# Blosc/c-blosc

Measured on AMD Instinct MI355X. Metric: compress+decompress GB/s (uncompressed) at 1/2/4/8 GPUs vs HBM roofline; ratio, higher is better.
Workload: dtype u8; 1 GPU; config #2: byte-shuffle + lz4 clevel=5 typesize=8, 128 x 64 MiB bench19 chunks per GPU (8 GiB), step = compress pass + decompress pass, device-resident; chunks_per_gpu=128, chunks_total=128, chunk_bytes=67108864

## Files before the change

c-blosc_amd/csrc/blosc_api.hip:

```cpp
#include <errno.h>
#include <pthread.h>
#include <stdio.h>
#include <stdlib.h>
#include <string.h>

#include <memory>
#include <new>

#include "../../include/blosc.h"
#include "../../include/blosc_gpu.h"
#include "../../include/blosc_gpu_packed.h"
#include "../../include/blosc_gpu_params.h"
#include "../../include/blosc_gpu_select.h"
#include "../../include/blosc_gpu_getitem.h"
#include "../../include/blosc_gpu_take.h"
#include "../../include/blosc_gpu_put.h"
#include "../../include/blosc_gpu_checksum.h"
#include "blosc_format.h"
#include "engine.h"

using namespace bamd;

static pthread_mutex_t g_mutex = PTHREAD_MUTEX_INITIALIZER;
static int g_compressor = BLOSC_BLOSCLZ;
// ... 289 lines not shown

int blosc_decompress(const void* src, void* dest, size_t destsize) {
  if (!g_initlib) blosc_init();
  const char* ev;
  if ((ev = getenv("BLOSC_NTHREADS")) != NULL) {
    long v = strtol(ev, NULL, 10);
    if (v != EINVAL && v > 0) { int r = blosc_set_nthreads((int)v); if (r < 0) return r; }
  }
  const bool nolock = getenv("BLOSC_NOLOCK") != NULL;
  if (!nolock) pthread_mutex_lock(&g_mutex);
  int r = decompress_one(src, dest, destsize);
  if (!nolock) pthread_mutex_unlock(&g_mutex);
  return r;
}

int blosc_getitem(const void* src, int start, int nitems, void* dest) {
  return engine_getitem(src, start, nitems, dest, engine_is_device_pointer(src), engine_is_device_pointer(dest), (hipStream_t)0);
}

int blosc_gpu_set_device(int device) { return engine_set_device(device); }

static int compress_batch(int clevel, int doshuffle, size_t typesize, const char* compressor, size_t blocksize,
                          int nchunks, const void* const* src, const size_t* nbytes, void* const* dest,
                          const size_t* destsize, int* cbytes_out, void* stream, bool device_ptrs) {
  if (nchunks <= 0) return 0;
  CompressParams p;
  if (!call_params(clevel, doshuffle, typesize, compressor, blocksize, &p)) return answer_not_built(nchunks, cbytes_out, nullptr);
  return compress_call(&p, false, nchunks, jobs_from_arrays(nchunks, src, dest, nbytes, destsize), cbytes_out, device_ptrs, stream, nullptr);
}
int blosc_gpu_compress_batch(int clevel, int doshuffle, size_t typesize, const char* compressor, size_t blocksize,
                             int nchunks, const void* const* src, const size_t* nbytes, void* const* dest,
                             const size_t* destsize, int* cbytes_out, void* stream) {
  return compress_batch(clevel, doshuffle, typesize, compressor, blocksize, nchunks, src, nbytes, dest, destsize, cbytes_out, stream, true);
}
int blosc_gpu_compress_batch_host(int clevel, int doshuffle, size_t typesize, const char* compressor, size_t blocksize,
                                  int nchunks, const void* const* src, const size_t* nbytes, void* const* dest,
                                  const size_t* destsize, int* cbytes_out) {
  return compress_batch(clevel, doshuffle, typesize, compressor, blocksize, nchunks, src, nbytes, dest, destsize, cbytes_out, nullptr, false);
}

static int decompress_batch(int nchunks, const void* const* src, const size_t* srcsize, void* const* dest,
                            const size_t* destsize, int* nbytes_out, void* stream, bool device_ptrs) {
  if (nchunks <= 0) return 0;
  return decompress_call(nchunks, jobs_from_arrays(nchunks, src, dest, srcsize, destsize), nbytes_out, device_ptrs, stream, nullptr);
}
int blosc_gpu_decompress_batch(int nchunks, const void* const* src, const size_t* srcsize, void* const* dest,
                               const size_t* destsize, int* nbytes_out, void* stream) {
  return decompress_batch(nchunks, src, srcsize, dest, destsize, nbytes_out, stream, true);
}
int blosc_gpu_decompress_batch_host(int nchunks, const void* const* src, const size_t* srcsize, void* const* dest,
                                    const size_t* destsize, int* nbytes_out) {
  return decompress_batch(nchunks, src, srcsize, dest, destsize, nbytes_out, nullptr, false);
}

size_t blosc_gpu_packed_bound(int nchunks, const size_t* nbytes, size_t align) {
  if (nchunks <= 0 || !nbytes || !packed_align(&align)) return 0;
  size_t total = 0;
  for (int i = 0; i < nchunks; i++) total += (nbytes[i] + BLOSC_MAX_OVERHEAD + align - 1) / align * align;
  return total;
}

int blosc_gpu_compress_packed(int clevel, int doshuffle, size_t typesize, const char* compressor, size_t blocksize,
                              int nchunks, const void* const* src, const size_t* nbytes, void* dest, size_t destsize, size_t align,
                              size_t* offsets_out, int* cbytes_out, void* stream) {
  const int c = packed_compress_opening(nchunks, src, nbytes, dest, destsize, &align, offsets_out, cbytes_out);
  if (c != kGo) return c;
  CompressParams p;
  if (!call_params(clevel, doshuffle, typesize, compressor, blocksize, &p)) return answer_not_built(nchunks, cbytes_out, offsets_out);
  const PackedBuffer pk{dest, destsize, align, offsets_out};
  return compress_call(&p, false, nchunks, jobs_from_arrays(nchunks, src, nullptr, nbytes, nullptr), cbytes_out, true, stream, &pk);
}

int blosc_gpu_compress_batch_params(int nchunks, const blosc_gpu_cparams* params, const void* const* src, const size_t* nbytes,
                                    void* const* dest, const size_t* destsize, int* cbytes_out, void* stream) {
  if (nchunks <= 0) return 0;
  if (!params || !src || !nbytes || !dest || !destsize || !cbytes_out) return -1;
  return compress_call(chunk_params(nchunks, params).get(), true, nchunks, jobs_from_arrays(nchunks, src, dest, nbytes, destsize), cbytes_out, true, stream,
                       nullptr);
}
int blosc_gpu_compress_packed_params(int nchunks, const blosc_gpu_cparams* params, const void* const* src, const size_t* nbytes,
                                     void* dest, size_t destsize, size_t align, size_t* offsets_out, int* cbytes_out, void* stream) {
  const int c = packed_compress_opening(nchunks, src, nbytes, dest, destsize, &align, offsets_out, cbytes_out);
  if (c != kGo) return c;
  if (!params) return -1;
  const PackedBuffer pk{dest, destsize, align, offsets_out};
  return compress_call(chunk_params(nchunks, params).get(), true, nchunks, jobs_from_arrays(nchunks, src, nullptr, nbytes, nullptr), cbytes_out, true, stream,
                       &pk);
}

static bool select_tables(int nchunks, const int* cand_first, const blosc_gpu_cparams* cands, const int* choice_out) {
  if (!cand_first || !cands || !choice_out || cand_first[0] != 0) return false;
  for (int i = 0; i < nchunks; i++) if (cand_first[i + 1] < cand_first[i]) return false;
  return true;
}
int blosc_gpu_compress_batch_select(int nchunks, const int* cand_first, const blosc_gpu_cparams* cands, const void* const* src, const size_t* nbytes,
                                    void* const* dest, const size_t* destsize, int* cbytes_out, int* choice_out, int* cand_cbytes_out, void* stream) {
  if (nchunks <= 0) return 0;
  if (!src || !nbytes || !dest || !destsize || !cbytes_out || !select_tables(nchunks, cand_first, cands, choice_out)) return -1;
  const CandidateSelect sel{cand_first, choice_out, cand_cbytes_out};
  return compress_call(chunk_params(cand_first[nchunks], cands).get(), true, nchunks, jobs_from_arrays(nchunks, src, dest, nbytes, destsize), cbytes_out, true,
                       stream, nullptr, &sel);
}
int blosc_gpu_compress_packed_select(int nchunks, const int* cand_first, const blosc_gpu_cparams* cands, const void* const* src, const size_t* nbytes,
                                     void* dest, size_t destsize, size_t align, size_t* offsets_out, int* cbytes_out, int* choice_out,
                                     int* cand_cbytes_out, void* stream) {
  const int c = packed_compress_opening(nchunks, src, nbytes, dest, destsize, &align, offsets_out, cbytes_out);
  if (c != kGo) return c;
  if (!select_tables(nchunks, cand_first, cands, choice_out)) return -1;
  const PackedBuffer pk{dest, destsize, align, offsets_out};
  const CandidateSelect sel{cand_first, choice_out, cand_cbytes_out};
  return compress_call(chunk_params(cand_first[nchunks], cands).get(), true, nchunks, jobs_from_arrays(nchunks, src, nullptr, nbytes, nullptr), cbytes_out, true,
                       stream, &pk, &sel);
}

int blosc_gpu_decompress_packed(int nchunks, const void* container, size_t containersize, const size_t* offsets,
                                void* dest, size_t destsize, size_t* dest_offsets_out, int* nbytes_out, void* stream) {
  const int c = packed_opening(nchunks, dest_offsets_out);
  if (c != kGo) return c;
  if (!container || !offsets || !nbytes_out) return -1;
  const PackedBuffer pk{dest, dest ? destsize : 0, 0, dest_offsets_out};
  return decompress_call(nchunks, jobs_from_spans(nchunks, container, containersize, offsets, nullptr, BLOSC_MIN_HEADER_LENGTH), nbytes_out, true, stream, &pk);
}

int blosc_gpu_cbuffer_sizes_batch(int nchunks, const void* const* src, size_t* nbytes, size_t* cbytes, size_t* blocksize, void* stream) {
  if (nchunks < 0 || (nchunks > 0 && !src)) return -1;
  if (nchunks == 0) return 0;
  Table<Header> h = table<Header>(nchunks);
  if (!h) return -1;
  const int r = engine_chunk_headers(nchunks, src, h.get(), (hipStream_t)stream);
  for (int i = 0; r == 0 && i < nchunks; i++) {
    const bool known = h[i].version == BLOSC_VERSION_FORMAT;
    if (nbytes) nbytes[i] = known ? (size_t)h[i].nbytes : 0;
    if (cbytes) cbytes[i] = known ? (size_t)h[i].cbytes : 0;
    if (blocksize) blocksize[i] = known ? (size_t)h[i].blocksize : 0;
  }
  return r;
}

int blosc_gpu_device_count(void) { return engine_device_count(); }
int blosc_gpu_partition(size_t nchunks, int world, int rank, size_t* lo, size_t* hi) {
  if (world <= 0 || rank < 0 || rank >= world || !lo || !hi) return -1;
  const size_t w = (size_t)world, r = (size_t)rank;
  size_t l = (r * nchunks + w - 1) / w, h = ((r + 1) * nchunks + w - 1) / w;
  if (h > nchunks) h = nchunks;
  *lo = l; *hi = h;
  return 0;
}
struct MultiArg {
  int dev, rc; bool compress; size_t lo, hi;
  int clevel, doshuffle; size_t typesize; const char* compressor; size_t blocksize;
  const void* const* src; const size_t* insize; void* const* dest; const size_t* destsize; int* out;
};
static void* multi_worker(void* p) {
  MultiArg& a = *(MultiArg*)p;
  a.rc = 0;
  if (a.hi == a.lo) return nullptr;
  if (engine_thread_device(a.dev) != 0) { a.rc = -1; return nullptr; }
  const int n = (int)(a.hi - a.lo);
  const bool devp = engine_is_device_pointer(a.src[a.lo]);
  if (a.compress) a.rc = compress_batch(a.clevel, a.doshuffle, a.typesize, a.compressor, a.blocksize, n, a.src + a.lo, a.insize + a.lo, a.dest + a.lo,
                                        a.destsize + a.lo, a.out + a.lo, nullptr, devp);
  else a.rc = decompress_batch(n, a.src + a.lo, a.insize ? a.insize + a.lo : nullptr, a.dest + a.lo, a.destsize + a.lo, a.out + a.lo, nullptr, devp);
  (void)engine_thread_device(-1);
  return nullptr;
}
static int run_multi(MultiArg proto, int ndev, const int* devices, int nchunks) {
  if (nchunks <= 0) return 0;
  const int have = engine_device_count();
  if (ndev <= 0 || ndev > 64) return -1;
  MultiArg args[64];
  pthread_t th[64];
  for (int r = 0; r < ndev; r++) {
    args[r] = proto;
    args[r].dev = devices ? devices[r] : r;
    if (args[r].dev < 0 || args[r].dev >= have) { fprintf(stderr, "blosc_amd: multi-GPU call names device %d, this node shows %d\n", args[r].dev, have); return -1; }
    (void)blosc_gpu_partition((size_t)nchunks, ndev, r, &args[r].lo, &args[r].hi);
  }
  int started = 0, rc = 0;
  for (; started < ndev; started++) if (pthread_create(&th[started], nullptr, multi_worker, &args[started]) != 0) { rc = -1; break; }
  for (int r = 0; r < started; r++) { pthread_join(th[r], nullptr); if (args[r].rc < 0) rc = args[r].rc; }
  return rc;
}
int blosc_gpu_compress_batch_multi(int ndev, const int* devices, int clevel, int doshuffle, size_t typesize, const char* compressor, size_t blocksize,
                                   int nchunks, const void* const* src, const size_t* nbytes, void* const* dest, const size_t* destsize, int* cbytes_out) {
  MultiArg a{}; a.compress = true; a.clevel = clevel; a.doshuffle = doshuffle; a.typesize = typesize; a.compressor = compressor; a.blocksize = blocksize;
  a.src = src; a.insize = nbytes; a.dest = dest; a.destsize = destsize; a.out = cbytes_out;
  return run_multi(a, ndev, devices, nchunks);
}
int blosc_gpu_decompress_batch_multi(int ndev, const int* devices, int nchunks, const void* const* src, const size_t* srcsize, void* const* dest,
                                     const size_t* destsize, int* nbytes_out) {
  MultiArg a{}; a.compress = false; a.src = src; a.insize = srcsize; a.dest = dest; a.destsize = destsize; a.out = nbytes_out;
  return run_multi(a, ndev, devices, nchunks);
}

int blosc_gpu_getitem(const void* src, int start, int nitems, void* dest, void* stream) {
  return engine_getitem(src, start, nitems, dest, true, true, (hipStream_t)stream);
}

int blosc_gpu_getitem_batch(int nchunks, const void* const* src, int nranges, const int* chunk, const int* start, const int* nitems,
                            void* const* dest, int* result_out, void* stream) {
  if (nchunks < 0 || nranges < 0) return -1;
  if (nranges == 0) return 0;
  if ((nchunks > 0 && !src) || !chunk || !start || !nitems || !dest || !result_out) return -1;
  return getitem_call(nchunks, jobs_from_arrays(nchunks, src, nullptr, nullptr, nullptr), nranges, chunk, start, nitems, dest, result_out, stream, nullptr);
}
int blosc_gpu_getitem_packed(int nchunks, const void* container, size_t containersize, const size_t* offsets,
                             int nranges, const int* chunk, const int* start, const int* nitems,
                             void* dest, size_t destsize, size_t* dest_offsets_out, int* result_out, void* stream) {
  if (nchunks < 0) return -1;
  const int c = packed_opening(nranges, dest_offsets_out);
  if (c != kGo) return c;
  if ((nchunks > 0 && (!container || !offsets)) || !chunk || !start || !nitems || !result_out) return -1;
  const PackedBuffer pk{dest, dest ? destsize : 0, 0, dest_offsets_out};
  return getitem_call(nchunks, jobs_from_spans(nchunks, container, containersize, offsets, nullptr, BLOSC_MIN_HEADER_LENGTH), nranges, chunk, start, nitems,
                      nullptr, result_out, stream, &pk);
}

static int take_opening(int nchunks, size_t row_bytes, size_t nidx, const void* index, const void* dest) {
  if (nchunks < 0 || row_bytes < 1 || row_bytes > 65536) return -1;
  if (nidx && (!index || !dest)) return -1;
  return kGo;
}
static int take_call(int nchunks, const Table<Job>& jobs, size_t row_bytes, size_t nidx, const int64_t* index, void* dest, int* status,
                     int* chunk_rows_out, size_t* failed_out, void* stream) {
  if (!jobs) return -1;
  if (nchunks == 0 && nidx == 0) return 0;
  return engine_take(nchunks, jobs.get(), row_bytes, nidx, index, dest, status, chunk_rows_out, failed_out, (hipStream_t)stream);
}
int blosc_gpu_take_batch(int nchunks, const void* const* src, size_t row_bytes, size_t nidx, const int64_t* index, void* dest, int* status,
                         int* chunk_rows_out, size_t* failed_out, void* stream) {
  const int c = take_opening(nchunks, row_bytes, nidx, index, dest);
  if (c != kGo) return c;
  if (nchunks > 0 && !src) return -1;
  return take_call(nchunks, jobs_from_arrays(nchunks, src, nullptr, nullptr, nullptr), row_bytes, nidx, index, dest, status, chunk_rows_out, failed_out, stream);
}
int blosc_gpu_take_packed(int nchunks, const void* container, size_t containersize, const size_t* offsets, size_t row_bytes, size_t nidx,
                          const int64_t* index, void* dest, int* status, int* chunk_rows_out, size_t* failed_out, void* stream) {
  const int c = take_opening(nchunks, row_bytes, nidx, index, dest);
  if (c != kGo) return c;
  if (nchunks > 0 && (!container || !offsets)) return -1;
  return take_call(nchunks, jobs_from_spans(nchunks, container, containersize, offsets, nullptr, BLOSC_MIN_HEADER_LENGTH), row_bytes, nidx, index, dest, status,
                   chunk_rows_out, failed_out, stream);
}

static int put_opening(int nchunks, size_t row_bytes, size_t nidx, const void* index, const void* rows, const blosc_gpu_cparams* params, void* dest,
                       size_t destsize, size_t* align, size_t* offsets_out, int* cbytes_out) {
  const int c = take_opening(nchunks, row_bytes, nidx, index, rows);
  if (c != kGo) return c;
  if (nidx > (size_t)UINT32_MAX - 1 || !packed_align(align) || !offsets_out || (!dest && destsize)) return -1;
  if (nchunks > 0 && (!params || !cbytes_out)) return -1;
  return kGo;
}
static int put_call(int nchunks, const Table<Job>& jobs, size_t row_bytes, size_t nidx, const int64_t* index, const void* rows, const blosc_gpu_cparams* params,
                    void* dest, size_t destsize, size_t align, size_t* offsets_out, int* cbytes_out, int* rewritten_out, int* status, int* chunk_rows_out,
                    size_t* failed_out, void* stream) {
  if (!jobs) return -1;
  if (nchunks == 0 && nidx == 0) { offsets_out[0] = 0; if (failed_out) *failed_out = 0; return 0; }
  Table<CompressParams> p = chunk_params(nchunks, params);
  if (!p) return -1;
  const PackedBuffer pk{dest, destsize, align, offsets_out};
  return engine_put(nchunks, jobs.get(), row_bytes, nidx, index, rows, p.get(), &pk, cbytes_out, rewritten_out, status, chunk_rows_out, failed_out, (hipStream_t)stream);
}
int blosc_gpu_put_batch(int nchunks, const void* const* src, size_t row_bytes, size_t nidx, const int64_t* index, const void* rows,
                        const blosc_gpu_cparams* params, void* dest, size_t destsize, size_t align, size_t* offsets_out, int* cbytes_out,
                        int* rewritten_out, int* status, int* chunk_rows_out, size_t* failed_out, void* stream) {
  const int c = put_opening(nchunks, row_bytes, nidx, index, rows, params, dest, destsize, &align, offsets_out, cbytes_out);
  if (c != kGo) return c;
  if (nchunks > 0 && !src) return -1;
  return put_call(nchunks, jobs_from_arrays(nchunks, src, nullptr, nullptr, nullptr), row_bytes, nidx, index, rows, params, dest, destsize, align, offsets_out,
                  cbytes_out, rewritten_out, status, chunk_rows_out, failed_out, stream);
}
int blosc_gpu_put_packed(int nchunks, const void* container, size_t containersize, const size_t* offsets, size_t row_bytes, size_t nidx,
                         const int64_t* index, const void* rows, const blosc_gpu_cparams* params, void* dest, size_t destsize, size_t align,
                         size_t* offsets_out, int* cbytes_out, int* rewritten_out, int* status, int* chunk_rows_out, size_t* failed_out, void* stream) {
  const int c = put_opening(nchunks, row_bytes, nidx, index, rows, params, dest, destsize, &align, offsets_out, cbytes_out);
  if (c != kGo) return c;
  if (nchunks > 0 && (!container || !offsets)) return -1;
  const uintptr_t s0 = (uintptr_t)container, s1 = s0 + containersize, d0 = (uintptr_t)dest, d1 = d0 + destsize;
  if (nchunks > 0 && destsize && containersize && s0 < d1 && d0 < s1) return -1;
  return put_call(nchunks, jobs_from_spans(nchunks, container, containersize, offsets, nullptr, BLOSC_MIN_HEADER_LENGTH), row_bytes, nidx, index, rows, params,
                  dest, destsize, align, offsets_out, cbytes_out, rewritten_out, status, chunk_rows_out, failed_out, stream);
}

int blosc_gpu_checksum_batch(int kind, int nruns, const void* const* src, const size_t* nbytes, unsigned int* digest_out, void* stream) {
  const int c = checksum_opening(kind, nruns);
  if (c != kGo) return c;
  if (!src || !nbytes || !digest_out) return -1;
  return checksum_call(kind, nruns, jobs_from_arrays(nruns, src, nullptr, nbytes, nullptr), digest_out, stream);
}
int blosc_gpu_checksum_packed(int kind, int nruns, const void* container, size_t containersize, const size_t* offsets,
                              const size_t* length, unsigned int* digest_out, void* stream) {
  const int c = checksum_opening(kind, nruns);
  if (c != kGo) return c;
  if (!offsets || !digest_out) return -1;
  if (!container && offsets[nruns] > offsets[0]) return -1;
  return checksum_call(kind, nruns, jobs_from_spans(nruns, container, containersize, offsets, length, 0), digest_out, stream);
}

__attribute__((visibility("default"))) int blosc_internal_persistent_grids(int cap, const char** names, int* launched, int* occupancy) {
  return bamd::engine_persistent_grids(cap, names, launched, occupancy);
}
__attribute__((visibility("default"))) int blosc_internal_enc_lz_occupancy(int dynamic_lds) { return bamd::engine_enc_lz_occupancy(dynamic_lds); }
__attribute__((visibility("default"))) void blosc_internal_last_compress_tasks(unsigned out[3]) { bamd::engine_last_compress_tasks(out); }

__attribute__((visibility("default"))) void blosc_internal_shuffle(const size_t typesize, const size_t blocksize,
                                                                   const uint8_t* src, const uint8_t* dest) {
  if (engine_filter(0, typesize, blocksize, src, (void*)dest) != 0) fprintf(stderr, "blosc_amd: shuffle failed (no GPU?)\n");
}
__attribute__((visibility("default"))) void blosc_internal_unshuffle(const size_t typesize, const size_t blocksize,
                                                                     const uint8_t* src, const uint8_t* dest) {
  if (engine_filter(1, typesize, blocksize, src, (void*)dest) != 0) fprintf(stderr, "blosc_amd: unshuffle failed (no GPU?)\n");
}
__attribute__((visibility("default"))) void blosc_internal_shuffle_generic(const size_t typesize, const size_t blocksize,
                                                                           const uint8_t* const src, uint8_t* const dest) {
  blosc_internal_shuffle(typesize, blocksize, src, dest);
}
__attribute__((visibility("default"))) void blosc_internal_unshuffle_generic(const size_t typesize, const size_t blocksize,
                                                                             const uint8_t* const src, uint8_t* const dest) {
  blosc_internal_unshuffle(typesize, blocksize, src, dest);
}
#define BAMD_SHUFFLE_ALIAS(isa)                                                                                                                  \
  __attribute__((visibility("default"))) void blosc_internal_shuffle_##isa(const size_t typesize, const size_t blocksize, const uint8_t* const src, \
                                                                           uint8_t* const dest) { blosc_internal_shuffle(typesize, blocksize, src, dest); } \
  __attribute__((visibility("default"))) void blosc_internal_unshuffle_##isa(const size_t typesize, const size_t blocksize, const uint8_t* const src, \
                                                                             uint8_t* const dest) { blosc_internal_unshuffle(typesize, blocksize, src, dest); }
BAMD_SHUFFLE_ALIAS(sse2)
BAMD_SHUFFLE_ALIAS(avx2)
#undef BAMD_SHUFFLE_ALIAS
__attribute__((visibility("default"))) int blosc_internal_bitshuffle(const size_t typesize, const size_t blocksize,
                                                                     const uint8_t* src, const uint8_t* dest,
                                                                     const uint8_t* tmp) {
  (void)tmp;
  if (engine_filter(2, typesize, blocksize, src, (void*)dest) != 0) return -1;
  const size_t n = blocksize / typesize;
  return (int)((n % 8) ? n : n * typesize);
}
__attribute__((visibility("default"))) int blosc_internal_bitunshuffle(const size_t typesize, const size_t blocksize,
                                                                       const uint8_t* src, const uint8_t* dest,
                                                                       const uint8_t* tmp) {
  (void)tmp;
  if (engine_filter(3, typesize, blocksize, src, (void*)dest) != 0) return -1;
  const size_t n = blocksize / typesize;
  return (int)((n % 8) ? n : n * typesize);
}

__attribute__((visibility("default"))) int blosc_amd_policy_blocksize(int clevel, int typesize, int nbytes, int forced,
                                                                      int codec, int splitmode) {
  return compute_blocksize(clevel, typesize, nbytes, forced, codec, splitmode);
}
__attribute__((visibility("default"))) int blosc_amd_policy_split(int codec, int typesize, int blocksize, int splitmode) {
  return split_block(codec, typesize, blocksize, splitmode);
}
__attribute__((visibility("default"))) void blosc_amd_getitem_pass_bytes(size_t bytes) { engine_getitem_pass_bytes(bytes); }

__attribute__((visibility("default"))) void blosc_amd_checksum_tile_bytes(size_t bytes) { engine_checksum_tile_bytes(bytes); }

void blosc_gpu_profile(int enable) { engine_prof_enable(enable); }
void blosc_gpu_profile_reset(void) { engine_prof_reset(); }
int blosc_gpu_profile_get(const char* kernel, double* total_ms, int* launches) { return engine_prof_get(kernel, total_ms, launches); }

}
```

c-blosc_amd/csrc/enc_lz.h:

```cpp
constexpr int ENC_WAVES = 1;
#ifndef BAMD_ENC_HASH_BITS
#define BAMD_ENC_HASH_BITS 11
#endif
constexpr int ENC_HASH_BITS = BAMD_ENC_HASH_BITS;
constexpr int ENC_TAB = 1 << ENC_HASH_BITS;
typedef uint32_t enc_entry_t;
#ifndef BAMD_ENC_SPLIT_TAB
#define BAMD_ENC_SPLIT_TAB 1
#endif
constexpr int ENC_TAB_BYTES = BAMD_ENC_SPLIT_TAB ? ENC_TAB * 3 : ENC_TAB * 4;
#ifndef BAMD_ENC_MINWAVES
#define BAMD_ENC_MINWAVES (BAMD_ENC_SPLIT_TAB ? 6 : 5)
#endif
#ifndef BAMD_ENC_SEQ_SKIPCAP
#define BAMD_ENC_SEQ_SKIPCAP 32u
#endif
#ifndef BAMD_ENC_LZ_MINWAVES
#define BAMD_ENC_LZ_MINWAVES 6
#endif
constexpr int LDS_BYTES_PER_CU = 160 * 1024;
constexpr int LDS_GRANULE_BYTES = 1280;
constexpr int lds_occupied(int bytes) { return (bytes + LDS_GRANULE_BYTES - 1) / LDS_GRANULE_BYTES * LDS_GRANULE_BYTES; }
constexpr int lds_workgroups_per_cu(int bytes) { return bytes > 0 ? LDS_BYTES_PER_CU / lds_occupied(bytes) : 32; }
constexpr int ENC_LDS_WAVES = lds_workgroups_per_cu(ENC_TAB_BYTES);
constexpr int ENC_WAVES_PER_CU = ENC_LDS_WAVES < 4 * BAMD_ENC_MINWAVES ? ENC_LDS_WAVES : 4 * BAMD_ENC_MINWAVES;
constexpr int ENC_LZ_SCR_BYTES = 256;
constexpr int ENC_LZ_LDS_WAVES = lds_workgroups_per_cu(ENC_TAB_BYTES + ENC_LZ_SCR_BYTES);
constexpr int ENC_LZ_WAVES_PER_CU = ENC_LZ_LDS_WAVES < 4 * BAMD_ENC_LZ_MINWAVES ? ENC_LZ_LDS_WAVES : 4 * BAMD_ENC_LZ_MINWAVES;
static_assert(lds_occupied(ENC_TAB_BYTES + ENC_LZ_SCR_BYTES) * ENC_LZ_WAVES_PER_CU <= LDS_BYTES_PER_CU, "the LZ4 kernel's workgroups of one CU fit its LDS");

struct EncTable {
  __attribute__((address_space(3))) uint32_t* w;
  __attribute__((address_space(3))) uint16_t* pos;
  __attribute__((address_space(3))) uint8_t* tag;
  __device__ __forceinline__ void init(void* base) {
    w = (__attribute__((address_space(3))) uint32_t*)base;
    pos = (__attribute__((address_space(3))) uint16_t*)base;
    tag = (__attribute__((address_space(3))) uint8_t*)base + 2 * ENC_TAB;
  }
  __device__ __forceinline__ void clear(int lane) {
    for (int k = lane; k < ENC_TAB_BYTES / 4; k += 64) w[k] = 0u;
  }
  __device__ __forceinline__ void put(uint32_t h, uint32_t entry) {
    if (BAMD_ENC_SPLIT_TAB) { pos[h] = (uint16_t)entry; tag[h] = (uint8_t)(entry >> 24); }
    else w[h] = entry;
  }
  __device__ __forceinline__ uint32_t get(uint32_t h) const {
    if (BAMD_ENC_SPLIT_TAB) return (uint32_t)pos[h] | ((uint32_t)tag[h] << 24);
    return w[h];
  }
  __device__ __forceinline__ static bool tag_equal(uint32_t a, uint32_t b) {
    return BAMD_ENC_SPLIT_TAB ? ((a ^ b) >> 24) == 0u : ((a ^ b) >> 16) == 0u;
  }
};

__device__ __forceinline__ uint32_t enc_mix(uint32_t seq) { return seq * 2654435761u; }
__device__ __forceinline__ uint32_t enc_slot(uint32_t mix) { return mix >> (32 - ENC_HASH_BITS); }
__device__ __forceinline__ uint32_t enc_entry(uint32_t mix, uint32_t p) { return ((mix << ENC_HASH_BITS) & 0xffff0000u) | (p & 0xffffu); }

__device__ __forceinline__ uint64_t ld8u(const gu8* p) { return g_ld8(p); }

__device__ __forceinline__ uint32_t common16(const uint4& x, const uint4& y) {
  const uint64_t lo = ((uint64_t)(x.y ^ y.y) << 32) | (x.x ^ y.x);
  const uint64_t hi = ((uint64_t)(x.w ^ y.w) << 32) | (x.z ^ y.z);
  if (lo) return (uint32_t)__builtin_ctzll(lo) >> 3;
  return hi ? 8u + ((uint32_t)__builtin_ctzll(hi) >> 3) : 16u;
}

__device__ __forceinline__ uint32_t wave_common_fwd_rest(const gu8* src, uint32_t n, uint32_t a, uint32_t b,
                                                         uint32_t maxlen, uint32_t done, int lane) {
  if (done == 256u && done < maxlen && a + done + 1024u <= n) {
    const uint4 x0 = g_ld16(src + a + done + 16 * lane), y0 = g_ld16(src + b + done + 16 * lane);
    const uint32_t q1 = done + 16u * (uint32_t)lane;
    uint32_t e1 = common16(x0, y0);
    const uint32_t r1 = q1 < maxlen ? maxlen - q1 : 0u;
    if (e1 > r1) e1 = r1;
    const uint64_t s1 = __ballot(e1 < 16u);
    if (s1) { const int f = __builtin_ctzll(s1); return done + 16u * (uint32_t)f + (uint32_t)__builtin_amdgcn_readlane((int)e1, f); }
    done += 1024u;
  }
  while (done < maxlen && a + done + 2048u <= n) {
    const gu8* pa = src + a + done + 16 * lane;
    const gu8* pb = src + b + done + 16 * lane;
    const uint4 x0 = g_ld16(pa), x1 = g_ld16(pa + 1024);
    const uint4 y0 = g_ld16(pb), y1 = g_ld16(pb + 1024);
    const uint32_t q = done + 16u * (uint32_t)lane;
    uint32_t e0 = common16(x0, y0), e1 = common16(x1, y1);
    const uint32_t r0 = q < maxlen ? maxlen - q : 0u;
    const uint32_t r1 = q + 1024u < maxlen ? maxlen - q - 1024u : 0u;
    if (e0 > r0) e0 = r0;
    if (e1 > r1) e1 = r1;
    const uint64_t s0 = __ballot(e0 < 16u);
    if (s0) { const int f = __builtin_ctzll(s0); return done + 16u * (uint32_t)f + (uint32_t)__builtin_amdgcn_readlane((int)e0, f); }
    const uint64_t s1 = __ballot(e1 < 16u);
    if (s1) { const int f = __builtin_ctzll(s1); return done + 1024u + 16u * (uint32_t)f + (uint32_t)__builtin_amdgcn_readlane((int)e1, f); }
    done += 2048u;
  }
  while (done < maxlen) {
    const uint32_t q = done + 8u * (uint32_t)lane;
    uint32_t vb = 0;
    if (q < maxlen) vb = (maxlen - q < 8u) ? maxlen - q : 8u;
    uint32_t eq = 0;
    if (vb) {
      if (a + q + 8u <= n) {
        uint64_t x = ld8u(src + a + q) ^ ld8u(src + b + q);
        eq = x ? (uint32_t)(__builtin_ctzll(x) >> 3) : 8u;
        if (eq > vb) eq = vb;
      } else {
        while (eq < vb && src[a + q + eq] == src[b + q + eq]) eq++;
      }
    }
    const uint64_t stop = __ballot(eq < 8u);
    if (stop) {
      const int f = __builtin_ctzll(stop);
      return done + 8u * (uint32_t)f + (uint32_t)__builtin_amdgcn_readlane((int)eq, f);
    }
    done += 512u;
  }
  return maxlen;
}
__device__ __forceinline__ uint32_t wave_common_first256(uint32_t x, uint32_t maxlen, int lane) {
  const uint32_t q = 4u * (uint32_t)lane;
  uint32_t e0 = x ? (uint32_t)(__builtin_ctz(x) >> 3) : 4u;
  const uint32_t r0 = q < maxlen ? maxlen - q : 0u;
  if (e0 > r0) e0 = r0;
  const uint64_t s0 = __ballot(e0 < 4u);
  if (s0) { const int f = __builtin_ctzll(s0); return 4u * (uint32_t)f + (uint32_t)__builtin_amdgcn_readlane((int)e0, f); }
  return 0xffffffffu;
}
__device__ __forceinline__ uint32_t wave_common_fwd(const gu8* src, uint32_t n, uint32_t a, uint32_t b,
                                                    uint32_t maxlen, int lane) {
  uint32_t done = 0;
  if (maxlen && a + 256u <= n) {
    const uint32_t r = wave_common_first256(g_ld4(src + a + 4 * lane) ^ g_ld4(src + b + 4 * lane), maxlen, lane);
    if (r != 0xffffffffu) return r;
    done = 256u;
  }
  return wave_common_fwd_rest(src, n, a, b, maxlen, done, lane);
}

#ifdef BAMD_ENC_NOSTORE
#define ENC_ST1(ptr, val) do { (void)(ptr); (void)(val); } while (0)
#else
#define ENC_ST1(ptr, val) do { *(ptr) = (val); } while (0)
#endif
__device__ __forceinline__ uint32_t emit_ext255(gu8* p, uint32_t v, int lane) {
  const uint32_t n255 = v / 255u, rem = v - n255 * 255u;
  for (uint32_t k = (uint32_t)lane; k < n255; k += 64u) ENC_ST1(p + k, (uint8_t)255u);
  if (lane == 0) ENC_ST1(p + n255, (uint8_t)rem);
  return n255 + 1u;
}

enum { EF_LZ4 = 0, EF_BLOSCLZ = 1, EF_ZSTD = 2, EF_ZLIB = 3, EF_ZLIB2 = 4 };
#ifndef BAMD_ZSTD_MINLEN
#define BAMD_ZSTD_MINLEN 4
#endif

struct ZsSink {
  gu8* lit;
  uint32_t nlit, litcap;
  BAMD_GAS uint64_t* seq;
  uint32_t nseq, seqcap;
};
__device__ __forceinline__ uint32_t zs_emit_seq(ZsSink& z, const gu8* lit, uint32_t ll, uint32_t off, uint32_t mlen, int lit_lane0, uint32_t ownbyte, int lane);

struct DflSink {
  gu8* out; uint32_t cap;
  uint32_t pos;
  uint32_t acc, nb;
  volatile BAMD_LAS uint32_t* zb;
};
__device__ __forceinline__ uint32_t wave_incl_scan_u32(uint32_t v, int lane) {
#pragma unroll
  for (int d = 1; d < 64; d <<= 1) { const uint32_t t = (uint32_t)__shfl_up((int)v, d, 64); if (lane >= d) v += t; }
  return v;
}
__device__ __forceinline__ bool dfl_put_symbols(DflSink& z, uint32_t bits, uint32_t nbits, int lane) {
  const uint32_t incl = wave_incl_scan_u32(nbits, lane);
  const uint32_t total = (uint32_t)__builtin_amdgcn_readlane((int)incl, 63);
  z.zb[lane] = lane == 0 ? z.acc : 0u;
  if (lane == 0) z.zb[64] = 0u;
  BAMD_LDS_SYNC();
  if (nbits) {
    const uint32_t start = z.nb + incl - nbits, w = start >> 5, sh = start & 31u;
    __hip_atomic_fetch_or((BAMD_LAS uint32_t*)z.zb + w, bits << sh, __ATOMIC_RELAXED, __HIP_MEMORY_SCOPE_WAVEFRONT);
    if (sh + nbits > 32u) __hip_atomic_fetch_or((BAMD_LAS uint32_t*)z.zb + w + 1u, bits >> (32u - sh), __ATOMIC_RELAXED, __HIP_MEMORY_SCOPE_WAVEFRONT);
  }
  const uint32_t fill = z.nb + total, ndw = fill >> 5;
  if (z.pos + 4u * ndw + 16u > z.cap) return false;
  BAMD_LDS_SYNC();
  const uint32_t mine = z.zb[lane], rest = z.zb[ndw];
  if ((uint32_t)lane < ndw) g_st4(z.out + z.pos + 4u * (uint32_t)lane, mine);
  z.acc = uni(rest); z.nb = fill & 31u; z.pos += 4u * ndw;
  return true;
}
__device__ __forceinline__ uint32_t dfl_emit_seq(DflSink& z, const gu8* lit, uint32_t ll, uint32_t dist, uint32_t mlen, int lit_lane0, uint32_t ownbyte, int lane) {
  const bool in_regs = lit_lane0 >= 0 && ll <= 64u && (uint32_t)lit_lane0 + ll <= 64u;
  const uint32_t np = mlen ? dfl::npieces(mlen) : 0u;
  uint32_t ldone = 0, pdone = 0;
  do {
    const uint32_t lcnt = ll - ldone < 64u ? ll - ldone : 64u;
    uint32_t pcnt = 0;
    if (ldone + lcnt == ll) { pcnt = np - pdone < 64u - lcnt ? np - pdone : 64u - lcnt; }
    const uint32_t vreg = in_regs ? (uint32_t)__builtin_amdgcn_ds_bpermute((int)(((uint32_t)lit_lane0 + (uint32_t)lane) & 63u) << 2, (int)ownbyte) & 0xffu : 0u;
    dfl::Sym s = {0u, 0u};
    if ((uint32_t)lane < lcnt) s = dfl::literal(in_regs ? vreg : (uint32_t)lit[ldone + (uint32_t)lane]);
    else if ((uint32_t)lane < lcnt + pcnt) s = dfl::match(dfl::piece_len(mlen, pdone + (uint32_t)lane - lcnt, np), dist);
    if (!dfl_put_symbols(z, s.bits, s.nbits, lane)) return 0xffffffffu;
    ldone += lcnt; pdone += pcnt;
  } while (ldone < ll || pdone < np);
  return 0u;
}

__device__ __forceinline__ void emit_literals(gu8* dst, const gu8* lit, uint32_t ll, int lit_lane0, uint32_t ownbyte, int lane) {
  if (lit_lane0 >= 0 && ll <= 64u && (uint32_t)lit_lane0 + ll <= 64u) {
    const uint32_t v = (uint32_t)__builtin_amdgcn_ds_bpermute((int)(((uint32_t)lit_lane0 + (uint32_t)lane) & 63u) << 2, (int)ownbyte);
    if ((uint32_t)lane < ll) ENC_ST1(dst + lane, (uint8_t)v);
  } else {
    wave_copy_disjoint(dst, lit, ll, lane);
  }
}

__device__ __forceinline__ uint32_t lz4_emit_seq(gu8* dst, uint32_t op, uint32_t cap, const gu8* lit,
                                                 uint32_t ll, uint32_t off, uint32_t mlen, int lit_lane0, uint32_t ownbyte, int lane) {
  if (op + 1u + ll + (2u + 1u + 5u) + ll / 255u > cap) return 0xffffffffu;
  const uint32_t mcode = mlen - 4u;
  if (ll < 15u && mcode < 15u + 255u && (ll == 0u || (lit_lane0 >= 0 && (uint32_t)lit_lane0 + ll <= 64u))) {
    if (op + 1u + ll + 2u + (1u + 5u) + (mcode + 240u) / 255u > cap) return 0xffffffffu;
    const uint32_t v = (uint32_t)__builtin_amdgcn_ds_bpermute((int)(((uint32_t)lit_lane0 + (uint32_t)lane - 1u) & 63u) << 2, (int)ownbyte);
    uint32_t b = v;
    b = lane == 0 ? ((ll << 4) | (mcode < 15u ? mcode : 15u)) : b;
    b = (uint32_t)lane == ll + 1u ? off : b;
    b = (uint32_t)lane == ll + 2u ? off >> 8 : b;
    b = (uint32_t)lane == ll + 3u ? mcode - 15u : b;
    const uint32_t total = ll + 3u + (mcode >= 15u ? 1u : 0u);
    if ((uint32_t)lane < total) ENC_ST1(dst + op + lane, (uint8_t)b);
    return op + total;
  }
  const uint32_t tok = ((ll < 15u ? ll : 15u) << 4) | (mcode < 15u ? mcode : 15u);
  if (lane == 0) ENC_ST1(dst + op, (uint8_t)tok);
  op += 1u;
  if (ll >= 15u) op += emit_ext255(dst + op, ll - 15u, lane);
  emit_literals(dst + op, lit, ll, lit_lane0, ownbyte, lane);
  op += ll;
  if (lane < 2) ENC_ST1(dst + op + lane, (uint8_t)(off >> (8 * lane)));
  op += 2u;
  if (op + (1u + 5u) + (mcode + 240u) / 255u > cap) return 0xffffffffu;
  if (mcode >= 15u) op += emit_ext255(dst + op, mcode - 15u, lane);
  return op;
}
__device__ __forceinline__ uint32_t lz4_emit_tail(gu8* dst, uint32_t op, uint32_t cap, const gu8* lit,
                                                  uint32_t run, int lane) {
  if (op + run + 1u + (run + 255u - 15u) / 255u > cap) return 0xffffffffu;
  if (lane == 0) dst[op] = (uint8_t)((run < 15u ? run : 15u) << 4);
  op += 1u;
  if (run >= 15u) op += emit_ext255(dst + op, run - 15u, lane);
  wave_copy_disjoint(dst + op, lit, run, lane);
  return op + run;
}

__device__ __forceinline__ uint32_t blz_emit_literals(gu8* dst, uint32_t op, uint32_t cap, const gu8* lit,
                                                      uint32_t ll, int lane) {
  if (ll == 0u) return op;
  const uint32_t nch = (ll + 31u) >> 5;
  if (op + ll + nch > cap) return 0xffffffffu;
  for (uint32_t c = (uint32_t)lane; c < nch; c += 64u) {
    const uint32_t cnt = (ll - 32u * c < 32u) ? ll - 32u * c : 32u;
    dst[op + 33u * c] = (uint8_t)(cnt - 1u);
  }
  for (uint32_t k = (uint32_t)lane; k < ll; k += 64u) dst[op + k + (k >> 5) + 1u] = lit[k];
  return op + ll + nch;
}
__device__ __forceinline__ uint32_t blz_emit_match(gu8* dst, uint32_t op, uint32_t cap, uint32_t dist,
                                                   uint32_t mlen, int lane) {
  const uint32_t L = mlen - 2u;
  uint32_t bd = dist - 1u;
  const bool far = bd >= 8191u;
  if (far) bd -= 8191u;
  const uint32_t hi = far ? 31u : (bd >> 8);
  const uint32_t next = (L >= 7u) ? (L - 7u) / 255u + 1u : 0u;
  const uint32_t total = 1u + next + (far ? 3u : 1u);
  if (op + total + 2u > cap) return 0xffffffffu;
  if (lane == 0) dst[op] = (uint8_t)(((L < 7u ? L : 7u) << 5) | hi);
  op += 1u;
  if (L >= 7u) op += emit_ext255(dst + op, L - 7u, lane);
  if (far) {
    if (lane == 0) { dst[op] = 255u; dst[op + 1] = (uint8_t)(bd >> 8); dst[op + 2] = (uint8_t)bd; }
    op += 3u;
  } else {
    if (lane == 0) dst[op] = (uint8_t)bd;
    op += 1u;
  }
  return op;
}

#ifndef BAMD_ENC_RANK_CAP
#define BAMD_ENC_RANK_CAP 20
#endif
constexpr uint32_t RANK_CAP = BAMD_ENC_RANK_CAP;

struct Bytes20 { uint64_t a, b; uint32_t c; };

__device__ __forceinline__ Bytes20 load20(const gu8* src, uint32_t pos, uint32_t n) {
  Bytes20 r;
  if (pos + 20u <= n) { r.a = g_ld8(src + pos); r.b = g_ld8(src + pos + 8u); r.c = RANK_CAP > 16u ? g_ld4(src + pos + 16u) : 0u; }
  else {
    r.a = 0; r.b = 0; r.c = 0;
    for (uint32_t k = 0; k < 20u && pos + k < n; k++) {
      const uint64_t v = src[pos + k];
      if (k < 8u) r.a |= v << (8u * k); else if (k < 16u) r.b |= v << (8u * (k - 8u)); else r.c |= (uint32_t)v << (8u * (k - 16u));
    }
  }
  return r;
}
__device__ __forceinline__ uint32_t common20(const Bytes20& x, const Bytes20& y) {
  uint64_t d = x.a ^ y.a;
  if (d) return (uint32_t)__builtin_ctzll(d) >> 3;
  d = x.b ^ y.b;
  if (d) return 8u + ((uint32_t)__builtin_ctzll(d) >> 3);
  const uint32_t e = x.c ^ y.c;
  return e ? 16u + ((uint32_t)__builtin_ctz(e) >> 3) : 20u;
}
__device__ __forceinline__ uint32_t runlen20(const Bytes20& x, uint32_t v) {
  const uint64_t rep = 0x0101010101010101ull * (uint64_t)v;
  Bytes20 y; y.a = rep; y.b = rep; y.c = (uint32_t)rep;
  return common20(x, y);
}
template <int N> __device__ __forceinline__ uint32_t dpp_row_shr0(uint32_t v) {
  return (uint32_t)__builtin_amdgcn_update_dpp(0, (int)v, 0x110 + N, 0xf, 0xf, true);
}
__device__ __forceinline__ uint32_t wave_max_u32(uint32_t v) {
  uint32_t t;
// ... 452 lines not shown
```

c-blosc_amd/csrc/enc_lz4p.h:

```cpp
#ifndef BAMD_ENC_PAR
#define BAMD_ENC_PAR 1
#endif
constexpr int ENC_SCR_BYTES = 256;
static_assert(ENC_SCR_BYTES == ENC_LZ_SCR_BYTES, "enc_lz.h sizes the persistent grid with this scratch in mind");
static_assert((ENC_TAB_BYTES + ENC_SCR_BYTES) % LDS_GRANULE_BYTES == 0 || !BAMD_ENC_SPLIT_TAB, "table + scratch fill whole LDS granules");
#ifndef BAMD_ENC_BACK2
#define BAMD_ENC_BACK2 1
#endif
#ifndef BAMD_ENC_SKIPCAP
#define BAMD_ENC_SKIPCAP 32u
#endif
#ifndef BAMD_ENC_NEIGHBOUR
#define BAMD_ENC_NEIGHBOUR 4u
#endif
#ifndef BAMD_ENC_KEEPJ
#define BAMD_ENC_KEEPJ 0
#endif
#ifndef BAMD_ENC_EXT2
#define BAMD_ENC_EXT2 1
#endif
#ifndef BAMD_ENC_LAUNDER
#define BAMD_ENC_LAUNDER 1
#endif
#ifndef BAMD_ENC_PREFULL
#define BAMD_ENC_PREFULL 1
#endif

template <int N> __device__ __forceinline__ uint32_t dpp_row_shl0(uint32_t v) {
  return (uint32_t)__builtin_amdgcn_update_dpp(0, (int)v, 0x100 + N, 0xf, 0xf, true);
}
__device__ __forceinline__ uint32_t umax32(uint32_t a, uint32_t b) { return a > b ? a : b; }
__device__ __forceinline__ uint32_t umin32(uint32_t a, uint32_t b) { return a < b ? a : b; }

__device__ __forceinline__ uint32_t wave_common_fwd_lite(const gu8* src, uint32_t n, uint32_t a, uint32_t b, uint32_t maxlen, int lane) {
  uint32_t done = 0;
  if (maxlen && a + 256u <= n) {
    const uint32_t x = g_ld4(src + a + 4 * lane) ^ g_ld4(src + b + 4 * lane);
    const uint32_t q = 4u * (uint32_t)lane;
    uint32_t e0 = x ? (uint32_t)(__builtin_ctz(x) >> 3) : 4u;
    const uint32_t r0 = q < maxlen ? maxlen - q : 0u;
    if (e0 > r0) e0 = r0;
    const uint64_t s0 = __ballot(e0 < 4u);
    if (s0) { const int f = __builtin_ctzll(s0); return 4u * (uint32_t)f + (uint32_t)__builtin_amdgcn_readlane((int)e0, f); }
    done = 256u;
  }
  while (done < maxlen && a + done + 1024u <= n) {
    const uint4 x0 = g_ld16(src + a + done + 16 * lane), y0 = g_ld16(src + b + done + 16 * lane);
    const uint32_t q1 = done + 16u * (uint32_t)lane;
    uint32_t e1 = common16(x0, y0);
    const uint32_t r1 = q1 < maxlen ? maxlen - q1 : 0u;
    if (e1 > r1) e1 = r1;
    const uint64_t s1 = __ballot(e1 < 16u);
    if (s1) { const int f = __builtin_ctzll(s1); return done + 16u * (uint32_t)f + (uint32_t)__builtin_amdgcn_readlane((int)e1, f); }
    done += 1024u;
  }
  while (done < maxlen) {
    const uint32_t q = done + 8u * (uint32_t)lane;
    uint32_t vb = 0;
    if (q < maxlen) vb = (maxlen - q < 8u) ? maxlen - q : 8u;
    uint32_t eq = 0;
    if (vb) {
      if (a + q + 8u <= n) {
        const uint64_t x = ld8u(src + a + q) ^ ld8u(src + b + q);
        eq = x ? (uint32_t)(__builtin_ctzll(x) >> 3) : 8u;
        if (eq > vb) eq = vb;
      } else {
        while (eq < vb && src[a + q + eq] == src[b + q + eq]) eq++;
      }
    }
    const uint64_t stop = __ballot(eq < 8u);
    if (stop) { const int f = __builtin_ctzll(stop); return done + 8u * (uint32_t)f + (uint32_t)__builtin_amdgcn_readlane((int)eq, f); }
    done += 512u;
  }
  return maxlen;
}

template <int SS>
__device__ uint32_t lz4_encode_wave_par(const gu8* __restrict__ src, uint32_t n, gu8* __restrict__ dst, uint32_t cap,
                                        int clevel, enc_entry_t* tab_generic, int lane_in EPROF_ARG) {
  static_assert(SS == 0 || SS == 1, "one or two positions per lane");
  const int lane = lane_in;
  constexpr uint32_t SPAN = 64u << SS;
  EncTable tab;
  tab.init((void*)tab_generic);
  volatile BAMD_LAS uint32_t* scr = (volatile BAMD_LAS uint32_t*)((BAMD_LAS uint8_t*)(void*)tab_generic + ENC_TAB_BYTES);
  if (n < 13u) return 0u;
  const uint32_t last_start = n - 12u;
  const uint32_t mlimit = n - 5u;
  const int accel = 10 - clevel;
  const uint32_t minlen = clevel >= 9 ? 4u : (clevel >= 6 ? 5u : 7u);
  tab.clear(lane);
  EncWindow win;
  win.init(src, n, lane);
  uint32_t ip = 0, anchor = 0, op = 0, nfail = 0;
  bool ins_pending = false;
  while (ip <= last_start) {
    int lane = lane_in;
#if !defined(BAMD_WAVE_EMU) && BAMD_ENC_LAUNDER
    asm volatile("; lane of this step" : "+v"(lane));
#endif
    const uint32_t lq = (uint32_t)lane << SS;
    const uint32_t p = ip + lq;
    const bool live = p <= last_start;
    const bool live1 = SS && p + 1u <= last_start;
    win.seek(ip, lane);
    const uint32_t lo = ip >= 4u ? ip - 4u : 0u;
    const uint32_t rb = lo & ~3u;
    const uint32_t D = (rb - win.wbase) >> 2;
    const int gsel = (int)((D + (uint32_t)lane) << 2);
    const uint32_t ra = (uint32_t)__builtin_amdgcn_ds_bpermute(gsel, (int)win.w0);
    const uint32_t rc = (uint32_t)__builtin_amdgcn_ds_bpermute(gsel, (int)win.w1);
    const uint32_t r = (D + (uint32_t)lane < 64u) ? ra : rc;
    const uint32_t bo0 = ip - rb;
    const uint32_t bo = bo0 + lq;
    const int ksel = (int)((bo >> 2) << 2);
    const uint32_t x0 = (uint32_t)__builtin_amdgcn_ds_bpermute(ksel, (int)r);
    const uint32_t x1 = (uint32_t)__builtin_amdgcn_ds_bpermute(ksel + 4, (int)r);
    const uint32_t x2 = (uint32_t)__builtin_amdgcn_ds_bpermute(ksel + 8, (int)r);
    const uint32_t x3 = (uint32_t)__builtin_amdgcn_ds_bpermute(ksel + 12, (int)r);
    const uint32_t x4 = (uint32_t)__builtin_amdgcn_ds_bpermute(ksel + 16, (int)r);
    const uint32_t x5 = (uint32_t)__builtin_amdgcn_ds_bpermute(ksel + 20, (int)r);
    const uint32_t sh = bo & 3u;
    const uint32_t o0 = __builtin_amdgcn_alignbyte(x1, x0, sh), o1 = __builtin_amdgcn_alignbyte(x2, x1, sh);
    const uint32_t o2 = __builtin_amdgcn_alignbyte(x3, x2, sh), o3 = __builtin_amdgcn_alignbyte(x4, x3, sh);
    const uint32_t o4 = __builtin_amdgcn_alignbyte(x5, x4, sh);
    const uint32_t ownpre = __builtin_amdgcn_alignbyte(x0, (uint32_t)__builtin_amdgcn_ds_bpermute(ksel - 4, (int)r), sh);
    Bytes20 own;
    own.a = ((uint64_t)o1 << 32) | o0; own.b = ((uint64_t)o3 << 32) | o2; own.c = RANK_CAP > 16u ? o4 : 0u;
    const uint64_t r01 = ((uint64_t)(uint32_t)__builtin_amdgcn_readlane((int)r, 1) << 32) | (uint32_t)__builtin_amdgcn_readlane((int)r, 0);
    const uint32_t before2 = bo0 >= 2u ? (uint32_t)(r01 >> (8u * (bo0 - 2u))) & 0xffffu : 0u;
    uint32_t prev;
    if (SS) prev = ownpre >> 24;
    else prev = (uint32_t)__builtin_amdgcn_update_dpp(0, (int)(o0 & 0xffu), 0x138, 0xf, 0xf, false);
    if (lane == 0) prev = ip ? (bo0 >= 2u ? before2 >> 8 : (uint32_t)(r01 >> (8u * (bo0 - 1u))) & 0xffu) : 0x100u;
    if (ins_pending) {
      const uint32_t m2 = enc_mix(before2 | (o0 << 16));
      if (lane == 0) tab.put(enc_slot(m2), enc_entry(m2, ip - 2u));
      ins_pending = false;
    }
    uint32_t cand = 0, limit = 0;
    bool tab_ok = false;
    const uint32_t mix = enc_mix(o0);
#define PAR_PUT() do { const uint32_t mix_ = enc_mix((uint32_t)own.a); tab.put(enc_slot(mix_), enc_entry(mix_, p)); } while (0)
#define PAR_PUT1() do { const uint32_t mix1_ = enc_mix((uint32_t)(own.a >> 8)); tab.put(enc_slot(mix1_), enc_entry(mix1_, p + 1u)); } while (0)
    if (live) {
      limit = mlimit - p; if (limit > RANK_CAP) limit = RANK_CAP;
      const uint32_t h = enc_slot(mix), mine = enc_entry(mix, p);
      const uint32_t e = tab.get(h);
      const uint32_t d = (p - e) & 0xffffu;
      if (d != 0u && d <= p && EncTable::tag_equal(e, mine)) { cand = p - d; tab_ok = true; }
    } else {
      prev = 0x100u;
    }
    PROF_LAP(8); PROF_ADD(0, 1);
    uint32_t len = 0, nb = 0;
    if (tab_ok) {
      const uint32_t cpre = cand >= 4u ? ld4u(src + cand - 4u) : 0u;
      const Bytes20 cb = load20(src, cand, n);
      if (cand >= 4u) { const uint32_t x = cpre ^ ownpre; nb = x ? (uint32_t)__builtin_clz(x) >> 3 : 4u; }
      len = common20(own, cb);
      if (len > limit) len = limit;
      if (len < 4u || len + (SS && nb ? 1u : 0u) < minlen) len = 0;
    }
    if (live && prev < 0x100u) {
      uint32_t rl = runlen20(own, prev);
      if (rl > limit) rl = limit;
      const uint32_t xr = (ownpre ^ (ownpre << 8)) | 0xffu;
      const uint32_t nbr = p >= 5u ? (uint32_t)__builtin_clz(xr) >> 3 : 0u;
      if (rl >= 4u && rl + (SS && nbr ? 1u : 0u) >= minlen && rl > len) { len = rl; cand = p - 1u; nb = nbr; }
    }
    win.settle(lane);
    PROF_LAP(9);
    const uint32_t step_end = ip + SPAN;
    const uint32_t cn = (p - cand) | (nb << 28);
    uint32_t S = len ? (((len + (SS && nb ? 1u : 0u) + SPAN - lq) << 11) | ((63u - (uint32_t)lane) << 5) | len) : 0u;
    S = umax32(S, dpp_row_shl0<1>(S)); S = umax32(S, dpp_row_shl0<2>(S)); S = umax32(S, dpp_row_shl0<4>(S)); S = umax32(S, dpp_row_shl0<8>(S));
    {
      const uint32_t t3 = (uint32_t)__builtin_amdgcn_readlane((int)S, 48);
      const uint32_t t2 = umax32((uint32_t)__builtin_amdgcn_readlane((int)S, 32), t3);
      const uint32_t t1 = umax32((uint32_t)__builtin_amdgcn_readlane((int)S, 16), t2);
      const uint32_t add = lane < 16 ? t1 : (lane < 32 ? t2 : (lane < 48 ? t3 : 0u));
      S = umax32(S, add);
    }
    uint32_t J0;
    {
      const uint32_t wS = 63u - ((S >> 5) & 63u), LS = S & 31u;
      const uint32_t nx = ((wS << SS) + LS + (SS ? 1u : 0u)) >> SS;
      J0 = (S == 0u || LS >= RANK_CAP || nx > 63u) ? 63u : nx;
    }
#if BAMD_ENC_KEEPJ
    const uint32_t J1 = (uint32_t)__builtin_amdgcn_ds_bpermute((int)(J0 << 2), (int)J0);
    const uint32_t J2 = (uint32_t)__builtin_amdgcn_ds_bpermute((int)(J1 << 2), (int)J1);
    const uint32_t J3 = (uint32_t)__builtin_amdgcn_ds_bpermute((int)(J2 << 2), (int)J2);
#endif
    uint32_t lane_lo = 0;
    bool any = false, tail_open = false;
    for (;;) {
#if !defined(BAMD_WAVE_EMU) && BAMD_ENC_LAUNDER
      asm volatile("; lane of this chain" : "+v"(lane));
#endif
#if !BAMD_ENC_KEEPJ
      const uint32_t J1 = (uint32_t)__builtin_amdgcn_ds_bpermute((int)(J0 << 2), (int)J0);
      const uint32_t J2 = (uint32_t)__builtin_amdgcn_ds_bpermute((int)(J1 << 2), (int)J1);
      const uint32_t J3 = (uint32_t)__builtin_amdgcn_ds_bpermute((int)(J2 << 2), (int)J2);
#endif
      uint32_t c = umin32((lane_lo + (SS ? 1u : 0u)) >> SS, 63u);
      { const uint32_t t = (uint32_t)__builtin_amdgcn_ds_bpermute((int)(c << 2), (int)J0); c = (lane & 1) ? t : c; }
      { const uint32_t t = (uint32_t)__builtin_amdgcn_ds_bpermute((int)(c << 2), (int)J1); c = (lane & 2) ? t : c; }
      { const uint32_t t = (uint32_t)__builtin_amdgcn_ds_bpermute((int)(c << 2), (int)J2); c = (lane & 4) ? t : c; }
      { const uint32_t t = (uint32_t)__builtin_amdgcn_ds_bpermute((int)(c << 2), (int)J3); c = (lane & 8) ? t : c; }
      const uint32_t Sr = (uint32_t)__builtin_amdgcn_ds_bpermute((int)(c << 2), (int)S);
      const bool valid = lane < 16 && c < 63u && Sr != 0u;
      const uint32_t nseq = (uint32_t)__builtin_popcountll(__ballot(valid));
      if (nseq == 0u) { tail_open = any; break; }
      any = true;
      const uint32_t last = nseq - 1u;
      const uint32_t w = 63u - ((Sr >> 5) & 63u), L = Sr & 31u;
      const uint32_t wq = w << SS;
      const uint32_t cnr = (uint32_t)__builtin_amdgcn_ds_bpermute((int)(w << 2), (int)cn);
      const uint32_t dist_r = cnr & 0xffffu, nb_r = cnr >> 28;
      const uint32_t cand_r = ip + wq - dist_r;
      uint32_t cq = c;
      if (SS) { const uint32_t e_prev = dpp_row_shr0<1>(wq + L); cq = lane == 0 ? lane_lo : e_prev; }
      const uint32_t room = wq - cq;
      const uint32_t w_last = (uint32_t)__builtin_amdgcn_readlane((int)wq, (int)last), L_last = (uint32_t)__builtin_amdgcn_readlane((int)L, (int)last);
      const uint32_t pm_last = ip + w_last;
      uint32_t mext = 0;
      if (L_last >= RANK_CAP && pm_last + RANK_CAP < mlimit) {
        const uint32_t c_last = (uint32_t)__builtin_amdgcn_readlane((int)cand_r, (int)last);
        mext = BAMD_ENC_EXT2 ? wave_common_fwd(src, n, pm_last + RANK_CAP, c_last + RANK_CAP, mlimit - (pm_last + RANK_CAP), lane)
                              : wave_common_fwd_lite(src, n, pm_last + RANK_CAP, c_last + RANK_CAP, mlimit - (pm_last + RANK_CAP), lane);
      }
      uint32_t back = valid ? umin32(nb_r, umin32(room, cand_r)) : 0u;
      if (BAMD_ENC_BACK2) {
        const bool more = valid && back == 4u && room > 4u && cand_r >= 12u;
        if (__ballot(more)) {
          const uint32_t pm = ip + wq;
          const uint64_t a = g_ld8(src + (more ? pm - 12u : 0u)), b = g_ld8(src + (more ? cand_r - 12u : 0u));
          const uint64_t x = a ^ b;
          const uint32_t eq = x ? (uint32_t)__builtin_clzll(x) >> 3 : 8u;
          if (more) back += umin32(eq, room - 4u);
        }
      }
      uint32_t pre = lane_lo == 0u ? ip - anchor : 0u;
      uint32_t pre_ext = 0;
      if (BAMD_ENC_PREFULL && pre) {
        const uint32_t b0 = (uint32_t)__builtin_amdgcn_readlane((int)back, 0), room0 = (uint32_t)__builtin_amdgcn_readlane((int)room, 0);
        const uint32_t cand0 = (uint32_t)__builtin_amdgcn_readlane((int)cand_r, 0);
        if (b0 == room0 && cand0 > b0) {
          uint32_t maxb = umin32(pre, cand0 - b0);
          if (maxb > 64u) maxb = 64u;
          const uint32_t pm0 = ip + (uint32_t)__builtin_amdgcn_readlane((int)wq, 0) - b0, cm0 = cand0 - b0;
          const bool bl = (uint32_t)lane < maxb;
          const uint32_t bx = src[bl ? pm0 - 1u - (uint32_t)lane : pm0], by = src[bl ? cm0 - 1u - (uint32_t)lane : cm0];
          const uint64_t bm = __ballot(!bl || bx != by);
          pre_ext = bm ? (uint32_t)__builtin_ctzll(bm) : 64u;
          pre -= pre_ext;
        }
      }
      PROF_LAP(10); PROF_ADD(2, L_last >= RANK_CAP); PROF_ADD(6, nseq);
      const uint32_t mlen = L + back + ((uint32_t)lane == last ? mext : 0u) + (lane == 0 ? pre_ext : 0u);
      const uint32_t mcode = mlen - 4u;
      const uint32_t inl = room - back;
      const uint32_t ll = inl + (lane == 0 ? pre : 0u);
      const bool r0pre = pre != 0u && lane == 0;
      const uint32_t hdr = r0pre ? 0u : (ll >= 15u ? 2u : 1u);
      const uint32_t nme = mcode >= 15u ? 1u : 0u;
      const uint32_t size = valid ? hdr + inl + 2u + nme : 0u;
      uint32_t incl = size;
      incl += dpp_row_shr0<1>(incl); incl += dpp_row_shr0<2>(incl); incl += dpp_row_shr0<4>(incl); incl += dpp_row_shr0<8>(incl);
      const uint32_t excl = incl - size;
      const uint32_t mcode_last = (uint32_t)__builtin_amdgcn_readlane((int)mcode, (int)last);
      const uint32_t extra_last = mcode_last >= 15u + 255u ? (mcode_last - 15u) / 255u : 0u;
      const uint32_t total = (uint32_t)__builtin_amdgcn_readlane((int)incl, (int)last) + extra_last;
      uint32_t ll0 = 0, prebytes = 0;
      if (pre) { ll0 = (uint32_t)__builtin_amdgcn_readlane((int)ll, 0); prebytes = 1u + (ll0 >= 15u ? 1u + (ll0 - 15u) / 255u : 0u) + pre; }
      if (op + prebytes + total + 8u > cap) return 0u;
      if (pre) {
        const uint32_t mc0 = (uint32_t)__builtin_amdgcn_readlane((int)mcode, 0);
        if (lane == 0) ENC_ST1(dst + op, (uint8_t)(((ll0 < 15u ? ll0 : 15u) << 4) | (mc0 < 15u ? mc0 : 15u)));
        op += 1u;
        if (ll0 >= 15u) op += emit_ext255(dst + op, ll0 - 15u, lane);
        wave_copy_disjoint(dst + op, src + anchor, pre, lane);
        op += pre;
        PROF_ADD(3, 1);
      }
      scr[lane] = 0u;
      BAMD_LDS_SYNC();
      if (valid) scr[cq >> SS] = 0x80000000u | (excl + hdr) | (inl << 10) | (w << 17) | (L << 23) | (SS ? (cq & 1u) << 28 : 0u);
      BAMD_LDS_SYNC();
      const uint32_t pw = scr[lane];
      const uint32_t myw = (SS && (pw & (1u << 28))) ? 0u : pw;
      const uint32_t myw1 = (SS && (pw & (1u << 28))) ? pw : 0u;
      const uint64_t fm = __ballot((myw >> 31) != 0u);
      uint32_t s;
      bool has;
      if (SS) {
        const uint64_t fm1 = __ballot((myw1 >> 31) != 0u);
        const uint64_t be = fm & ((2ull << lane) - 1ull), bo_ = fm1 & ((1ull << lane) - 1ull);
        const uint32_t se = 2u * (63u - (uint32_t)__builtin_clzll(be | 1ull)), so = 2u * (63u - (uint32_t)__builtin_clzll(bo_ | 1ull)) + 1u;
        s = (bo_ != 0ull && (be == 0ull || so > se)) ? so : se;
        has = (be | bo_) != 0ull;
      } else {
        const uint64_t below = fm & ((2ull << lane) - 1ull);
        s = 63u - (uint32_t)__builtin_clzll(below | 1ull);
        has = below != 0ull;
      }
      const uint32_t inf = scr[s >> SS];
      BAMD_LDS_SYNC();
      {
        const uint32_t tpos = op + excl;
        if (valid && hdr) ENC_ST1(dst + tpos, (uint8_t)(((ll < 15u ? ll : 15u) << 4) | (mcode < 15u ? mcode : 15u)));
        if (valid && hdr == 2u) ENC_ST1(dst + tpos + 1u, (uint8_t)(ll - 15u));
        const uint32_t opos = tpos + hdr + inl;
#ifndef BAMD_ENC_NOSTORE
        if (valid) g_st2(dst + opos, dist_r);
#endif
        if (valid && nme) ENC_ST1(dst + opos + 2u, (uint8_t)(mcode - 15u < 255u ? mcode - 15u : 255u));
        if (extra_last) {
          const uint32_t opos_last = (uint32_t)__builtin_amdgcn_readlane((int)opos, (int)last);
          emit_ext255(dst + opos_last + 2u, mcode_last - 15u, lane);
        }
      }
      {
        const uint32_t k = lq - s;
        const uint32_t i_out = inf & 1023u, i_inl = (inf >> 10) & 127u, i_w = ((inf >> 17) & 63u) << SS, i_L = (inf >> 23) & 31u;
        if (has && k < i_inl) ENC_ST1(dst + op + i_out + k, (uint8_t)own.a);
        const bool open_end = i_L < RANK_CAP;
        const uint32_t e = i_w + i_L;
        if (live && has && (lq <= i_w || (open_end && (lq + 2u == e || lq >= e)))) PAR_PUT();
      }
      if (SS) {
        const bool own1 = (myw1 >> 31) != 0u;
        const uint32_t inf1 = own1 ? myw1 : inf;
        const bool has1 = has || own1;
        const uint32_t q1 = lq + 1u, k1 = own1 ? 0u : q1 - s;
        const uint32_t j_out = inf1 & 1023u, j_inl = (inf1 >> 10) & 127u, j_w = ((inf1 >> 17) & 63u) << SS, j_L = (inf1 >> 23) & 31u;
        if (has1 && k1 < j_inl) ENC_ST1(dst + op + j_out + k1, (uint8_t)(own.a >> 8));
        const bool open1 = j_L < RANK_CAP;
        const uint32_t e1 = j_w + j_L;
        if (live1 && has1 && (q1 <= j_w || (open1 && (q1 + 2u == e1 || q1 >= e1)))) PAR_PUT1();
      }
      op += total;
      const uint32_t e_last = w_last + L_last + mext;
      anchor = ip + e_last;
      PROF_LAP(11);
      if (L_last < RANK_CAP || e_last >= SPAN) break;
      lane_lo = e_last;
      if (live && lq + 2u == lane_lo) PAR_PUT();
      if (live1 && lq + 3u == lane_lo) PAR_PUT1();
    }
    if (!any) {
      PROF_ADD(1, 1);
      if (live) PAR_PUT();
      if (live1) PAR_PUT1();
      nfail += 1u << SS;
      uint32_t adv = (nfail * (uint32_t)accel) / 16u;
      if (adv > BAMD_ENC_SKIPCAP - (1u << SS)) adv = BAMD_ENC_SKIPCAP - (1u << SS);
      if (BAMD_ENC_NEIGHBOUR && ((nfail >> SS) & (BAMD_ENC_NEIGHBOUR - 1u)) == 0u) adv = 0u;
      ip += SPAN + 64u * adv;
      continue;
    }
    nfail = 0;
    if (anchor >= step_end) {
      ip = anchor;
      ins_pending = true;
    } else {
      if (tail_open && live && lq >= lane_lo) PAR_PUT();
      if (tail_open && live1 && lq + 1u >= lane_lo) PAR_PUT1();
      ip = step_end;
    }
  }
#undef PAR_PUT
#undef PAR_PUT1
  op = lz4_emit_tail(dst, op, cap, src + anchor, n - anchor, lane);
  if (op == 0xffffffffu) return 0u;
  PROF_LAP(12);
  return op < n ? op : 0u;
}

#ifndef BAMD_ENC_STRIDE2_MAXCLEVEL
#define BAMD_ENC_STRIDE2_MAXCLEVEL 5
#endif
__device__ __forceinline__ uint32_t lz4_encode_wave_auto(const gu8* __restrict__ src, uint32_t n, gu8* __restrict__ dst, uint32_t cap,
                                                         int clevel, enc_entry_t* tab_generic, int lane EPROF_ARG) {
  if (clevel <= BAMD_ENC_STRIDE2_MAXCLEVEL) return lz4_encode_wave_par<1>(src, n, dst, cap, clevel, tab_generic, lane EPROF_PASS);
  return lz4_encode_wave_par<0>(src, n, dst, cap, clevel, tab_generic, lane EPROF_PASS);
}
```

c-blosc_amd/csrc/enc_shuffle.h:

```cpp
template <int T>
struct ElemRows { uint4 a, b; };

template <int T>
__device__ __forceinline__ ElemRows<T> shuffle_load(const gu8* src, uint32_t e, int lane) {
  ElemRows<T> x;
  const gu8* in = src + (size_t)(e + 4u * (uint32_t)lane) * T;
  x.a = g_ld16(in);
  if (T == 8) x.b = g_ld16(in + 16); else x.b = make_uint4(0, 0, 0, 0);
  return x;
}
template <int T>
__device__ __forceinline__ void shuffle_store(gu8* dst, uint32_t N, uint32_t e, int lane, const ElemRows<T>& x) {
  gu8* o = dst + e + 4u * (uint32_t)lane;
  uint32_t r0, r1, r2, r3;
  if (T == 8) {
    transpose4x4(x.a.x, x.a.z, x.b.x, x.b.z, r0, r1, r2, r3);
    g_st4(o, r0); g_st4(o + (size_t)N, r1); g_st4(o + 2 * (size_t)N, r2); g_st4(o + 3 * (size_t)N, r3);
    transpose4x4(x.a.y, x.a.w, x.b.y, x.b.w, r0, r1, r2, r3);
    g_st4(o + 4 * (size_t)N, r0); g_st4(o + 5 * (size_t)N, r1); g_st4(o + 6 * (size_t)N, r2); g_st4(o + 7 * (size_t)N, r3);
  } else {
    transpose4x4(x.a.x, x.a.y, x.a.z, x.a.w, r0, r1, r2, r3);
    g_st4(o, r0); g_st4(o + (size_t)N, r1); g_st4(o + 2 * (size_t)N, r2); g_st4(o + 3 * (size_t)N, r3);
  }
}
struct ElemRows2 { uint32_t lo, hi; };
struct ElemRows16 { uint4 v[4]; };
__device__ __forceinline__ ElemRows2 shuffle_load2(const gu8* src, uint32_t e, int lane) {
  const uint64_t w = g_ld8(src + (size_t)(e + 4u * (uint32_t)lane) * 2u);
  ElemRows2 x; x.lo = (uint32_t)w; x.hi = (uint32_t)(w >> 32);
  return x;
}
__device__ __forceinline__ void shuffle_rows2(const ElemRows2& x, uint32_t (&r)[16]) {
  r[0] = __builtin_amdgcn_perm(x.hi, x.lo, 0x06040200u);
  r[1] = __builtin_amdgcn_perm(x.hi, x.lo, 0x07050301u);
}
__device__ __forceinline__ ElemRows16 shuffle_load16(const gu8* src, uint32_t e, int lane) {
  const gu8* in = src + (size_t)(e + 16u * ((uint32_t)lane >> 2) + ((uint32_t)lane & 3u)) * 16u;
  ElemRows16 x;
#pragma unroll
  for (int k = 0; k < 4; k++) x.v[k] = g_ld16(in + 64 * k);
  return x;
}
__device__ __forceinline__ void shuffle_rows16(const ElemRows16& x, uint32_t (&r)[16], int lane) {
  transpose4x4(x.v[0].x, x.v[1].x, x.v[2].x, x.v[3].x, r[0], r[1], r[2], r[3]);
  transpose4x4(x.v[0].y, x.v[1].y, x.v[2].y, x.v[3].y, r[4], r[5], r[6], r[7]);
  transpose4x4(x.v[0].z, x.v[1].z, x.v[2].z, x.v[3].z, r[8], r[9], r[10], r[11]);
  transpose4x4(x.v[0].w, x.v[1].w, x.v[2].w, x.v[3].w, r[12], r[13], r[14], r[15]);
#pragma unroll
  for (int j = 0; j < 16; j++) r[j] = quad_byte_transpose(r[j], lane);
}
template <int T>
__device__ __forceinline__ void shuffle_store_rows(gu8* dst, uint32_t N, uint32_t e, int lane, const uint32_t (&r)[16]) {
  gu8* o = dst + e + 4u * (uint32_t)lane;
#pragma unroll
  for (int k = 0; k < T; k++) g_st4(o + (size_t)k * N, r[k]);
}
__device__ __forceinline__ uint32_t shuffle_block_rows2(const gu8* src, gu8* dst, uint32_t N, int lane) {
  uint32_t e = 0, r[16];
  for (; e + 1024u <= N; e += 1024u) {
    const ElemRows2 a = shuffle_load2(src, e, lane), b = shuffle_load2(src, e + 256u, lane);
    const ElemRows2 c = shuffle_load2(src, e + 512u, lane), d = shuffle_load2(src, e + 768u, lane);
    shuffle_rows2(a, r); shuffle_store_rows<2>(dst, N, e, lane, r);
    shuffle_rows2(b, r); shuffle_store_rows<2>(dst, N, e + 256u, lane, r);
    shuffle_rows2(c, r); shuffle_store_rows<2>(dst, N, e + 512u, lane, r);
    shuffle_rows2(d, r); shuffle_store_rows<2>(dst, N, e + 768u, lane, r);
  }
  for (; e + 256u <= N; e += 256u) { shuffle_rows2(shuffle_load2(src, e, lane), r); shuffle_store_rows<2>(dst, N, e, lane, r); }
  return e;
}
__device__ __forceinline__ uint32_t shuffle_block_rows16(const gu8* src, gu8* dst, uint32_t N, int lane) {
  uint32_t e = 0, r[16];
  for (; e + 512u <= N; e += 512u) {
    const ElemRows16 a = shuffle_load16(src, e, lane), b = shuffle_load16(src, e + 256u, lane);
    shuffle_rows16(a, r, lane); shuffle_store_rows<16>(dst, N, e, lane, r);
    shuffle_rows16(b, r, lane); shuffle_store_rows<16>(dst, N, e + 256u, lane, r);
  }
  for (; e + 256u <= N; e += 256u) { shuffle_rows16(shuffle_load16(src, e, lane), r, lane); shuffle_store_rows<16>(dst, N, e, lane, r); }
  return e;
}
template <int T>
__device__ void shuffle_block_wave_T(const gu8* src, gu8* dst, uint32_t bsize, int lane) {
  const uint32_t N = bsize / T;
  uint32_t e = 0;
  if constexpr (T == 2) e = shuffle_block_rows2(src, dst, N, lane);
  else if constexpr (T == 16) e = shuffle_block_rows16(src, dst, N, lane);
  else {
  for (; e + 1024u <= N; e += 1024u) {
    const ElemRows<T> a = shuffle_load<T>(src, e, lane), b = shuffle_load<T>(src, e + 256u, lane);
    const ElemRows<T> c = shuffle_load<T>(src, e + 512u, lane), d = shuffle_load<T>(src, e + 768u, lane);
    shuffle_store<T>(dst, N, e, lane, a); shuffle_store<T>(dst, N, e + 256u, lane, b);
    shuffle_store<T>(dst, N, e + 512u, lane, c); shuffle_store<T>(dst, N, e + 768u, lane, d);
  }
  for (; e + 256u <= N; e += 256u) shuffle_store<T>(dst, N, e, lane, shuffle_load<T>(src, e, lane));
  }
  for (uint32_t k = e * T + (uint32_t)lane; k < N * T; k += 64u) { const uint32_t el = k / T, j = k - el * T; dst[(size_t)j * N + el] = src[k]; }
  for (uint32_t k = N * T + (uint32_t)lane; k < bsize; k += 64u) dst[k] = src[k];
}

template <int T>
__device__ __forceinline__ void shuffle_rows(const ElemRows<T>& x, uint32_t (&r)[8]) {
  if (T == 8) {
    transpose4x4(x.a.x, x.a.z, x.b.x, x.b.z, r[0], r[1], r[2], r[3]);
    transpose4x4(x.a.y, x.a.w, x.b.y, x.b.w, r[4], r[5], r[6], r[7]);
  } else {
    transpose4x4(x.a.x, x.a.y, x.a.z, x.a.w, r[0], r[1], r[2], r[3]);
    r[4] = r[5] = r[6] = r[7] = 0;
  }
}
__device__ __forceinline__ uint32_t row_period(uint32_t w, int lane) {
  uint32_t p = 256u;
  for (uint32_t sh = 32u; sh >= 1u; sh >>= 1) {
    const uint32_t other = (uint32_t)__builtin_amdgcn_ds_bpermute((int)((((uint32_t)lane + sh) & 63u) << 2), (int)w);
    if (__ballot(other != w) != 0ull) return p;
    p = 4u * sh;
  }
  const uint32_t w0 = (uint32_t)__builtin_amdgcn_readfirstlane((int)w);
  if ((w0 >> 16) != (w0 & 0xffffu)) return 4u;
  return ((w0 >> 8) & 0xffu) == (w0 & 0xffu) ? 1u : 2u;
}
template <int T>
__device__ uint32_t shuffle_block_wave_detect(const gu8* src, gu8* dst, uint32_t bsize, int lane, uint32_t (&period)[8]) {
  const uint32_t N = bsize / T;
  uint32_t row0[8], r[8];
  uint32_t per = (1u << T) - 1u;
  shuffle_rows<T>(shuffle_load<T>(src, 0u, lane), row0);
  auto step = [&](const ElemRows<T>& x, uint32_t e) {
    if (per == 0u) { shuffle_store<T>(dst, N, e, lane, x); return; }
    shuffle_rows<T>(x, r);
    gu8* o = dst + e + 4u * (uint32_t)lane;
#pragma unroll
    for (int k = 0; k < T; k++) {
      if (per & (1u << k)) {
        if (__ballot(r[k] != row0[k]) == 0ull) continue;
        per &= ~(1u << k);
        for (uint32_t t = 0; t < e; t += 256u) g_st4(dst + (size_t)k * N + t + 4u * (uint32_t)lane, row0[k]);
      }
      g_st4(o + (size_t)k * N, r[k]);
    }
  };
  uint32_t e = 256u;
  for (; e + 1024u <= N; e += 1024u) {
    const ElemRows<T> a = shuffle_load<T>(src, e, lane), b = shuffle_load<T>(src, e + 256u, lane);
    const ElemRows<T> c = shuffle_load<T>(src, e + 512u, lane), d = shuffle_load<T>(src, e + 768u, lane);
    step(a, e); step(b, e + 256u); step(c, e + 512u); step(d, e + 768u);
  }
  for (; e + 256u <= N; e += 256u) step(shuffle_load<T>(src, e, lane), e);
#pragma unroll
  for (int k = 0; k < T; k++) {
    period[k] = 0u;
    if (per & (1u << k)) {
      g_st4(dst + (size_t)k * N + 4u * (uint32_t)lane, row0[k]);
      period[k] = row_period(row0[k], lane);
    }
  }
  return per;
}

template <int T>
__device__ uint32_t shuffle_block_wave_detect_x(const gu8* src, gu8* dst, uint32_t bsize, int lane, uint32_t (&period)[16]) {
  static_assert(T == 2 || T == 16, "typesize 4 / 8 use shuffle_block_wave_detect");
  const uint32_t N = bsize / T;
  uint32_t row0[16], r[16];
  uint32_t per = (1u << T) - 1u;
  if constexpr (T == 2) shuffle_rows2(shuffle_load2(src, 0u, lane), row0); else shuffle_rows16(shuffle_load16(src, 0u, lane), row0, lane);
  auto step = [&](uint32_t e) {
    if (per == 0u) { shuffle_store_rows<T>(dst, N, e, lane, r); return; }
    gu8* o = dst + e + 4u * (uint32_t)lane;
#pragma unroll
    for (int k = 0; k < T; k++) {
      if (per & (1u << k)) {
        if (__ballot(r[k] != row0[k]) == 0ull) continue;
        per &= ~(1u << k);
        for (uint32_t t = 0; t < e; t += 256u) g_st4(dst + (size_t)k * N + t + 4u * (uint32_t)lane, row0[k]);
      }
      g_st4(o + (size_t)k * N, r[k]);
    }
  };
  uint32_t e = 256u;
  if constexpr (T == 2) {
    for (; e + 1024u <= N; e += 1024u) {
      const ElemRows2 a = shuffle_load2(src, e, lane), b = shuffle_load2(src, e + 256u, lane);
      const ElemRows2 c = shuffle_load2(src, e + 512u, lane), d = shuffle_load2(src, e + 768u, lane);
      shuffle_rows2(a, r); step(e); shuffle_rows2(b, r); step(e + 256u); shuffle_rows2(c, r); step(e + 512u); shuffle_rows2(d, r); step(e + 768u);
    }
    for (; e + 256u <= N; e += 256u) { shuffle_rows2(shuffle_load2(src, e, lane), r); step(e); }
  } else {
    for (; e + 256u <= N; e += 256u) { shuffle_rows16(shuffle_load16(src, e, lane), r, lane); step(e); }
  }
#pragma unroll
  for (int k = 0; k < T; k++) {
    period[k] = 0u;
    if (per & (1u << k)) {
      g_st4(dst + (size_t)k * N + 4u * (uint32_t)lane, row0[k]);
      period[k] = row_period(row0[k], lane);
    }
  }
  return per;
}

template <int T>
__device__ __forceinline__ void shuffle_block_detect_T(const gu8* src, gu8* dst, uint32_t bsize, StreamDesc* planes, int lane) {
  uint32_t period[(T == 4 || T == 8) ? 8 : 16];
  uint32_t per;
  if constexpr (T == 4 || T == 8) per = shuffle_block_wave_detect<T>(src, dst, bsize, lane, period);
  else per = shuffle_block_wave_detect_x<T>(src, dst, bsize, lane, period);
#pragma unroll
  for (int k = 0; k < T; k++)
    if ((per & (1u << k)) && lane == 0) planes[k].result = -(int32_t)period[k];
}
__device__ __attribute__((noinline)) void shuffle_block_task_x(const gu8* src_, gu8* dst_, uint32_t bsize_, uint32_t T_, bool det_, StreamDesc* planes_, int lane) {
  const gu8* src = uni_ptr(src_); gu8* dst = uni_ptr(dst_);
  const uint32_t bsize = uni(bsize_), T = uni(T_); const bool det = uni((uint32_t)det_) != 0u;
  const uint64_t pv = (uint64_t)planes_;
  StreamDesc* planes = (StreamDesc*)(((uint64_t)uni((uint32_t)(pv >> 32)) << 32) | uni((uint32_t)pv));
  if (T == 16u) { if (det) shuffle_block_detect_T<16>(src, dst, bsize, planes, lane); else shuffle_block_wave_T<16>(src, dst, bsize, lane); }
  else { if (det) shuffle_block_detect_T<2>(src, dst, bsize, planes, lane); else shuffle_block_wave_T<2>(src, dst, bsize, lane); }
}
template <int T, int EPL>
__device__ __forceinline__ void bitshuffle_pass(const gu8* src, gu8* dst, uint32_t rowlen, uint32_t e0, uint32_t nchunks, int lane) {
  constexpr uint32_t CB = (uint32_t)EPL * T, NDW = CB / 4u;
  constexpr int G = EPL / 8;
  static_assert(EPL == 32 || EPL == 16, "a dword or two bytes of every bit row per lane");
  const uint32_t m0 = e0 >> 3, t = (uint32_t)lane;
  if (t >= nchunks) return;
  const gu8* in = src + (size_t)(e0 + (uint32_t)EPL * t) * T;
  uint32_t w[NDW];
#pragma unroll
  for (uint32_t k = 0; k < NDW / 4u; k++) { const uint4 v = g_ld16(in + 16u * k); w[4 * k] = v.x; w[4 * k + 1] = v.y; w[4 * k + 2] = v.z; w[4 * k + 3] = v.w; }
#pragma unroll
  for (int j = 0; j < T; j++) {
    uint64_t x[G];
#pragma unroll
    for (int g = 0; g < G; g++) {
      uint64_t v = 0;
#pragma unroll
      for (int k = 0; k < 8; k++) { const int idx = (8 * g + k) * T + j; v |= (uint64_t)((w[idx >> 2] >> (8 * (idx & 3))) & 0xffu) << (8 * k); }
      x[g] = bit_transpose8(v);
    }
#pragma unroll
    for (int b = 0; b < 8; b++) {
      uint32_t rw = 0;
#pragma unroll
      for (int g = 0; g < G; g++) rw |= (uint32_t)((x[g] >> (8 * b)) & 0xff) << (8 * g);
      gu8* rp = dst + (size_t)(8 * j + b) * rowlen + m0 + (uint32_t)G * t;
      if (G == 4) g_st4(rp, rw); else g_st2(rp, rw);
    }
  }
}
template <int T>
__device__ void bitshuffle_block_wave_T(const gu8* src, gu8* dst, uint32_t bsize, int lane) {
  constexpr int EPL = T == 8 ? 16 : 32;
  const uint32_t N = bsize / T;
  if (bsize < T || (N & 7u)) {
    for (uint32_t k = 16u * (uint32_t)lane; k < bsize; k += 1024u) {
      if (k + 16u <= bsize) g_st16(dst + k, g_ld16(src + k));
      else for (uint32_t t = k; t < bsize; t++) dst[t] = src[t];
    }
    return;
  }
  const uint32_t rowlen = N >> 3;
  uint32_t e0 = 0;
  for (; e0 + 64u * EPL <= N; e0 += 64u * EPL) bitshuffle_pass<T, EPL>(src, dst, rowlen, e0, 64u, lane);
  if (N - e0 >= (uint32_t)EPL) { const uint32_t nch = (N - e0) / (uint32_t)EPL; bitshuffle_pass<T, EPL>(src, dst, rowlen, e0, nch, lane); e0 += (uint32_t)EPL * nch; }
  if ((uint32_t)lane < ((N - e0) >> 3)) {
    const uint32_t m = (e0 >> 3) + (uint32_t)lane;
#pragma unroll
    for (int j = 0; j < T; j++) {
      uint64_t v = 0;
#pragma unroll
      for (int k = 0; k < 8; k++) v |= (uint64_t)src[(size_t)(8u * m + (uint32_t)k) * T + (uint32_t)j] << (8 * k);
      v = bit_transpose8(v);
#pragma unroll
      for (int b = 0; b < 8; b++) dst[(size_t)(8 * j + b) * rowlen + m] = (uint8_t)(v >> (8 * b));
    }
  }
  for (uint32_t k = N * T + (uint32_t)lane; k < bsize; k += 64u) dst[k] = src[k];
}
__device__ __attribute__((noinline)) void bitshuffle_block_task_x(const gu8* src_, gu8* dst_, uint32_t bsize_, uint32_t T_, int lane) {
  const gu8* src = uni_ptr(src_); gu8* dst = uni_ptr(dst_);
  const uint32_t bsize = uni(bsize_), T = uni(T_);
  if (T == 8u) bitshuffle_block_wave_T<8>(src, dst, bsize, lane);
  else if (T == 4u) bitshuffle_block_wave_T<4>(src, dst, bsize, lane);
  else if (T == 2u) bitshuffle_block_wave_T<2>(src, dst, bsize, lane);
  else bitshuffle_block_wave_T<1>(src, dst, bsize, lane);
}

__device__ __forceinline__ bool shuffle_generic_T(uint32_t T) { return T >= 3u && T <= 32u && T != 4u && T != 8u && T != 16u; }
__device__ __attribute__((noinline)) void shuffle_block_generic(volatile uint32_t* lds_, const gu8* src_, gu8* dst_, uint32_t bsize_, uint32_t T_, int lane) {
  const uint64_t lv = (uint64_t)lds_;
  lu8* S = (lu8*)(BAMD_LAS uint32_t*)(volatile uint32_t*)(((uint64_t)uni((uint32_t)(lv >> 32)) << 32) | uni((uint32_t)lv));
  const gu8* src = uni_ptr(src_); gu8* dst = uni_ptr(dst_);
  const uint32_t bsize = uni(bsize_), T = uni(T_), N = bsize / T;
  const uint32_t H = ((uint32_t)ENC_TAB_BYTES / 128u) / T;
  static_assert(128u * 32u <= (uint32_t)ENC_TAB_BYTES, "a half tile of the widest element must fit the smallest table a wave owns");
  uint32_t e = 0;
  while (e + 128u <= N) {
    const uint32_t h_here = (N - e) / 128u < H ? (N - e) / 128u : H, K = 128u * h_here;
    const gu8* in = src + (size_t)e * T;
    for (uint32_t q = (uint32_t)lane; q < K * T / 16u; q += 64u) l_st16(S + 16u * q, g_ld16(in + 16u * q));
    LDS_ORDER(); BAMD_LDS_SYNC();
    for (uint32_t el = 4u * (uint32_t)lane; el < K; el += 256u) {
      const lu8* mine = S + el * T;
      if ((T & 3u) == 0u) {
        const BAMD_LAS uint32_t* w = (const BAMD_LAS uint32_t*)mine;
        for (uint32_t j = 0; j < T; j += 4u) {
          uint32_t r0, r1, r2, r3;
          transpose4x4(w[j / 4u], w[(T + j) / 4u], w[(2u * T + j) / 4u], w[(3u * T + j) / 4u], r0, r1, r2, r3);
          gu8* o = dst + (size_t)j * N + e + el;
          g_st4(o, r0); g_st4(o + (size_t)N, r1); g_st4(o + 2 * (size_t)N, r2); g_st4(o + 3 * (size_t)N, r3);
        }
        continue;
      }
      for (uint32_t j = 0; j < T; j++) {
        const uint32_t v = (uint32_t)mine[j] | ((uint32_t)mine[T + j] << 8) | ((uint32_t)mine[2u * T + j] << 16) | ((uint32_t)mine[3u * T + j] << 24);
        g_st4(dst + (size_t)j * N + e + el, v);
      }
    }
    LDS_ORDER(); BAMD_LDS_SYNC();
    e += K;
  }
  for (uint32_t k = e * T + (uint32_t)lane; k < N * T; k += 64u) { const uint32_t el = k / T, j = k - el * T; dst[(size_t)j * N + el] = src[k]; }
  for (uint32_t k = N * T + (uint32_t)lane; k < bsize; k += 64u) dst[k] = src[k];
}

__device__ __attribute__((noinline)) void shuffle_block_task(const ChunkDesc* chunks, const BlockDesc* blocks, uint32_t gb,
                                                             uint32_t* blk_ready, StreamDesc* streams, int detect, int lane, volatile uint32_t* lds) {
  const BlockDesc* b = blocks + gb;
  const ChunkDesc* c = chunks + uni((uint32_t)b->chunk);
  const uint32_t blk = uni((uint32_t)b->blk), bsize = uni((uint32_t)b->bsize), bs = uni((uint32_t)c->blocksize);
  const gu8* src = uni_ptr(as_global(c->src)) + (size_t)blk * bs;
  gu8* dst = uni_ptr(as_global(c->filt)) + (size_t)blk * bs;
  const uint32_t T = uni((uint32_t)c->typesize), N = bsize / T;
  const bool det = detect && uni((uint32_t)b->nstreams) == T && N * T == bsize && (N & 255u) == 0u && N >= 1024u &&
                   (uni((uint32_t)c->fmt) == (uint32_t)FMT_LZ4 || uni((uint32_t)c->fmt) == (uint32_t)FMT_BLOSCLZ);
  StreamDesc* planes = streams + uni((uint32_t)b->first_stream);
  if (uni(c->mode) & CH_BITSHUFFLE) bitshuffle_block_task_x(src, dst, bsize, T, lane);
  else if (shuffle_generic_T(T)) shuffle_block_generic(lds, src, dst, bsize, T, lane);
  else if (T == 8u) { if (det) shuffle_block_detect_T<8>(src, dst, bsize, planes, lane); else shuffle_block_wave_T<8>(src, dst, bsize, lane); }
  else if (T == 4u) { if (det) shuffle_block_detect_T<4>(src, dst, bsize, planes, lane); else shuffle_block_wave_T<4>(src, dst, bsize, lane); }
  else shuffle_block_task_x(src, dst, bsize, T, det, planes, lane);
  __builtin_amdgcn_s_waitcnt(0);
  if (lane == 0) __hip_atomic_store(&blk_ready[gb], 1u, __ATOMIC_RELAXED, __HIP_MEMORY_SCOPE_AGENT);
}

__device__ __forceinline__ uint32_t emit_periodic_stream(const gu8* in, uint32_t n, gu8* out, uint32_t cap, uint32_t p, bool lz4, int lane) {
  uint32_t op;
  if (lz4) {
    op = lz4_emit_seq(out, 0u, cap, in, p, p, n - 5u - p, -1, 0u, lane);
    if (op == 0xffffffffu) return 0u;
    op = lz4_emit_tail(out, op, cap, in + 251u, 5u, lane);
    return op == 0xffffffffu ? 0u : op;
  }
  op = blz_emit_literals(out, 0u, cap, in, p, lane);
  if (op == 0xffffffffu) return 0u;
  op = blz_emit_match(out, op, cap, p, n - 2u - p, lane);
  if (op == 0xffffffffu) return 0u;
  op = blz_emit_literals(out, op, cap, in + 254u, 2u, lane);
  if (op == 0xffffffffu) return 0u;
  if (lane == 0) out[0] |= 0x20u;
  return op;
}
```

c-blosc_amd/csrc/engine.h:

```cpp
#pragma once
#include <hip/hip_runtime.h>
#include <stddef.h>
#include <stdint.h>

namespace bamd {

struct CompressParams {
  int clevel;
  int doshuffle;
  size_t typesize;
  int codec;
  int32_t forced_blocksize;
  int splitmode;
};

struct Job {
  const void* src;
  void* dst;
  size_t srcsize;
  size_t dstsize;
};

struct PackedBuffer {
  void* base;
  size_t size;
  size_t align;
  size_t* offsets;
};

struct CandidateSelect {
  const int* cand_first;
  int* choice;
  int* cand_results;
};
int engine_compress_batch(const CompressParams* params, bool per_chunk, int n, const Job* jobs, int* results, bool device_ptrs,
                          hipStream_t stream, const PackedBuffer* packed = nullptr, const CandidateSelect* select = nullptr);
int engine_decompress_batch(int n, const Job* jobs, int* results, bool device_ptrs, hipStream_t stream,
                            const PackedBuffer* packed = nullptr);
struct Header;
int engine_chunk_headers(int n, const void* const* src, Header* out, hipStream_t stream);
int engine_getitem(const void* src, int start, int nitems, void* dest, bool src_on_device, bool dst_on_device,
                   hipStream_t stream);
struct ItemRange { int chunk, start, nitems; void* dst; };
int engine_getitem_batch(int nchunks, const Job* chunks, int nranges, const ItemRange* ranges, int* results, hipStream_t stream,
                         const PackedBuffer* packed = nullptr);
void engine_getitem_pass_bytes(size_t bytes);
int engine_take(int nchunks, const Job* chunks, size_t row_bytes, size_t nidx, const int64_t* index, void* dest, int* status,
                int* chunk_rows_out, size_t* failed_out, hipStream_t stream);
int engine_put(int nchunks, const Job* chunks, size_t row_bytes, size_t nidx, const int64_t* index, const void* rows, const CompressParams* params,
               const PackedBuffer* out, int* cbytes_out, int* rewritten_out, int* status, int* chunk_rows_out, size_t* failed_out, hipStream_t stream);

int engine_checksum_batch(int kind, int n, const Job* runs, uint32_t* digests, hipStream_t stream);
void engine_checksum_tile_bytes(size_t bytes);

int engine_filter(int kind, size_t typesize, size_t blocksize, const void* src, void* dst);

int engine_persistent_grids(int cap, const char** names, int* launched, int* occupancy);
int engine_enc_lz_occupancy(int dynamic_lds);
void engine_last_compress_tasks(uint32_t out[3]);

int engine_set_device(int dev);
int engine_thread_device(int dev);
int engine_device_count();
void engine_release();
bool engine_is_device_pointer(const void* p);

void engine_prof_enable(int on);
void engine_prof_reset();
int engine_prof_get(const char* kernel, double* total_ms, int* launches);

}
```

c-blosc_amd/csrc/engine.hip:

```cpp
#include "engine.h"

#include <pthread.h>
#include <stdio.h>
#include <stdlib.h>
#include <string.h>

#include <map>
#include <atomic>
#include <mutex>
#include <string>
#include <vector>
#include <algorithm>

#include <chrono>
#include "blosc_format.h"
#include "dev_types.h"
#include "queue_order.h"

#include "k_filters.hip"
#include "k_decode.hip"
#include "k_encode.hip"
#include "k_zstd.hip"
#include "k_zstd2.hip"
#include "k_zlib.hip"
// ... 269 lines not shown
  }
}

static void atfork_prepare() { g_pick_mu.lock(); for (int i = 0; i < kMaxCtx; i++) g_ctx[i].mu.lock(); }
static void atfork_parent() { for (int i = kMaxCtx - 1; i >= 0; i--) g_ctx[i].mu.unlock(); g_pick_mu.unlock(); }
static void atfork_child() { for (int i = kMaxCtx - 1; i >= 0; i--) g_ctx[i].mu.unlock(); g_pick_mu.unlock(); g_forked = true; }

static int ensure_device(EngineState& st) {
  if (g_forked) {
    fprintf(stderr, "blosc_amd: this process was forked after the library had initialised its HIP device; a device context does not survive fork() - call exec() or use the library only in the parent\n");
    return -1;
  }
  static std::once_flag atfork_once;
  std::call_once(atfork_once, [] { (void)pthread_atfork(atfork_prepare, atfork_parent, atfork_child); });
  const int want_dev = wanted_device();
  if (st.device_ok && want_dev == st.device) { HIP_TRY(hipSetDevice(st.device)); return 0; }
  if (st.device_ok) {
    (void)hipSetDevice(st.device);
    st.dev.release(); st.io.release(); st.enc_tabs.drop(); st.dec_tabs.drop();
    if (st.own) { (void)hipStreamDestroy(st.own); st.own = nullptr; }
    for (auto& p : st.prof_pending) { (void)hipEventDestroy(p.a); (void)hipEventDestroy(p.b); }
    st.prof_pending.clear();
    for (hipEvent_t e : st.ev_pool) (void)hipEventDestroy(e);
    st.ev_pool.clear();
    st.device_ok = false;
  }
  st.device = want_dev;
  int cnt = 0;
  hipError_t e = hipGetDeviceCount(&cnt);
  if (e != hipSuccess || cnt <= 0) {
    if (!g_warned.exchange(true))
      fprintf(stderr, "blosc_amd: no usable HIP device (%s); this library has no CPU path\n",
              e == hipSuccess ? "device count 0" : hipGetErrorString(e));
    return -1;
  }
  if (st.device >= 0) HIP_TRY(hipSetDevice(st.device));
  else { HIP_TRY(hipGetDevice(&st.device)); int none = -1; (void)g_device.compare_exchange_strong(none, st.device); }
  probe_topology(st);
  hipDeviceProp_t pr;
  const bool have_props = hipGetDeviceProperties(&pr, st.device) == hipSuccess;
  st.cus = (have_props && pr.multiProcessorCount > 0) ? pr.multiProcessorCount : 256;
  if (!st.single_queue && !(have_props && (strncmp(pr.gcnArchName, "gfx950", 6) == 0 || strncmp(pr.gcnArchName, "gfx942", 6) == 0))) {
    st.single_queue = true;
    if (debug_enabled()) fprintf(stderr, "blosc_amd: %s is not on the allow-list of the relaxed in-kernel hand-off; using one task queue and unfused filters\n", have_props ? pr.gcnArchName : "(unknown device)");
  }
  query_persistent_grids(st.grid_wpc, st.grid_occupancy);
  st.enc_cost_valid = st.dec_cost_valid = false;
  st.device_ok = true;
  st.device_hint.store(st.device, std::memory_order_relaxed);
  return 0;
}

static hipEvent_t prof_event(EngineState& st) {
  if (!st.ev_pool.empty()) { hipEvent_t e = st.ev_pool.back(); st.ev_pool.pop_back(); return e; }
  hipEvent_t e; (void)hipEventCreate(&e); return e;
}
struct HostTime { double t[2][6] = {}; long calls[2] = {}; };
static HostTime g_ht;
static double now_ms() { return std::chrono::duration<double, std::milli>(std::chrono::steady_clock::now().time_since_epoch()).count(); }
static std::mutex g_ht_mu;
struct HostPhases {
  const int dir; double last = 0.0;
  explicit HostPhases(int dir_) : dir(dir_) { if (hosttime_on()) { last = now_ms(); std::lock_guard<std::mutex> l(g_ht_mu); g_ht.calls[dir]++; } }
  void mark(int i) {
    if (!hosttime_on()) return;
    const double t = now_ms();
    std::lock_guard<std::mutex> l(g_ht_mu);
    g_ht.t[dir][i] += t - last; last = t;
  }
};
struct ProfScope {
  EngineState& st; hipStream_t s; const char* name; hipEvent_t a{}, b{}; bool on;
  ProfScope(EngineState& st_, hipStream_t s_, const char* n) : st(st_), s(s_), name(n), on(g_prof.load(std::memory_order_relaxed)) {
    if (on) { a = prof_event(st); b = prof_event(st); (void)hipEventRecord(a, s); }
  }
  ~ProfScope() { if (on) { (void)hipEventRecord(b, s); st.prof_pending.push_back({name, a, b}); } }
};
static void prof_collect(EngineState& st) {
  for (auto& p : st.prof_pending) {
    float ms = 0;
    if (hipEventElapsedTime(&ms, p.a, p.b) == hipSuccess) { auto& e = st.prof_acc[p.name]; e.ms += ms; e.launches++; }
    st.ev_pool.push_back(p.a); st.ev_pool.push_back(p.b);
  }
  st.prof_pending.clear();
}

__global__ void k_gather_headers(const uint8_t* const* __restrict__ srcs, uint8_t* __restrict__ out, int n) {
  int i = blockIdx.x * blockDim.x + threadIdx.x;
  if (i >= n * 16) return;
  out[i] = srcs[i >> 4][i & 15];
}

static unsigned persistent_grid(const EngineState& st, size_t nitems, int waves_per_cu) {
  const int cus = st.cus > 0 ? st.cus : 256;
  size_t g = (size_t)cus * (size_t)waves_per_cu;
  if (nitems < g) g = nitems;
  return (unsigned)(g < 8 ? 8 : g);
}

static dim3 grid1(size_t n, int per) { return dim3((unsigned)((n + per - 1) / per)); }

static bool fused_typesize(int T) { return T >= 2 && T <= 32; }
static bool fused_fast_typesize(int T) { return T == 8 || T == 4 || T == 2 || T == 16; }
static bool bitunshuffle_fused_host(int T) { return T == 1 || T == 2 || T == 4 || T == 8; }

static void order_signature(const std::vector<BlockDesc>& blocks, const uint32_t* cost, bool valid, std::vector<int>& sig) {
  bool seen[257] = {false};
  for (const BlockDesc& b : blocks) seen[b.nstreams < 0 ? 0 : (b.nstreams > 256 ? 256 : b.nstreams)] = true;
  sig.clear();
  std::vector<int> order; int nheavy = 0;
  for (int T = 2; T <= 256; T++) {
    if (!seen[T]) continue;
    plane_order(cost, valid && sched_enabled(), T, order, &nheavy);
    std::sort(order.begin(), order.begin() + (nheavy < T ? nheavy : T));
    sig.push_back(T); sig.push_back(nheavy); sig.insert(sig.end(), order.begin(), order.begin() + (nheavy < T ? nheavy : 0));
  }
}

static int call_stream(EngineState& st, bool host_buffers, hipStream_t* stream) {
  if (!host_buffers || *stream != (hipStream_t)0 || ctx_count() == 1) return 0;
  if (!st.own) HIP_TRY(hipStreamCreateWithFlags(&st.own, hipStreamNonBlocking));
  *stream = st.own;
  return 0;
}

static int filter_tile_count(int32_t elems, int per_tile) { const int t = (elems + per_tile - 1) / per_tile; return t < 1 ? 1 : t; }

constexpr size_t kTicketGap = 32;
constexpr size_t kEncTicketWords = 16;
constexpr size_t kDecTicketWords = 8;
static size_t ticket_offset(size_t nchunks) { return sizeof(int32_t) * nchunks + kTicketGap; }

struct HostStaging {
  const bool host;
  size_t in_bytes = 0, out_bytes = 0, in_at = 0, out_at = 0;
  uint8_t *in_base = nullptr, *out_base = nullptr;
  void add(size_t in, size_t out) { if (host) { in_bytes = align_up(in_bytes, 256) + in; out_bytes = align_up(out_bytes, 256) + out; } }
  int reserve(DeviceArena& io) {
    if (!host) return 0;
    const size_t out_off = align_up(in_bytes + 256, 256);
    if (io.ensure(out_off + out_bytes + 512)) return -1;
    in_base = io.base; out_base = io.base + out_off; return 0;
  }
  int stage(ChunkDesc& c, const void* src, size_t in, size_t out, hipStream_t stream) {
    if (!host) return 0;
    in_at = align_up(in_at, 256); out_at = align_up(out_at, 256);
    HIP_TRY(hipMemcpyAsync(in_base + in_at, src, in, hipMemcpyHostToDevice, stream));
    c.src = in_base + in_at; c.dst = out_base + out_at;
    in_at += in; out_at += out; return 0;
  }
  int collect(int n, const Job* jobs, const std::vector<ChunkDesc>& chunks, const std::vector<uint8_t>& live, const int* results, hipStream_t stream) {
    if (!host) return 0;
    for (int i = 0; i < n; i++)
      if (live[(size_t)i] && results[i] > 0) HIP_TRY(hipMemcpyAsync(jobs[i].dst, chunks[(size_t)i].dst, (size_t)results[i], hipMemcpyDeviceToHost, stream));
    HIP_TRY(hipStreamSynchronize(stream));
    return 0;
  }
};

#ifdef BAMD_PROFILE_DECODE
struct StreamProfile {
  uint32_t* d = nullptr; std::string path; size_t bytes; hipStream_t stream;
  StreamProfile(const char* switch_name, size_t nrec, hipStream_t s, const char* suffix = "") : path(getenv(switch_name) ? getenv(switch_name) : ""), bytes(nrec * 64), stream(s) {
    if (!path.empty()) path += suffix;
    if (!path.empty() && bytes && hipMalloc((void**)&d, bytes) == hipSuccess) (void)hipMemsetAsync(d, 0, bytes, stream);
  }
  ~StreamProfile() {
    if (!d) return;
    std::vector<uint32_t> h(bytes / 4);
    (void)hipStreamSynchronize(stream); (void)hipMemcpy(h.data(), d, bytes, hipMemcpyDeviceToHost); (void)hipFree(d);
    FILE* f = fopen(path.c_str(), "wb");
    if (f) { fwrite(h.data(), 4, h.size(), f); fclose(f); }
  }
};
#define BAMD_STREAM_PROFILE(var, switch_name, nstr) StreamProfile var(switch_name, nstr, stream)
#define BAMD_WAVE_PROFILE(var, switch_name, nwaves) StreamProfile var(switch_name, nwaves, stream, ".waves")
#define BAMD_PROF_ARG(var) , var.d
#else
#define BAMD_STREAM_PROFILE(var, switch_name, nstr)
#define BAMD_WAVE_PROFILE(var, switch_name, nwaves)
#define BAMD_PROF_ARG(var)
#endif

struct EncVariant { int mode = kEncModes; int waves_per_cu = 0; };
static const char* enc_profile_name(int mode) {
  return kEncMode[mode].family == FAM_ZSTD ? "k_zstd_encode" : (kEncMode[mode].family == FAM_ZLIB ? "k_zlib_encode" : (kEncMode[mode].search ? "k_lz4hc_encode" : "k_encode_streams"));
}
constexpr int enc_mode_wanted(int family, bool search, bool tables, bool huffman, bool dynamic) {
  const bool zstd = family == FAM_ZSTD;
  const EncMode want = {nullptr, family, search, zstd && (tables || search), zstd && huffman && (tables || search), family == FAM_ZLIB && dynamic};
  int m = 0;
  while (m < kEncModes && !(kEncMode[m].family == want.family && kEncMode[m].search == want.search && kEncMode[m].tables == want.tables &&
                            kEncMode[m].huffman == want.huffman && kEncMode[m].dynamic == want.dynamic)) m++;
  return m;
}
constexpr int enc_modes_composed() {
  unsigned seen = 0;
  for (int s = 0; s < (FAM_ZLIB + 1) * 16; s++) {
    const int m = enc_mode_wanted(s >> 4, s & 1, s & 2, s & 4, s & 8);
    if (m == kEncModes) return -1;
    seen |= 1u << m;
  }
  return __builtin_popcount(seen);
}
static_assert(enc_modes_composed() == kEncModes, "every setting of the encoder switches has its row, and every row a setting");
static EncVariant encoder_variant(const EngineState& st, int codec, int clevel) {
  EncVariant v;
  const int family = codec == kZstd ? FAM_ZSTD : (codec == kZlib ? FAM_ZLIB : FAM_LZ);
  const bool search = family == FAM_ZSTD ? zstd_search_enabled(clevel) : (family == FAM_ZLIB ? zlib_search_enabled() : codec == kLZ4HC && lz4hc_search_enabled());
  v.mode = enc_mode_wanted(family, search, zstd_tables_enabled(), zstd_huffman_enabled(), zlib_dynamic_enabled());
  v.waves_per_cu = st.grid_wpc[v.mode];
  return v;
}

struct EncodeBatch {
  std::vector<ChunkDesc> chunks; std::vector<uint8_t> live;
  std::vector<uint8_t> variant;
  EncVariant variants[kEncModes]; bool present[kEncModes] = {false}; int ngroups = 0;
  EngineState::TableKey key;
  size_t nstr = 0, filt_bytes = 0, stage_bytes = 0;
  int tiles_shuf = 0, tiles_bit = 0; bool any_shuf = false, any_bit = false;
  explicit EncodeBatch(int n) : chunks((size_t)n), live((size_t)n, 0), variant((size_t)n, (uint8_t)kEncModes) {}
};

static bool add_encode_chunk(const CompressParams& p, const Job& job, int i, int n, bool may_fuse, EncodeBatch& B, int* result) {
  ChunkDesc& c = B.chunks[(size_t)i];
  std::vector<BlockDesc>& blocks = B.key.blocks;
  memset(&c, 0, sizeof c);
  c.mode = CH_SKIP;
  size_t nbytes = job.srcsize, destsize = job.dstsize, typesize = p.typesize;
  const int codec = p.codec;
  *result = 0;
  if (nbytes > (size_t)kMaxBufferSize || destsize < (size_t)kMaxOverhead) return false;
  if (destsize - kMaxOverhead > nbytes) destsize = nbytes + kMaxOverhead;
  if (p.clevel < 0 || p.clevel > 9 || (p.doshuffle != 0 && p.doshuffle != 1 && p.doshuffle != 2) || typesize == 0) { *result = -10; return false; }
  if (typesize > (size_t)kMaxTypeSize) typesize = 1;
  if (codec != kBloscLZ && codec != kLZ4 && codec != kLZ4HC && codec != kZlib && codec != kZstd) { *result = -5; return false; }
  const int32_t T = (int32_t)typesize, nb = (int32_t)nbytes;
  const int32_t bs = compute_blocksize(p.clevel, T, nb, p.forced_blocksize, codec, p.splitmode);
  const int32_t leftover = nb % bs, nblocks = nb / bs + (leftover > 0 ? 1 : 0);
  const bool memcpyed = (p.clevel == 0) || (nb < kMinBufferSize);
  const int split = split_block(codec, T, bs, p.splitmode);
  int flags = ((!split) << 4) | (codec_to_format(codec) << 5);
  if (memcpyed) flags |= kFlagMemcpyed;
  if (p.doshuffle == 1) flags |= kFlagShuffle;
  if (p.doshuffle == 2) flags |= kFlagBitShuffle;
  if (memcpyed && (size_t)nb + kMaxOverhead > destsize) return false;

  c.src = (const uint8_t*)job.src; c.dst = (uint8_t*)job.dst;
  c.nbytes = nb; c.cbytes = (int32_t)destsize; c.blocksize = bs; c.typesize = T;
  c.nblocks = nblocks; c.leftover = leftover; c.nsplits = split ? T : 1;
  c.fmt = codec_to_format(codec); c.clevel = (codec == kLZ4HC) ? 9 : p.clevel; c.hdr_flags = flags;
  c.mode = 0;
  c.first_block = (int32_t)blocks.size(); c.first_stream = (int32_t)B.nstr;
  if (memcpyed) c.mode |= CH_MEMCPYED;
  else if (p.doshuffle == 1 && T > 1) { c.mode |= CH_SHUFFLE; if (fused_typesize(T) && fuse_enabled() && may_fuse) c.mode |= CH_FUSED_SHUF; }
  else if (p.doshuffle == 2) { c.mode |= CH_BITSHUFFLE; if (bitunshuffle_fused_host(T) && fuse_enabled() && may_fuse) c.mode |= CH_FUSED_SHUF; }
  const bool filtered = (c.mode & (CH_SHUFFLE | CH_BITSHUFFLE)) != 0;
  if (filtered && !(c.mode & CH_FUSED_SHUF)) {
    if (c.mode & CH_SHUFFLE) { B.any_shuf = true; B.tiles_shuf = std::max(B.tiles_shuf, filter_tile_count(bs / T, shuffle_tile_elems(T))); }
    else { B.any_bit = true; B.tiles_bit = std::max(B.tiles_bit, filter_tile_count(bs / T, bitshuffle_tile_elems(T))); }
  }
  if (blocks.capacity() < blocks.size() + (size_t)nblocks) blocks.reserve(std::max(blocks.size() + (size_t)nblocks, (size_t)(n - i) * (size_t)nblocks + blocks.size()));
  for (int32_t j = 0; j < nblocks; j++) {
    BlockDesc b;
    b.chunk = i; b.blk = j; b.first_stream = (int32_t)B.nstr;
    const bool last = (j == nblocks - 1) && leftover > 0;
    b.nstreams = memcpyed ? 0 : ((split && !last) ? T : 1);
    b.bsize = last ? leftover : bs; b.flags = 0;
    B.nstr += (size_t)b.nstreams;
    blocks.push_back(b);
  }
  if (!memcpyed) {
    if (filtered) B.filt_bytes = align_up(B.filt_bytes, 256) + (size_t)nb;
    B.stage_bytes = align_up(B.stage_bytes, 256) + (size_t)nb;
  }
  return true;
}

int engine_persistent_grids(int cap, const char** names, int* launched, int* occupancy) {
  CtxGuard ctx; EngineState& st = *ctx.st;
  int wpc[kGridKernels], occ[kGridKernels];
  if (st.device_ok && wanted_device() == st.device) { memcpy(wpc, st.grid_wpc, sizeof wpc); memcpy(occ, st.grid_occupancy, sizeof occ); }
  else {
    const int dev = wanted_device();
    if (dev < 0 || hipSetDevice(dev) != hipSuccess) return -1;
    query_persistent_grids(wpc, occ);
  }
  for (int i = 0; i < kGridKernels && i < cap; i++) { names[i] = grid_kernels()[i].name; launched[i] = wpc[i]; occupancy[i] = occ[i]; }
  return kGridKernels;
}
int engine_enc_lz_occupancy(int dynamic_lds) {
#ifdef BAMD_WAVE_EMU
  return -1;
#else
  const int dev = wanted_device();
  int occ = -1;
  if (dev < 0 || hipSetDevice(dev) != hipSuccess) return -1;
  if (hipOccupancyMaxActiveBlocksPerMultiprocessor(&occ, grid_kernels()[ENC_LZ].fn, 64 * ENC_WAVES, (size_t)dynamic_lds) != hipSuccess) { (void)hipGetLastError(); return -1; }
  return occ;
#endif
}
static std::atomic<uint32_t> g_last_enc_tasks[3];
void engine_last_compress_tasks(uint32_t out[3]) { for (int i = 0; i < 3; i++) out[i] = g_last_enc_tasks[i].load(); }

struct SelectRun { int nchunks; const int* first; int* choice; int* answers; };

static int compress_entries_in(EngineState& st, const CompressParams* params, bool per_chunk, int n, const Job* jobs, int* results, bool device_ptrs,
                               hipStream_t stream, const PackedBuffer* packed, const SelectRun* sel) {
  if (n <= 0) return 0;
  if ((packed || sel) && !device_ptrs) return -1;
  if (ensure_device(st) || call_stream(st, !device_ptrs, &stream)) return -1;
  HostPhases ht(0);
  EncodeBatch B(n);
  HostStaging io{!device_ptrs};
  std::vector<ChunkDesc>& chunks = B.chunks;
  int8_t variant_of[6][10]; memset(variant_of, -1, sizeof variant_of);
  for (int i = 0; i < n; i++) {
    const CompressParams& p = params[per_chunk ? i : 0];
    B.live[(size_t)i] = add_encode_chunk(p, jobs[i], i, n, !st.single_queue, B, &results[i]);
    if (!B.live[(size_t)i]) continue;
    io.add((size_t)chunks[(size_t)i].nbytes, (size_t)chunks[(size_t)i].cbytes);
    if (chunks[(size_t)i].mode & CH_MEMCPYED) continue;
    int8_t& m = variant_of[p.codec][p.clevel];
    if (m < 0) { const EncVariant v = encoder_variant(st, p.codec, p.clevel); m = (int8_t)v.mode; B.variants[v.mode] = v; }
    B.variant[(size_t)i] = (uint8_t)m;
    if (!B.present[m]) { B.present[m] = true; B.ngroups++; }
  }
  const size_t nblk = B.key.blocks.size(), nstr = B.nstr;
  const bool feedback = B.ngroups <= 1;
  const bool cost_valid = feedback && st.enc_cost_valid;
  const size_t ngrp = (size_t)(B.ngroups > 0 ? B.ngroups : 1);
  ht.mark(0);
  EngineState::TableCache& tc = st.enc_tabs;
  B.key.nq = st.single_queue ? 1 : 8;
  B.key.modes.resize((size_t)n);
  for (int i = 0; i < n; i++) B.key.modes[(size_t)i] = (chunks[(size_t)i].mode & CH_FUSED_SHUF) | (B.variant[(size_t)i] < kEncModes ? (uint32_t)(B.variant[(size_t)i] + 1) << 8 : 0u);
  order_signature(B.key.blocks, st.enc_cost, cost_valid, B.key.order);
  Carver pc;
  if (tc.begin("compress", B.key, 0, 0, pc, [&](EngineState::TableCache& t) {
        t.groups.clear();
        std::vector<int32_t> q;
        for (int m = 0; m < kEncModes; m++) {
          if (!B.present[m]) continue;
          size_t sh_at = 0;
          build_encode_queues(B.key.blocks, chunks, st.enc_cost, cost_valid, q, B.key.nq, &sh_at, B.ngroups > 1 ? B.variant.data() : nullptr, m);
          t.groups.push_back({m, t.queues.size(), t.queues.size() + sh_at, q[8]});
          t.queues.insert(t.queues.end(), q.begin(), q.end());
        }
      })) return -1;
  Carver cv;
  const size_t o_chunks = cv.take(sizeof(ChunkDesc) * (size_t)n);
  const size_t o_streams = cv.take(sizeof(StreamDesc) * (nstr ? nstr : 1));
  const size_t o_blkoff = cv.take(sizeof(int32_t) * (nblk ? nblk : 1));
  const size_t sel_bytes = sel ? sizeof(int32_t) * ((size_t)sel->nchunks + (size_t)n) : 0;
  const size_t o_sel = cv.take(sel_bytes + ticket_offset((size_t)n) + sizeof(uint32_t) * kEncTicketWords * ngrp);
  const size_t o_results = o_sel + sel_bytes;
  const size_t o_ready = cv.take(sizeof(uint32_t) * (nblk ? nblk : 1));
  const size_t o_cost = cv.take(sizeof(uint32_t) * kCostWords * ngrp);
  const size_t clear_bytes = cv.off - o_results;
  const size_t o_filt = cv.take(B.filt_bytes + 256);
  const size_t o_stage = cv.take(B.stage_bytes + 256);
  const size_t p_chunks = pc.take(sizeof(ChunkDesc) * (size_t)n);
  const size_t p_results = pc.take(sel_bytes + sizeof(int32_t) * (size_t)n);
  const size_t p_first = sel ? pc.take(sizeof(int32_t) * ((size_t)sel->nchunks + 1 + (size_t)n)) : 0;
  const size_t p_cost = pc.take(sizeof(uint32_t) * kCostWords * ngrp);
  const size_t p_offsets = packed ? pc.take(sizeof(uint64_t) * ((size_t)n + 1)) : 0;
  struct GroupRun { const EngineState::EncGroup* g; EncVariant v; size_t o_ctabs, o_seqbufs, o_ticket, o_cost, p_cost; };
  std::vector<GroupRun> runs;
  for (size_t k = 0; k < tc.groups.size(); k++) {
    GroupRun r{&tc.groups[k], B.variants[tc.groups[k].mode], 0, 0, o_results + ticket_offset((size_t)n) + sizeof(uint32_t) * kEncTicketWords * k,
               o_cost + sizeof(uint32_t) * kCostWords * k, p_cost + sizeof(uint32_t) * kCostWords * k};
    const size_t zwaves = (size_t)(st.cus > 0 ? st.cus : 256) * (size_t)r.v.waves_per_cu;
    if (kEncMode[r.v.mode].family == FAM_ZSTD) r.o_ctabs = cv.take(sizeof(zenc::CTabs) + 64);
    if (enc_seq_words(r.v.mode)) r.o_seqbufs = cv.take(zwaves * enc_seq_words(r.v.mode) * sizeof(uint64_t) + 64);
    runs.push_back(r);
  }
  const size_t o_offsets = (packed || sel) ? cv.take(sizeof(uint64_t) * ((size_t)n + 1)) : 0;
  const size_t o_first = sel ? cv.take(sizeof(int32_t) * ((size_t)sel->nchunks + 1)) : 0;
  if (st.dev.ensure(cv.off)) return -1;
  uint8_t* D = st.dev.base;
  for (const GroupRun& r : runs) {
    if (!r.o_ctabs) continue;
    static const zenc::CTabs host_tabs = [] { zenc::CTabs t; zenc::build_predefined(t); return t; }();
    HIP_TRY(hipMemcpyAsync(D + r.o_ctabs, &host_tabs, sizeof host_tabs, hipMemcpyHostToDevice, stream));
  }
  if (io.reserve(st.io)) return -1;
  {
    size_t fo = 0, so = 0;
    for (int i = 0; i < n; i++) {
      if (!B.live[(size_t)i]) continue;
      ChunkDesc& c = chunks[(size_t)i];
      if (io.stage(c, jobs[i].src, (size_t)c.nbytes, (size_t)c.cbytes, stream)) return -1;
      if (c.mode & CH_MEMCPYED) continue;
      const bool filtered = (c.mode & (CH_SHUFFLE | CH_BITSHUFFLE)) != 0;
      if (filtered) { fo = align_up(fo, 256); c.filt = D + o_filt + fo; fo += (size_t)c.nbytes; }
      so = align_up(so, 256); c.stage = D + o_stage + so; so += (size_t)c.nbytes;
    }
  }
  ht.mark(1);
  if (st.pin.ensure(pc.off)) return -1;
  uint8_t* P = st.pin.base;
  memcpy(P + p_chunks, chunks.data(), sizeof(ChunkDesc) * (size_t)n);
  if (tc.upload(B.key, P, stream)) return -1;
  HIP_TRY(hipMemsetAsync(D + o_results, 0, clear_bytes, stream));
  HIP_TRY(hipMemcpyAsync(D + o_chunks, P + p_chunks, sizeof(ChunkDesc) * (size_t)n, hipMemcpyHostToDevice, stream));
  if (sel) {
    const size_t first_bytes = sizeof(int32_t) * ((size_t)sel->nchunks + 1);
    memcpy(P + p_first, sel->first, first_bytes);
    memcpy(P + p_first + first_bytes, results, sizeof(int32_t) * (size_t)n);
    HIP_TRY(hipMemcpyAsync(D + o_first, P + p_first, first_bytes, hipMemcpyHostToDevice, stream));
    HIP_TRY(hipMemcpyAsync(D + o_results, P + p_first + first_bytes, sizeof(int32_t) * (size_t)n, hipMemcpyHostToDevice, stream));
  }

  ChunkDesc* d_chunks = (ChunkDesc*)(D + o_chunks); BlockDesc* d_blocks = tc.d_blocks(); StreamDesc* d_streams = (StreamDesc*)(D + o_streams);
  int32_t* d_blkoff = (int32_t*)(D + o_blkoff); int32_t* d_results = (int32_t*)(D + o_results);
  ht.mark(2);
  if (nstr) hipLaunchKernelGGL(k_encode_plan, grid1(nblk, 256), dim3(256), 0, stream, d_chunks, d_blocks, d_streams, (int)nblk);
  if (B.any_shuf && nblk) {
    ProfScope ps(st, stream, "k_shuffle");
    hipLaunchKernelGGL(k_shuffle, dim3((unsigned)nblk, (unsigned)B.tiles_shuf), dim3(FT_THREADS), 0, stream, d_chunks, d_blocks);
  }
  if (B.any_bit && nblk) {
    ProfScope ps(st, stream, "k_bitshuffle");
    hipLaunchKernelGGL(k_bitfilter_fast<0>, dim3((unsigned)nblk, (unsigned)B.tiles_bit), dim3(FT_THREADS), 0, stream, d_chunks, d_blocks);
    hipLaunchKernelGGL(k_bitshuffle, dim3((unsigned)nblk, (unsigned)B.tiles_bit), dim3(FT_THREADS), 0, stream, d_chunks, d_blocks, 1);
  }
  for (const GroupRun& r : runs) {
    const EngineState::EncGroup& g = *r.g;
    if (!nstr || g.ntasks <= 0) continue;
    ProfScope ps(st, stream, enc_profile_name(r.v.mode));
    const int32_t* d_qoff = tc.d_qoff() + g.q_at; const int32_t* d_qlist = d_qoff + 9; const int32_t* d_shoff = tc.d_qoff() + g.sh_at;
    uint32_t* d_ticket = (uint32_t*)(D + r.o_ticket);
    uint32_t* d_cost = (uint32_t*)(D + r.o_cost);
    uint32_t* d_ready = (uint32_t*)(D + o_ready);
    uint64_t* d_seqbufs = r.o_seqbufs ? (uint64_t*)(D + r.o_seqbufs) : nullptr;
    const zenc::CTabs* d_ctabs = r.o_ctabs ? (const zenc::CTabs*)(D + r.o_ctabs) : nullptr;
    const int detect = (kEncMode[r.v.mode].family == FAM_LZ && periodic_enabled()) ? 1 : 0;
    const dim3 grid(persistent_grid(st, (size_t)g.ntasks, r.v.waves_per_cu)), block(64 * ENC_WAVES);
    BAMD_STREAM_PROFILE(prof, "BLOSC_AMD_ENC_PROFILE", nstr);
    BAMD_WAVE_PROFILE(wprof, "BLOSC_AMD_ENC_PROFILE", grid.x);
    hipLaunchKernelGGL(enc_kernel(r.v.mode), grid, block, 0, stream, d_streams, d_ticket, d_qlist, d_qoff, d_shoff, d_chunks, d_blocks, d_ready, d_cost, st.single_queue ? 1 : 0, d_seqbufs, d_ctabs, detect BAMD_PROF_ARG(prof) BAMD_PROF_ARG(wprof));
  }
  if (!packed && !sel) {
    ProfScope ps(st, stream, "k_chunk_scan");
    hipLaunchKernelGGL(k_chunk_scan, dim3((unsigned)n), dim3(SCAN_THREADS), 0, stream, d_chunks, d_blocks, d_streams, d_blkoff, d_results);
  } else {
    uint64_t* d_offsets = (uint64_t*)(D + o_offsets);
    {
      ProfScope ps(st, stream, "k_chunk_scan");
      hipLaunchKernelGGL(k_chunk_scan_packed, dim3((unsigned)n), dim3(SCAN_THREADS), 0, stream, d_chunks, d_blocks, d_streams, d_blkoff, d_results);
    }
    if (sel) {
      ProfScope ps(st, stream, "k_candidate_select");
      hipLaunchKernelGGL(k_candidate_select, dim3((unsigned)sel->nchunks), dim3(SELECT_THREADS), 0, stream, d_chunks, d_results, (const int32_t*)(D + o_first),
                         (int32_t*)(D + o_sel) + sel->nchunks, (int32_t*)(D + o_sel));
    }
    if (packed) {
      ProfScope ps(st, stream, "k_packed_layout");
      hipLaunchKernelGGL(k_packed_layout, dim3(1), dim3(SCAN_THREADS), 0, stream, d_chunks, d_results, n, (uint8_t*)packed->base, (uint64_t)packed->size,
                         (uint64_t)packed->align, d_offsets);
      hipLaunchKernelGGL(k_packed_headers, dim3((unsigned)n), dim3(SCAN_THREADS), 0, stream, d_chunks, d_blkoff, d_results, d_offsets, (uint64_t)packed->size);
    } else {
      HIP_TRY(hipMemsetAsync(d_offsets, 0, sizeof(uint64_t) * ((size_t)n + 1), stream));
      hipLaunchKernelGGL(k_packed_headers, dim3((unsigned)n), dim3(SCAN_THREADS), 0, stream, d_chunks, d_blkoff, d_results, d_offsets, (uint64_t)0);
    }
  }
  if (nblk) {
    ProfScope ps(st, stream, "k_chunk_compact");
    hipLaunchKernelGGL(k_chunk_compact, dim3((unsigned)nblk), dim3(COMPACT_THREADS), 0, stream, d_chunks, d_blocks, d_streams, d_blkoff);
  }
  HIP_TRY(hipGetLastError());
  HIP_TRY(hipMemcpyAsync(P + p_results, D + o_sel, sel_bytes + sizeof(int32_t) * (size_t)n, hipMemcpyDeviceToHost, stream));
  HIP_TRY(hipMemcpyAsync(P + p_cost, D + o_cost, sizeof(uint32_t) * kCostWords * ngrp, hipMemcpyDeviceToHost, stream));
  if (packed) HIP_TRY(hipMemcpyAsync(P + p_offsets, D + o_offsets, sizeof(uint64_t) * ((size_t)n + 1), hipMemcpyDeviceToHost, stream));
  ht.mark(3);
  HIP_TRY(hipStreamSynchronize(stream));
  ht.mark(4);
  prof_collect(st);
  uint32_t taken = 0, nshuf = 0;
  for (const GroupRun& r : runs) {
    if (!nstr) break;
    const uint32_t* cost = (const uint32_t*)(P + r.p_cost);
    if (check_done(cost, (size_t)r.g->ntasks, 0, "compress")) return -1;
    taken += cost[256];
    nshuf += (uint32_t)tc.queues[r.g->sh_at + 8];
  }
  if (packed) for (int i = 0; i <= n; i++) packed->offsets[i] = (size_t)((const uint64_t*)(P + p_offsets))[i];
  if (nstr) { g_last_enc_tasks[0] = taken; g_last_enc_tasks[1] = (uint32_t)nstr; g_last_enc_tasks[2] = nshuf; }
  tc.commit(B.key);
  if (feedback && nstr >= 4096) { memcpy(st.enc_cost, P + p_cost, sizeof st.enc_cost); st.enc_cost_valid = true; }
  const int32_t* r = (const int32_t*)(P + p_results + sel_bytes);
  for (int i = 0; i < n; i++) if (B.live[(size_t)i]) results[i] = r[i];
  if (sel) {
    memcpy(sel->choice, P + p_results, sizeof(int32_t) * (size_t)sel->nchunks);
    memcpy(sel->answers, P + p_results + sizeof(int32_t) * (size_t)sel->nchunks, sizeof(int32_t) * (size_t)n);
  }
  return io.collect(n, jobs, chunks, B.live, results, stream);
}

static int compress_entries(const CompressParams* params, bool per_chunk, int n, const Job* jobs, int* results, bool device_ptrs,
                            hipStream_t stream, const PackedBuffer* packed, const SelectRun* sel) {
  if (n <= 0) return 0;
  if ((packed || sel) && !device_ptrs) return -1;
  CtxGuard ctx;
  return compress_entries_in(*ctx.st, params, per_chunk, n, jobs, results, device_ptrs, stream, packed, sel);
}

int engine_compress_batch(const CompressParams* params, bool per_chunk, int n, const Job* jobs, int* results, bool device_ptrs,
                          hipStream_t stream, const PackedBuffer* packed, const CandidateSelect* select) {
  if (!select) return compress_entries(params, per_chunk, n, jobs, results, device_ptrs, stream, packed, nullptr);
  if (n <= 0) return 0;
  if (!device_ptrs || !per_chunk) return -1;
  const int* first = select->cand_first;
  const int E = first[n];
  std::vector<Job> entries((size_t)E);
  for (int i = 0; i < n; i++) for (int e = first[i]; e < first[i + 1]; e++) entries[(size_t)e] = jobs[i];
  std::vector<int> sizes((size_t)E, 0), answers((size_t)E, 0), choice((size_t)n, -1);
  std::vector<size_t> offsets((size_t)E + 1, 0);
  PackedBuffer pk{};
  if (packed) { pk = *packed; pk.offsets = offsets.data(); }
  const SelectRun run{n, first, choice.data(), answers.data()};
  if (compress_entries(params, true, E, entries.data(), sizes.data(), true, stream, packed ? &pk : nullptr, &run)) return -1;
  for (int i = 0; i < n; i++) {
    const int f = first[i], c = choice[(size_t)i];
    results[i] = f == first[i + 1] ? -10 : (c >= 0 ? sizes[(size_t)(f + c)] : answers[(size_t)f]);
    select->choice[i] = c;
    if (packed) packed->offsets[i] = offsets[(size_t)f];
  }
  if (packed) packed->offsets[n] = offsets[(size_t)E];
  if (select->cand_results && E > 0) memcpy(select->cand_results, answers.data(), sizeof(int) * (size_t)E);
  return 0;
}

static int classify_for_decompress(const Header& h, size_t srcsize, size_t destsize, int* res, int* fmt) {
  if (h.nbytes == 0) { *res = 0; return 0; }
  if (h.blocksize <= 0 || (size_t)h.blocksize > destsize || h.blocksize > kMaxBlockSize || h.typesize <= 0) { *res = -1; return 0; }
  if (h.version != kVersionFormat) { *res = -1; return 0; }
  if (h.flags & kFlagReserved) { *res = -1; return 0; }
  const bool neg = h.nbytes < 0;
  if (!neg && (size_t)h.nbytes > destsize) { *res = -1; return 0; }
  if (srcsize && (h.cbytes < 0 || (size_t)h.cbytes > srcsize)) { *res = -1; return 0; }
  if (h.flags & kFlagMemcpyed) {
    if ((int32_t)((uint32_t)h.nbytes + (uint32_t)kMaxOverhead) != h.cbytes) { *res = -1; return 0; }
    *fmt = 0;
    if (neg) { *res = 0; return 0; }
    return 1;
  }
  const int f = (h.flags & 0xe0) >> 5;
  if (f != FMT_BLOSCLZ && f != FMT_LZ4 && f != FMT_ZLIB && f != FMT_ZSTD) { *res = -5; return 0; }
  if (h.versionlz != 1) { *res = -9; return 0; }
  *fmt = f;
  int32_t nblocks = h.nbytes / h.blocksize + ((h.nbytes % h.blocksize) > 0 ? 1 : 0);
  if (nblocks > (h.cbytes - 16) / 4) { *res = -1; return 0; }
  if (neg) { *res = 0; return 0; }
  return 1;
}

static int fetch_headers(EngineState& st, int n, const Job* jobs, bool device_ptrs, hipStream_t stream,
                         std::vector<Header>& hdrs) {
  hdrs.resize((size_t)n);
  if (!device_ptrs) {
    for (int i = 0; i < n; i++) hdrs[(size_t)i] = parse_header((const uint8_t*)jobs[i].src);
    return 0;
  }
  if (st.dev.ensure(16)) return -1;
  Carver cv;
  const size_t o_ptrs = cv.take(sizeof(void*) * (size_t)n);
  const size_t o_hdr = cv.take(16 * (size_t)n);
  if (st.pin.ensure(cv.off)) return -1;
  const void** pp = (const void**)(st.pin.base + o_ptrs);
  bool any_short = false;
  for (int i = 0; i < n; i++) { const bool sh = jobs[i].srcsize && jobs[i].srcsize < (size_t)kMaxOverhead; any_short |= sh; pp[i] = sh ? (const void*)st.dev.base : jobs[i].src; }
  if (any_short) HIP_TRY(hipMemsetAsync(st.dev.base, 0, 16, stream));
  hipLaunchKernelGGL(k_gather_headers, grid1((size_t)n * 16, 256), dim3(256), 0, stream,
                     (const uint8_t* const*)(st.pin.base + o_ptrs), st.pin.base + o_hdr, n);
  HIP_TRY(hipGetLastError());
  HIP_TRY(hipStreamSynchronize(stream));
  for (int i = 0; i < n; i++) hdrs[(size_t)i] = parse_header(st.pin.base + o_hdr + 16 * (size_t)i);
  for (int i = 0; i < n; i++) if (jobs[i].srcsize && jobs[i].srcsize < (size_t)kMaxOverhead) { hdrs[(size_t)i] = Header{}; hdrs[(size_t)i].nbytes = -1; hdrs[(size_t)i].version = -1; }
  return 0;
}

static void add_decode_chunk(const Header& h, int fmt, int chunk_index, int32_t j0, int32_t j1,
                             ChunkDesc& c, std::vector<BlockDesc>& blocks, size_t& nstreams) {
  memset(&c, 0, sizeof c);
  const int32_t T = h.typesize, bs = h.blocksize;
  c.nbytes = h.nbytes; c.cbytes = h.cbytes; c.blocksize = bs; c.typesize = T;
  c.nblocks = h.nbytes / bs + ((h.nbytes % bs) ? 1 : 0);
  c.leftover = h.nbytes % bs;
  c.fmt = fmt;
  const bool dont_split = (h.flags & kFlagDontSplit) != 0;
  const bool split = !dont_split && T <= kMaxSplits && bs / T >= kMinBufferSize;
  c.nsplits = split ? T : 1;
  c.mode = 0;
  if (h.flags & kFlagMemcpyed) c.mode |= CH_MEMCPYED;
  else if ((h.flags & kFlagShuffle) && T > 1) c.mode |= CH_SHUFFLE;
  else if (h.flags & kFlagBitShuffle) c.mode |= CH_BITSHUFFLE;
  c.first_block = (int32_t)blocks.size();
  c.first_stream = (int32_t)nstreams;
  if (c.mode & CH_MEMCPYED) return;
  for (int32_t j = j0; j < j1; j++) {
    BlockDesc b;
    b.chunk = chunk_index; b.blk = j; b.first_stream = (int32_t)nstreams;
    const bool last = (j == c.nblocks - 1) && c.leftover > 0;
    b.nstreams = (split && !last) ? T : 1;
    b.bsize = last ? c.leftover : bs; b.flags = fmt == FMT_ZSTD ? BLK_Z : (fmt == FMT_ZLIB ? (BLK_Z | BLK_ZLIB) : 0);
    nstreams += (size_t)b.nstreams;
    blocks.push_back(b);
  }
}

struct DecodeLaunch {
  ChunkDesc* d_chunks; BlockDesc* d_blocks; StreamDesc* d_streams; int32_t* d_status; uint32_t* d_ticket; uint32_t* d_blkdone;
  size_t clear_bytes;
  uint32_t* d_spans; uint8_t* d_pat;
  uint32_t* d_cost;
  uint32_t* d_zticket; bool any_zstd;
  bool any_zlib;
  const int32_t* d_zqlist; const int32_t* d_zqoff; size_t nstr_zlib;
  ZMeta* d_zmeta; ptrdiff_t zseq_delta;
  ZgLds* d_zgscr;
  ZcTab* d_zctab;
  const int32_t* d_qlist; const int32_t* d_qoff;
  size_t nblk, nstr; int nchunks;
  bool any_shuf, any_bit, any_copy; int tiles_shuf, tiles_bit;
  size_t nstr_queued;
};

struct DecodeShape {
  int nchunks; size_t nblk, nstr;
  size_t filt_bytes;
  size_t zlit_bytes;
  bool any_zstd, two_phase;
  size_t out_bytes = 0;
  size_t extra_bytes = 0;
};
struct DecodeAreas { uint8_t *filt, *zlit, *out, *extra; };
static int decode_workspace(EngineState& st, const DecodeShape& s, DecodeLaunch& L, DecodeAreas& A) {
  const size_t n = (size_t)s.nchunks, nblk1 = s.nblk ? s.nblk : 1, nstr1 = s.nstr ? s.nstr : 1;
  const int zstd2 = (s.any_zstd && s.two_phase) ? zstd2_mode() : 0;
  const bool use_zctab = zstd2 == 2 && BAMD_ZSTD_SEQ_KERNEL && !BAMD_ZSTD_LDS_FSE;
  Carver cv;
  const size_t o_chunks = cv.take(sizeof(ChunkDesc) * n);
  const size_t o_streams = cv.take(sizeof(StreamDesc) * nstr1);
  const size_t o_blkdone = ticket_offset(n) + sizeof(uint32_t) * kDecTicketWords;
  const size_t o_status = cv.take(o_blkdone + sizeof(uint32_t) * nblk1);
  const size_t o_cost = cv.take(sizeof(uint32_t) * kCostWords);
  L.clear_bytes = cv.off - o_status;
  const size_t o_spans = cv.take(8 * nstr1);
  const size_t o_pat = cv.take(span_enabled() ? (size_t)2048 * nstr1 : 256);
  const size_t o_filt = cv.take(s.filt_bytes + 256);
  const size_t o_zlit = cv.take(s.zlit_bytes + 256);
  const size_t o_zseq = cv.take(s.zlit_bytes + 512);
  const size_t o_zmeta = cv.take(s.any_zstd && s.two_phase ? sizeof(ZMeta) * nstr1 : 64);
  const size_t o_zticket = cv.take(64);
  const size_t o_zgscr = cv.take(zstd2 == 2 ? sizeof(ZgLds) * nstr1 : 64);
  const size_t o_zctab = cv.take(use_zctab ? sizeof(ZcTab) * nstr1 : 64);
  const size_t o_out = cv.take(s.out_bytes ? s.out_bytes + 256 : 0);
  const size_t o_extra = cv.take(s.extra_bytes);
  if (st.dev.ensure(cv.off)) return -1;
  uint8_t* D = st.dev.base;
  A = DecodeAreas{D + o_filt, D + o_zlit, D + o_out, D + o_extra};
  L.d_chunks = (ChunkDesc*)(D + o_chunks); L.d_streams = (StreamDesc*)(D + o_streams);
  L.d_status = (int32_t*)(D + o_status);
  L.d_ticket = (uint32_t*)(D + o_status + ticket_offset(n));
  L.d_blkdone = (uint32_t*)(D + o_status + o_blkdone);
  L.d_cost = (uint32_t*)(D + o_cost);
  L.d_spans = span_enabled() ? (uint32_t*)(D + o_spans) : nullptr; L.d_pat = D + o_pat;
  L.d_zticket = (uint32_t*)(D + o_zticket);
  L.d_zmeta = (s.any_zstd && s.two_phase) ? (ZMeta*)(D + o_zmeta) : nullptr; L.zseq_delta = (ptrdiff_t)o_zseq - (ptrdiff_t)o_zlit + 8;
  L.d_zgscr = zstd2 == 2 ? (ZgLds*)(D + o_zgscr) : nullptr;
  L.d_zctab = use_zctab ? (ZcTab*)(D + o_zctab) : nullptr;
  L.nblk = s.nblk; L.nstr = s.nstr; L.nchunks = s.nchunks;
  return 0;
}
static int clear_decode_counters(const DecodeLaunch& L, hipStream_t stream) {
  HIP_TRY(hipMemsetAsync(L.d_status, 0, L.clear_bytes, stream));
  if (L.any_zstd || L.any_zlib) HIP_TRY(hipMemsetAsync(L.d_zticket, 0, 64, stream));
  return 0;
}

static int read_back_decode(const DecodeLaunch& L, void* status, void* cost, hipStream_t stream) {
  HIP_TRY(hipMemcpyAsync(status, L.d_status, sizeof(int32_t) * (size_t)L.nchunks, hipMemcpyDeviceToHost, stream));
  HIP_TRY(hipMemcpyAsync(cost, L.d_cost, sizeof(uint32_t) * kCostWords, hipMemcpyDeviceToHost, stream));
  return 0;
}
static int decode_feedback(EngineState& st, const DecodeLaunch& L, const void* cost, const char* what) {
  if (check_done((const uint32_t*)cost, L.nstr_queued, L.any_zstd ? L.nstr : 0, what, L.nstr_zlib)) return -1;
  if (L.nstr >= 4096) { memcpy(st.dec_cost, cost, sizeof st.dec_cost); st.dec_cost_valid = true; }
  return 0;
}

static int launch_decode(EngineState& st, const DecodeLaunch& L, hipStream_t stream) {
  if (L.nblk) {
    {
      ProfScope ps(st, stream, "k_decode_plan");
      hipLaunchKernelGGL(k_decode_plan, grid1(L.nblk, 256), dim3(256), 0, stream, L.d_chunks, L.d_blocks, L.d_streams, L.d_status, (int)L.nblk);
    }
    if (L.nstr_queued) {
      ProfScope ps(st, stream, "k_decode_streams");
      const dim3 dgrid(persistent_grid(st, L.nstr_queued ? L.nstr_queued : 1, st.grid_wpc[GRID_DECODE]));
      BAMD_STREAM_PROFILE(prof, "BLOSC_AMD_DEC_PROFILE", L.nstr);
      hipLaunchKernelGGL(k_decode_streams, dgrid, dim3(64 * DEC_WAVES), 0, stream, L.d_streams, L.d_status, L.d_ticket, L.d_qlist, L.d_qoff, L.d_chunks, L.d_blocks, L.d_blkdone, L.d_spans, L.d_pat, L.d_cost, st.single_queue ? 1 : 0 BAMD_PROF_ARG(prof));
    }
    const int zstd2 = zstd2_mode();
    const uint32_t* d_taken = nullptr;
    if (L.any_zstd && L.d_zmeta && zstd2) {
      {
        ProfScope ps(st, stream, "k_zstd_entropy");
        if (zstd2 == 2 && L.d_zgscr) hipLaunchKernelGGL(k_zstd_entropy_t<true>, grid1(L.nstr, ZG_FRAMES), dim3(64), 0, stream, L.d_streams, (int)L.nstr, L.d_chunks, L.d_blocks, L.d_zmeta, L.zseq_delta, L.d_zgscr, L.d_zctab);
        else hipLaunchKernelGGL(k_zstd_entropy_t<false>, grid1(L.nstr, ZG_FRAMES), dim3(64), 0, stream, L.d_streams, (int)L.nstr, L.d_chunks, L.d_blocks, L.d_zmeta, L.zseq_delta, (ZgLds*)nullptr, (ZcTab*)nullptr);
      }
      if (zstd2 == 2 && L.d_zgscr && BAMD_ZSTD_SEQ_KERNEL && !BAMD_ZSTD_LDS_FSE) {
        ProfScope ps(st, stream, "k_zstd_seq");
        hipLaunchKernelGGL(k_zstd_seq, grid1(L.nstr, ZSEQ_FRAMES), dim3(64), 0, stream, L.d_streams, (int)L.nstr, L.d_chunks, L.d_blocks, L.d_zmeta, L.zseq_delta, L.d_zgscr, L.d_zctab);
      }
      {
        ProfScope ps(st, stream, "k_zstd_exec");
        hipLaunchKernelGGL(k_zstd_exec, dim3(persistent_grid(st, L.nstr, st.grid_wpc[GRID_ZSTD_EXEC])), dim3(64), 0, stream, L.d_streams, (int)L.nstr, L.d_status, L.d_zticket + 1,
                           L.d_chunks, L.d_blocks, L.d_zmeta, L.zseq_delta);
      }
      d_taken = (const uint32_t*)L.d_zmeta;
    }
    if (L.any_zstd) {
      ProfScope ps(st, stream, "k_zstd_streams");
      BAMD_STREAM_PROFILE(zprof, "BLOSC_AMD_ZSTD_PROFILE", L.nstr);
      hipLaunchKernelGGL(k_zstd_streams, dim3(persistent_grid(st, L.nstr, st.grid_wpc[GRID_ZSTD_STREAMS])), dim3(64), 0, stream, L.d_streams, (int)L.nstr, L.d_status,
                         L.d_zticket, L.d_chunks, L.d_blocks, L.d_cost + 257, d_taken BAMD_PROF_ARG(zprof));
    }
    if (L.any_zlib) {
      ProfScope ps(st, stream, "k_zlib_streams");
      hipLaunchKernelGGL(k_zlib_streams, dim3(persistent_grid(st, L.nstr_zlib ? L.nstr_zlib : 1, st.grid_wpc[GRID_ZLIB_STREAMS])), dim3(64), 0, stream, L.d_streams, L.d_status,
                         L.d_zticket + 8, L.d_zqlist, L.d_zqoff, L.d_cost + 259, L.d_chunks, L.d_blocks, L.d_blkdone, st.single_queue ? 1 : 0);
    }
    if (L.any_shuf) {
      ProfScope ps(st, stream, "k_unshuffle");
      hipLaunchKernelGGL(k_unshuffle, dim3((unsigned)L.nblk, (unsigned)L.tiles_shuf), dim3(FT_THREADS), 0, stream, L.d_chunks, L.d_blocks);
    }
    if (L.any_bit) {
      ProfScope ps(st, stream, "k_bitunshuffle");
// ... 924 lines not shown
```

c-blosc_amd/csrc/k_encode.hip:

```cpp
#include <hip/hip_runtime.h>
#include <stdint.h>
#include "dev_types.h"
#include "wave_prims.h"
#include "zstd_enc.h"
#include "deflate_enc.h"

namespace bamd {

#ifdef BAMD_PROFILE_DECODE
#define EPROF_ARG , DecProf& prof_
#define EPROF_PASS , prof_
#else
#define EPROF_ARG
#define EPROF_PASS
#endif

#include "enc_lz.h"
#include "enc_lz4p.h"
#include "enc_zstd.h"
#include "enc_zlib.h"
#include "enc_shuffle.h"

enum { FAM_LZ, FAM_ZSTD, FAM_ZLIB };
struct EncMode { const char* name; int family; bool search, tables, huffman, dynamic; };
#define BAMD_ENC_MODES(ROW) \
  ROW(ENC_LZ,          FAM_LZ,   false, false, false, false) \
  ROW(ENC_ZSTD,        FAM_ZSTD, false, false, false, false) \
  ROW(ENC_ZLIB,        FAM_ZLIB, false, false, false, false) \
  ROW(ENC_HC,          FAM_LZ,   true,  false, false, false) \
  ROW(ENC_ZSTD_T,      FAM_ZSTD, false, true,  false, false) \
  ROW(ENC_ZSTD_HC,     FAM_ZSTD, true,  true,  false, false) \
  ROW(ENC_ZLIB_HC,     FAM_ZLIB, true,  false, false, false) \
  ROW(ENC_ZSTD_TH,     FAM_ZSTD, false, true,  true,  false) \
  ROW(ENC_ZSTD_HCH,    FAM_ZSTD, true,  true,  true,  false) \
  ROW(ENC_ZLIB_DYN,    FAM_ZLIB, false, false, false, true)  \
  ROW(ENC_ZLIB_DYN_HC, FAM_ZLIB, true,  false, false, true)
#define BAMD_ENC_ENUMERATOR(NAME, ...) NAME,
#define BAMD_ENC_ROW(NAME, ...) {"k_encode_streams_t<" #NAME ">", __VA_ARGS__},
enum { BAMD_ENC_MODES(BAMD_ENC_ENUMERATOR) kEncModes };
constexpr EncMode kEncMode[kEncModes] = {BAMD_ENC_MODES(BAMD_ENC_ROW)};
#undef BAMD_ENC_ENUMERATOR
#undef BAMD_ENC_ROW
constexpr uint32_t enc_seq_words(int mode) { return kEncMode[mode].family == FAM_ZSTD ? ZS_SEQCAP : (kEncMode[mode].dynamic ? ZD_SCRATCH_U64 : 0u); }
#ifndef BAMD_ENC_HELP
#define BAMD_ENC_HELP 256
#endif
template <int MODE>
__device__ __attribute__((noinline)) void encode_one_stream(StreamDesc* sd_, enc_entry_t* tab_, const ChunkDesc* chunks_, uint32_t* blk_ready_, int lane,
                                                            const BlockDesc* blocks_, uint32_t sid_, uint32_t* plane_cost_, uint64_t* seqbuf_
#ifdef BAMD_PROFILE_DECODE
                                                            , uint32_t* profslot_
#endif
                                                            ) {
  StreamDesc* sd; enc_entry_t* tab; const ChunkDesc* chunks; uint32_t* blk_ready; const BlockDesc* blocks; uint32_t sid; uint32_t* plane_cost; uint64_t* seqbuf;
#ifdef BAMD_PROFILE_DECODE
  uint32_t* profslot;
#endif
  PROF_DECL
#ifdef BAMD_PROFILE_DECODE
  prof_.c[4] = 0; prof_.c[5] = 0;
#endif
  sd = uni_gp(sd_); tab = uni_gp(tab_); chunks = uni_gp(chunks_); blk_ready = uni_gp(blk_ready_); blocks = uni_gp(blocks_);
  plane_cost = uni_gp(plane_cost_); seqbuf = uni_gp(seqbuf_); sid = uni(sid_);
#ifdef BAMD_PROFILE_DECODE
  profslot = uni_gp(profslot_);
#endif
  const uint32_t n = uni((uint32_t)sd->in_size), cap = uni((uint32_t)sd->out_size);
  const uint32_t aux = uni((uint32_t)sd->aux);
  const int clevel = (int)(aux & 15u);
  if (uni(chunks[uni((uint32_t)sd->chunk)].mode) & CH_FUSED_SHUF) {
    const uint32_t gb = aux >> 4;
    while (__hip_atomic_load(&blk_ready[gb], __ATOMIC_RELAXED, __HIP_MEMORY_SCOPE_AGENT) == 0u) __builtin_amdgcn_s_sleep(16);
    __builtin_amdgcn_fence(__ATOMIC_ACQUIRE, "agent");
  }
  PROF_LAP(13);
  const uint64_t cost_t0 = __builtin_amdgcn_s_memtime();
  uint32_t r;
  const int32_t hint = (int32_t)uni((uint32_t)sd->result);
  constexpr EncMode M = kEncMode[MODE];
  if (M.family == FAM_ZSTD) r = seqbuf ? zstd_encode_wave<M.tables, M.search, M.huffman>(uni_ptr(as_global(sd->in)), n, uni_ptr(as_global(sd->out)), cap, clevel, tab, (BAMD_GAS uint64_t*)seqbuf, lane EPROF_PASS) : 0u;
  else if (M.dynamic) r = seqbuf ? zlib_dyn_encode_wave<M.search>(uni_ptr(as_global(sd->in)), n, uni_ptr(as_global(sd->out)), cap, clevel, tab, (BAMD_GAS uint64_t*)seqbuf, lane EPROF_PASS) : 0u;
  else if (M.family == FAM_ZLIB) r = zlib_encode_wave<M.search>(uni_ptr(as_global(sd->in)), n, uni_ptr(as_global(sd->out)), cap, clevel, tab, lane EPROF_PASS);
  else if (hint < 0) r = emit_periodic_stream(uni_ptr(as_global(sd->in)), n, uni_ptr(as_global(sd->out)), cap, (uint32_t)-hint, uni((uint32_t)sd->fmt) == (uint32_t)FMT_LZ4, lane);
  else if (M.search) r = lz4hc_encode_wave(uni_ptr(as_global(sd->in)), n, uni_ptr(as_global(sd->out)), cap, tab, lane);
  else if (sd->fmt == FMT_LZ4) r = BAMD_ENC_PAR ? lz4_encode_wave_auto(uni_ptr(as_global(sd->in)), n, uni_ptr(as_global(sd->out)), cap, clevel, tab, lane EPROF_PASS)
                                                : lz_encode_wave<EF_LZ4>(uni_ptr(as_global(sd->in)), n, uni_ptr(as_global(sd->out)), cap, clevel, tab, lane EPROF_PASS);
  else r = lz_encode_wave<EF_BLOSCLZ>(uni_ptr(as_global(sd->in)), n, uni_ptr(as_global(sd->out)), cap, clevel, tab, lane EPROF_PASS);
  if (lane == 0) sd->result = (int32_t)r;
  if (plane_cost && lane == 0) {
    const uint32_t j = sid - (uint32_t)blocks[aux >> 4].first_stream;
    atomicAdd(plane_cost + (j & 255u), (uint32_t)((__builtin_amdgcn_s_memtime() - cost_t0) >> 10));
  }
#ifdef BAMD_PROFILE_DECODE
  prof_.c[15] = (uint32_t)__builtin_amdgcn_s_memrealtime();
  if (lane == 0 && profslot) for (int i_ = 0; i_ < 16; i_++) profslot[i_] = prof_.c[i_];
#endif
}

constexpr int enc_tab_bytes(int mode) { return kEncMode[mode].search ? HC_TAB_BYTES : ENC_TAB_BYTES; }
constexpr int enc_writer_lds_bytes(int mode) { return kEncMode[mode].family == FAM_ZSTD ? ZS_LDS_BYTES : (kEncMode[mode].family == FAM_ZLIB ? DFL_LDS_BYTES : (mode == ENC_LZ ? ENC_SCR_BYTES : 0)); }
constexpr int enc_lds_bytes(int mode) { return enc_tab_bytes(mode) + enc_writer_lds_bytes(mode); }
constexpr int enc_min_waves(int mode) { return kEncMode[mode].search ? 2 : (kEncMode[mode].tables ? 5 : (mode == ENC_LZ ? BAMD_ENC_LZ_MINWAVES : BAMD_ENC_MINWAVES)); }
constexpr int enc_grid_bound(int mode) { return lds_workgroups_per_cu(enc_lds_bytes(mode)) < 32 ? lds_workgroups_per_cu(enc_lds_bytes(mode)) : 32; }
template <int MODE>
__global__ __launch_bounds__(64 * ENC_WAVES, enc_min_waves(MODE)) void k_encode_streams_t(
    StreamDesc* __restrict__ streams, uint32_t* __restrict__ tickets , const int32_t* __restrict__ qlist,
    const int32_t* __restrict__ qoff , const int32_t* __restrict__ shoff , const ChunkDesc* __restrict__ chunks, const BlockDesc* __restrict__ blocks,
    uint32_t* __restrict__ blk_ready, uint32_t* __restrict__ plane_cost, int single_queue,
    uint64_t* __restrict__ seqbufs, const zenc::CTabs* __restrict__ ctabs, int detect_periodic
#ifdef BAMD_PROFILE_DECODE
    , uint32_t* __restrict__ profbuf, uint32_t* __restrict__ profwave
#endif
    ) {
#ifdef BAMD_PROFILE_DECODE
  const uint64_t wt_entry = __builtin_amdgcn_s_memtime(), wr_entry = __builtin_amdgcn_s_memrealtime();
  uint64_t wt_stream = 0, wt_shuffle = 0, wt_wait = 0, wt_wait_first = 0;
  uint32_t wn_stream = 0, wn_shuffle = 0;
#define WPROF_BEGIN(t) const uint64_t t = __builtin_amdgcn_s_memtime()
#define WPROF_END(acc, t) acc += __builtin_amdgcn_s_memtime() - t
#else
#define WPROF_BEGIN(t)
#define WPROF_END(acc, t)
#endif
  constexpr bool ZSTD = kEncMode[MODE].family == FAM_ZSTD;
  constexpr uint32_t SEQWORDS = enc_seq_words(MODE);
  constexpr int TABBYTES = enc_tab_bytes(MODE);
  __shared__ __attribute__((aligned(16))) enc_entry_t tabs[ENC_WAVES][lds_occupied(enc_lds_bytes(MODE)) / 4];
  static_assert(ENC_WAVES == 1, "one stream per wave, one wave per workgroup");
  const int lane = threadIdx.x & 63;
  if (ZSTD) {
    const uint32_t* g = (const uint32_t*)ctabs;
    for (uint32_t k = (uint32_t)lane; k < sizeof(zenc::CTabs) / 4u; k += 64u) tabs[0][TABBYTES / 4 + k] = g[k];
  }
  uint64_t* seqbuf = SEQWORDS ? seqbufs + (size_t)blockIdx.x * SEQWORDS : nullptr;
  const uint32_t xcc = single_queue ? 0u : (__builtin_amdgcn_s_getreg((3 << 11) | 20) & 7u);
  const uint32_t qbase = (uint32_t)qoff[xcc], qlen = (uint32_t)qoff[xcc + 1] - qbase;
  const uint32_t shbase = (uint32_t)shoff[xcc], shlen = (uint32_t)shoff[xcc + 1] - shbase;
  const int32_t* shlist = shoff + 9;
  auto shuffle_one = [&]() -> bool {
    const uint32_t s = take_ticket(tickets + 8 + xcc, lane);
    if (s >= shlen) return false;
    WPROF_BEGIN(ts_);
    shuffle_block_task(chunks, blocks, uni((uint32_t)shlist[shbase + s]), blk_ready, streams, detect_periodic, lane, (volatile uint32_t*)tabs[0]);
    WPROF_END(wt_shuffle, ts_);
#ifdef BAMD_PROFILE_DECODE
    wn_shuffle++;
#endif
    return true;
  };
  uint32_t t = take_ticket(tickets + xcc, lane);
  uint32_t ndone = 0;
  while (t < qlen) {
    const int32_t task = (int32_t)uni((uint32_t)qlist[qbase + t]);
    if (task < 0) {
      shuffle_one();
    } else {
      const StreamDesc* sd = streams + task;
      if (uni(chunks[uni((uint32_t)sd->chunk)].mode) & CH_FUSED_SHUF) {
        const uint32_t gb = uni((uint32_t)sd->aux) >> 4;
        const ChunkDesc* cd = chunks + uni((uint32_t)sd->chunk);
        bool more = !(uni(cd->mode) & CH_BITSHUFFLE) && shuffle_generic_T(uni((uint32_t)cd->typesize));
#ifdef BAMD_PROFILE_DECODE
        const uint64_t tw_ = __builtin_amdgcn_s_memtime(), sh0_ = wt_shuffle;
#endif
        while (__hip_atomic_load(&blk_ready[gb], __ATOMIC_RELAXED, __HIP_MEMORY_SCOPE_AGENT) == 0u) {
          if (BAMD_ENC_HELP && more && __hip_atomic_load(tickets + 8 + xcc, __ATOMIC_RELAXED, __HIP_MEMORY_SCOPE_AGENT) < (single_queue ? gb : gb / 8u) + (uint32_t)BAMD_ENC_HELP) more = shuffle_one();
          else __builtin_amdgcn_s_sleep(16);
        }
#ifdef BAMD_PROFILE_DECODE
        wt_wait += (__builtin_amdgcn_s_memtime() - tw_) - (wt_shuffle - sh0_);
        if (wn_stream == 0) wt_wait_first = wt_wait;
#endif
      }
#ifdef BAMD_PROFILE_DECODE
      const uint64_t te_ = __builtin_amdgcn_s_memtime();
      encode_one_stream<MODE>(streams + task, tabs[0], chunks, blk_ready, lane, blocks, (uint32_t)task, plane_cost, seqbuf, profbuf ? profbuf + (size_t)task * 16 : nullptr);
      wt_stream += __builtin_amdgcn_s_memtime() - te_; wn_stream++;
#else
      encode_one_stream<MODE>(streams + task, tabs[0], chunks, blk_ready, lane, blocks, (uint32_t)task, plane_cost, seqbuf);
#endif
    }
    ndone++;
    t = take_ticket(tickets + xcc, lane);
  }
  if (lane == 0 && ndone) atomicAdd(plane_cost + 256, ndone);
#ifdef BAMD_PROFILE_DECODE
  if (lane == 0 && profwave) {
    uint32_t* w = profwave + (size_t)blockIdx.x * 16;
    const uint64_t wt_exit = __builtin_amdgcn_s_memtime(), wr_exit = __builtin_amdgcn_s_memrealtime();
    w[0] = (uint32_t)wr_entry; w[1] = (uint32_t)(wr_entry >> 32); w[2] = (uint32_t)wr_exit; w[3] = (uint32_t)(wr_exit >> 32);
    w[4] = (uint32_t)wt_stream; w[5] = (uint32_t)wt_shuffle; w[6] = (uint32_t)wt_wait; w[7] = ndone; w[8] = wn_stream; w[9] = wn_shuffle; w[10] = xcc;
    w[11] = 1u;
    w[12] = (uint32_t)(wt_exit - wt_entry); w[13] = (uint32_t)wt_wait_first;
  }
#endif
#undef WPROF_BEGIN
#undef WPROF_END
}

__global__ __launch_bounds__(256) void k_encode_plan(const ChunkDesc* __restrict__ chunks, const BlockDesc* __restrict__ blocks,
                                                     StreamDesc* __restrict__ streams, int nblocks_total) {
  const int g = (int)(blockIdx.x * blockDim.x + threadIdx.x);
  if (g >= nblocks_total) return;
  const BlockDesc b = blocks[g];
  if (b.nstreams <= 0) return;
  const ChunkDesc& c = chunks[b.chunk];
  const uint8_t* inbase = (c.mode & (CH_SHUFFLE | CH_BITSHUFFLE)) ? c.filt : c.src;
  const int32_t neblock = b.bsize / b.nstreams;
  const size_t at = (size_t)b.blk * (size_t)c.blocksize;
  for (int32_t k = 0; k < b.nstreams; k++) {
    StreamDesc sd;
    sd.in = inbase + at + (size_t)k * (size_t)neblock;
    sd.out = c.stage + at + (size_t)k * (size_t)neblock;
    sd.in_size = neblock; sd.out_size = neblock; sd.chunk = b.chunk; sd.fmt = c.fmt; sd.aux = c.clevel | (int32_t)((uint32_t)g << 4); sd.result = 0;
    streams[(size_t)b.first_stream + k] = sd;
  }
}

constexpr int SCAN_THREADS = 256;

__device__ __forceinline__ void st_i32(gu8* p, int32_t v) { g_st_i32le(p, v); }

template <bool PACKED>
__device__ __forceinline__ void chunk_scan(ChunkDesc* __restrict__ chunks,
                                           const BlockDesc* __restrict__ blocks,
                                           const StreamDesc* __restrict__ streams,
                                           int32_t* __restrict__ blk_off,
                                           int32_t* __restrict__ results) {
  __shared__ int32_t part[SCAN_THREADS];
  __shared__ int32_t carry_s;
  const int cid = blockIdx.x, tid = threadIdx.x;
  ChunkDesc& c = chunks[cid];
  if (c.mode & CH_SKIP) return;
  gu8* d = as_global(c.dst);
  if (c.mode & CH_MEMCPYED) {
    if (tid == 0) {
      if (!PACKED) {
        d[0] = 2; d[1] = 1; d[2] = (uint8_t)c.hdr_flags; d[3] = (uint8_t)c.typesize;
        st_i32(d + 4, c.nbytes); st_i32(d + 8, c.blocksize); st_i32(d + 12, c.nbytes + 16);
      }
      results[cid] = c.nbytes + 16;
    }
    return;
  }
  if (tid == 0) carry_s = 16 + 4 * c.nblocks;
  __syncthreads();
  for (int base = 0; base < c.nblocks; base += SCAN_THREADS) {
    const int j = base + tid;
    int32_t mine = 0;
    if (j < c.nblocks) {
      const BlockDesc b = blocks[c.first_block + j];
      for (int s = 0; s < b.nstreams; s++) {
        const StreamDesc& sd = streams[b.first_stream + s];
        mine += 4 + (sd.result > 0 ? sd.result : sd.in_size);
      }
    }
    part[tid] = mine;
    __syncthreads();
    for (int o = 1; o < SCAN_THREADS; o <<= 1) {
      int32_t v = (tid >= o) ? part[tid - o] : 0;
      __syncthreads();
      part[tid] += v;
      __syncthreads();
    }
    const int32_t carry = carry_s;
    if (j < c.nblocks) {
      int64_t start = (int64_t)carry + part[tid] - mine;
      blk_off[c.first_block + j] = start > 0x7fffffff ? 0x7fffffff : (int32_t)start;
    }
    __syncthreads();
    if (tid == SCAN_THREADS - 1) {
      int64_t nc = (int64_t)carry + part[tid];
      carry_s = nc > 0x7fffffff ? 0x7fffffff : (int32_t)nc;
    }
    __syncthreads();
  }
  const int32_t total = carry_s;
  const int32_t maxbytes = c.cbytes;
  int32_t res;
  uint32_t flags = (uint32_t)c.hdr_flags;
  if (total <= maxbytes) {
    res = total;
    if (!PACKED) for (int j = tid; j < c.nblocks; j += SCAN_THREADS) st_i32(d + 16 + 4 * (size_t)j, blk_off[c.first_block + j]);
  } else if ((int64_t)c.nbytes + 16 <= (int64_t)maxbytes) {
    res = c.nbytes + 16;
    flags |= 0x2u;
    if (tid == 0) c.mode |= CH_MEMCPYED;
  } else {
    res = 0;
    if (tid == 0) c.mode |= CH_SKIP;
  }
  if (tid == 0) {
    if (!PACKED) {
      d[0] = 2;
      d[1] = 1;
      d[2] = (uint8_t)flags; d[3] = (uint8_t)c.typesize;
      st_i32(d + 4, c.nbytes); st_i32(d + 8, c.blocksize); st_i32(d + 12, res);
    }
    results[cid] = res;
  }
}
__global__ __launch_bounds__(SCAN_THREADS) void k_chunk_scan(ChunkDesc* __restrict__ chunks, const BlockDesc* __restrict__ blocks,
                                                            const StreamDesc* __restrict__ streams, int32_t* __restrict__ blk_off,
                                                            int32_t* __restrict__ results) {
  chunk_scan<false>(chunks, blocks, streams, blk_off, results);
}
__global__ __launch_bounds__(SCAN_THREADS) void k_chunk_scan_packed(ChunkDesc* __restrict__ chunks, const BlockDesc* __restrict__ blocks,
                                                                   const StreamDesc* __restrict__ streams, int32_t* __restrict__ blk_off,
                                                                   int32_t* __restrict__ results) {
  chunk_scan<true>(chunks, blocks, streams, blk_off, results);
}

constexpr int SELECT_THREADS = 64;
__global__ __launch_bounds__(SELECT_THREADS) void k_candidate_select(ChunkDesc* __restrict__ chunks, int32_t* __restrict__ results,
                                                                    const int32_t* __restrict__ first,
                                                                    int32_t* __restrict__ answers,
                                                                    int32_t* __restrict__ choice) {
  const int i = blockIdx.x, lane = threadIdx.x;
  const int32_t e0 = first[i], e1 = first[i + 1];
  uint64_t best = ~0ull;
  for (int32_t e = e0 + lane; e < e1; e += SELECT_THREADS) {
    const int32_t r = results[e];
    answers[e] = r;
    if (r > 0 && !(chunks[e].mode & CH_SKIP)) {
      const uint64_t key = ((uint64_t)(uint32_t)r << 32) | (uint32_t)e;
      best = key < best ? key : best;
    }
  }
  best = wave_min_u64(best);
  const int32_t winner = (uint32_t)(best >> 32) != 0xffffffffu ? (int32_t)(uint32_t)best : -1;
  for (int32_t e = e0 + lane; e < e1; e += SELECT_THREADS)
    if (e != winner) { chunks[e].mode |= CH_SKIP; results[e] = 0; }
  if (lane == 0) choice[i] = winner >= 0 ? winner - e0 : -1;
}

__global__ __launch_bounds__(SCAN_THREADS) void k_packed_layout(ChunkDesc* __restrict__ chunks, int32_t* __restrict__ results, int nchunks,
                                                               uint8_t* dest, uint64_t destsize, uint64_t align ,
                                                               uint64_t* __restrict__ offsets) {
  __shared__ uint64_t part[SCAN_THREADS];
  __shared__ uint64_t carry_s;
  const int tid = threadIdx.x;
  if (tid == 0) carry_s = 0;
  __syncthreads();
  for (int base = 0; base < nchunks; base += SCAN_THREADS) {
    const int i = base + tid;
    uint64_t size = 0, mine = 0;
    if (i < nchunks) {
      const int32_t r = results[i];
      size = r > 0 ? (uint64_t)r : 0;
      mine = (size + align - 1) & ~(align - 1);
    }
    part[tid] = mine;
    __syncthreads();
    for (int o = 1; o < SCAN_THREADS; o <<= 1) {
      uint64_t v = (tid >= o) ? part[tid - o] : 0;
      __syncthreads();
      part[tid] += v;
      __syncthreads();
    }
    const uint64_t carry = carry_s;
    if (i < nchunks) {
      const uint64_t off = carry + part[tid] - mine;
      offsets[i] = off;
      ChunkDesc& c = chunks[i];
      if (!(c.mode & CH_SKIP)) {
        if (off + size <= destsize) c.dst = dest + off;
        else { c.mode |= CH_SKIP; results[i] = 0; }
      }
    }
    __syncthreads();
    if (tid == SCAN_THREADS - 1) carry_s = carry + part[tid];
    __syncthreads();
  }
  if (tid == 0) offsets[nchunks] = carry_s;
}

__global__ __launch_bounds__(SCAN_THREADS) void k_packed_headers(const ChunkDesc* __restrict__ chunks, const int32_t* __restrict__ blk_off,
                                                                const int32_t* __restrict__ results, const uint64_t* __restrict__ offsets,
                                                                uint64_t destsize) {
  const int cid = blockIdx.x, tid = threadIdx.x;
  const ChunkDesc& c = chunks[cid];
  if (c.mode & CH_SKIP) return;
  gu8* d = as_global(c.dst);
  const int32_t res = results[cid];
  const bool memcpyed = (c.mode & CH_MEMCPYED) != 0;
  if (!memcpyed) for (int j = tid; j < c.nblocks; j += SCAN_THREADS) st_i32(d + 16 + 4 * (size_t)j, blk_off[c.first_block + j]);
  if (tid == 0) {
    d[0] = 2; d[1] = 1; d[2] = (uint8_t)((uint32_t)c.hdr_flags | (memcpyed ? 0x2u : 0u)); d[3] = (uint8_t)c.typesize;
    st_i32(d + 4, c.nbytes); st_i32(d + 8, c.blocksize); st_i32(d + 12, res);
  }
  const uint64_t next = offsets[cid + 1] < destsize ? offsets[cid + 1] : destsize;
  for (uint64_t k = offsets[cid] + (uint64_t)res + (uint64_t)tid; k < next; k += SCAN_THREADS) d[k - offsets[cid]] = 0;
}

constexpr int COMPACT_THREADS = 256;

__device__ __forceinline__ void wg_copy(gu8* dst, const gu8* src, uint32_t n) {
  const uint32_t tid = threadIdx.x;
  uint32_t full = n & ~15u;
  for (uint32_t k = tid * 16u; k < full; k += COMPACT_THREADS * 16u) st16u(dst + k, ld16u(src + k));
  for (uint32_t k = full + tid; k < n; k += COMPACT_THREADS) dst[k] = src[k];
}

__global__ __launch_bounds__(COMPACT_THREADS) void k_chunk_compact(const ChunkDesc* __restrict__ chunks,
                                                                  const BlockDesc* __restrict__ blocks,
                                                                  const StreamDesc* __restrict__ streams,
                                                                  const int32_t* __restrict__ blk_off) {
  const BlockDesc b = blocks[blockIdx.x];
  const ChunkDesc& c = chunks[b.chunk];
  if (c.mode & CH_SKIP) return;
  const uint32_t bsize = (uint32_t)b.bsize;
  if (c.mode & CH_MEMCPYED) {
    wg_copy(as_global(c.dst) + 16 + (size_t)b.blk * c.blocksize, as_global(c.src) + (size_t)b.blk * c.blocksize, bsize);
    return;
  }
  uint32_t pos = (uint32_t)blk_off[blockIdx.x];
  for (int s = 0; s < b.nstreams; s++) {
    const StreamDesc& sd = streams[b.first_stream + s];
    const bool raw = sd.result <= 0;
    const uint32_t sz = raw ? (uint32_t)sd.in_size : (uint32_t)sd.result;
    if (threadIdx.x == 0) st_i32(as_global(c.dst) + pos, (int32_t)sz);
    wg_copy(as_global(c.dst) + pos + 4, as_global(raw ? sd.in : (const uint8_t*)sd.out), sz);
    pos += 4u + sz;
  }
}

__global__ __launch_bounds__(COMPACT_THREADS) void k_copy_chunks(const ChunkDesc* __restrict__ chunks, int src_skip) {
  const ChunkDesc& c = chunks[blockIdx.y];
  if (!(c.mode & CH_MEMCPYED) || (c.mode & CH_SKIP)) return;
  const uint64_t per = (uint64_t)COMPACT_THREADS * 16u * 8u;
  for (uint64_t lo = (uint64_t)blockIdx.x * per; lo < (uint64_t)c.nbytes; lo += (uint64_t)gridDim.x * per) {
    uint64_t hi = lo + per < (uint64_t)c.nbytes ? lo + per : (uint64_t)c.nbytes;
    wg_copy(as_global(c.dst) + lo, as_global(c.src) + src_skip + lo, (uint32_t)(hi - lo));
  }
}

}
```

Measured before the change: 813.8 GB/s.

## Stream shuffled segments to LZ4 encoders before the whole block finishes

```diff
diff --git a/c-blosc_amd/csrc/blosc_api.hip b/c-blosc_amd/csrc/blosc_api.hip
--- a/c-blosc_amd/csrc/blosc_api.hip
+++ b/c-blosc_amd/csrc/blosc_api.hip
@@ -615,6 +615,7 @@
 }
 __attribute__((visibility("default"))) int blosc_internal_enc_lz_occupancy(int dynamic_lds) { return bamd::engine_enc_lz_occupancy(dynamic_lds); }
 __attribute__((visibility("default"))) void blosc_internal_last_compress_tasks(unsigned out[3]) { bamd::engine_last_compress_tasks(out); }
+__attribute__((visibility("default"))) int blosc_internal_enc_feed(int mode) { return bamd::engine_enc_feed(mode); }
 
 __attribute__((visibility("default"))) void blosc_internal_shuffle(const size_t typesize, const size_t blocksize,
                                                                    const uint8_t* src, const uint8_t* dest) {
diff --git a/c-blosc_amd/csrc/enc_lz.h b/c-blosc_amd/csrc/enc_lz.h
--- a/c-blosc_amd/csrc/enc_lz.h
+++ b/c-blosc_amd/csrc/enc_lz.h
@@ -28,6 +28,37 @@
 constexpr int ENC_LZ_LDS_WAVES = lds_workgroups_per_cu(ENC_TAB_BYTES + ENC_LZ_SCR_BYTES);
 constexpr int ENC_LZ_WAVES_PER_CU = ENC_LZ_LDS_WAVES < 4 * BAMD_ENC_LZ_MINWAVES ? ENC_LZ_LDS_WAVES : 4 * BAMD_ENC_LZ_MINWAVES;
 static_assert(lds_occupied(ENC_TAB_BYTES + ENC_LZ_SCR_BYTES) * ENC_LZ_WAVES_PER_CU <= LDS_BYTES_PER_CU, "the LZ4 kernel's workgroups of one CU fit its LDS");
+
+#ifndef BAMD_ENC_FEED_SEGMENTS
+#define BAMD_ENC_FEED_SEGMENTS 8
+#endif
+constexpr int ENC_FLAG_DETECT = 1, ENC_FLAG_FEED = 2;
+struct FeedWord {
+  static constexpr uint32_t DONE = 1u << 31;
+  static constexpr uint32_t SEG_SHIFT = 16u, SEG_MASK = 0x7fffu, NONPER_MASK = 0xffffu;
+  static constexpr uint32_t make(uint32_t segments, uint32_t nonper) { return (segments << SEG_SHIFT) | (nonper & NONPER_MASK); }
+  static constexpr uint32_t segments(uint32_t w) { return (w >> SEG_SHIFT) & SEG_MASK; }
+  static constexpr uint32_t nonper(uint32_t w) { return w & NONPER_MASK; }
+  static constexpr bool done(uint32_t w) { return (w & DONE) != 0u; }
+};
+static_assert(BAMD_ENC_FEED_SEGMENTS >= 1 && (uint32_t)BAMD_ENC_FEED_SEGMENTS <= FeedWord::SEG_MASK, "the segment count fits its field of the word");
+__device__ __forceinline__ uint32_t feed_seg_bytes(uint32_t N) {
+  const uint32_t groups = N >> 10 ? N >> 10 : 1u, g = groups < (uint32_t)BAMD_ENC_FEED_SEGMENTS ? groups : (uint32_t)BAMD_ENC_FEED_SEGMENTS;
+  return ((groups + g - 1u) / g) << 10;
+}
+__device__ __forceinline__ bool feed_geometry(uint32_t nstreams, uint32_t T, uint32_t N, uint32_t bsize) {
+  return nstreams == T && N * T == bsize && (N & 255u) == 0u && N >= 1024u;
+}
+__device__ __forceinline__ uint32_t feed_avail(uint32_t w, uint32_t n, uint32_t seg_bytes) {
+  if (FeedWord::done(w)) return n;
+  const uint64_t a = (uint64_t)FeedWord::segments(w) * seg_bytes;
+  return a < n ? (uint32_t)a : n;
+}
+__device__ __forceinline__ bool feed_may_start(uint32_t w, uint32_t j) { return j < 16u && ((w >> j) & 1u) != 0u && FeedWord::segments(w) >= 1u; }
+#ifdef BAMD_WAVE_EMU
+inline void (*g_emu_feed_published)(uint32_t word) = nullptr;
+inline void (*g_emu_feed_poll)() = nullptr;
+#endif
 
 struct EncTable {
   __attribute__((address_space(3))) uint32_t* w;
diff --git a/c-blosc_amd/csrc/enc_lz4p.h b/c-blosc_amd/csrc/enc_lz4p.h
--- a/c-blosc_amd/csrc/enc_lz4p.h
+++ b/c-blosc_amd/csrc/enc_lz4p.h
@@ -75,9 +75,9 @@
   return maxlen;
 }
 
-template <int SS>
-__device__ uint32_t lz4_encode_wave_par(const gu8* __restrict__ src, uint32_t n, gu8* __restrict__ dst, uint32_t cap,
-                                        int clevel, enc_entry_t* tab_generic, int lane_in EPROF_ARG) {
+template <int SS, bool FEED>
+__device__ uint64_t lz4_encode_wave_fed(const gu8* __restrict__ src, uint32_t n, gu8* __restrict__ dst, uint32_t cap,
+                                        int clevel, enc_entry_t* tab_generic, int lane_in EPROF_ARG, uint32_t* fword) {
   static_assert(SS == 0 || SS == 1, "one or two positions per lane");
   const int lane = lane_in;
   constexpr uint32_t SPAN = 64u << SS;
@@ -89,6 +89,22 @@
   const uint32_t mlimit = n - 5u;
   const int accel = 10 - clevel;
   const uint32_t minlen = clevel >= 9 ? 4u : (clevel >= 6 ? 5u : 7u);
+  uint32_t avail = n, fwaited = 0;
+  auto feed_wait = [&](uint32_t need) {
+    const uint64_t t0 = __builtin_amdgcn_s_memtime();
+    for (;;) {
+#ifdef BAMD_WAVE_EMU
+      if (lane_in == 0 && g_emu_feed_poll) g_emu_feed_poll();
+#endif
+      avail = feed_avail(uni(__hip_atomic_load(fword, __ATOMIC_RELAXED, __HIP_MEMORY_SCOPE_AGENT)), n, feed_seg_bytes(n));
+      if (avail >= need) break;
+      __builtin_amdgcn_s_sleep(16);
+    }
+    __builtin_amdgcn_fence(__ATOMIC_ACQUIRE, "agent");
+    fwaited += (uint32_t)(__builtin_amdgcn_s_memtime() - t0);
+  };
+#define PAR_RETURN(v) return (uint64_t)(uint32_t)(v) | ((uint64_t)(FEED ? fwaited : 0u) << 32)
+  if (FEED) { avail = 0u; feed_wait(n < 1024u ? n : 1024u); }
   tab.clear(lane);
   EncWindow win;
   win.init(src, n, lane);
@@ -103,6 +119,10 @@
     const uint32_t p = ip + lq;
     const bool live = p <= last_start;
     const bool live1 = SS && p + 1u <= last_start;
+    if (FEED && __builtin_expect(avail < n, 0)) {
+      const uint32_t need = umin32((uni(ip) & ~255u) + 1024u, n);
+      if (avail < need) feed_wait(need);
+    }
     win.seek(ip, lane);
     const uint32_t lo = ip >= 4u ? ip - 4u : 0u;
     const uint32_t rb = lo & ~3u;
@@ -228,8 +248,16 @@
       uint32_t mext = 0;
       if (L_last >= RANK_CAP && pm_last + RANK_CAP < mlimit) {
         const uint32_t c_last = (uint32_t)__builtin_amdgcn_readlane((int)cand_r, (int)last);
-        mext = BAMD_ENC_EXT2 ? wave_common_fwd(src, n, pm_last + RANK_CAP, c_last + RANK_CAP, mlimit - (pm_last + RANK_CAP), lane)
-                              : wave_common_fwd_lite(src, n, pm_last + RANK_CAP, c_last + RANK_CAP, mlimit - (pm_last + RANK_CAP), lane);
+        const uint32_t a0 = pm_last + RANK_CAP, b0 = c_last + RANK_CAP, maxl = mlimit - a0;
+        if (!FEED || __builtin_expect(avail >= n, 1)) {
+          mext = BAMD_ENC_EXT2 ? wave_common_fwd(src, n, a0, b0, maxl, lane) : wave_common_fwd_lite(src, n, a0, b0, maxl, lane);
+        } else for (;;) {
+          const uint32_t rest = uni(maxl - mext), room = uni(avail - (a0 + mext)), here = umin32(rest, room);
+          const uint32_t got = uni(wave_common_fwd_lite(src, avail, a0 + mext, b0 + mext, here, lane));
+          mext += got;
+          if (__builtin_expect(got < here || rest <= room, 1)) break;
+          feed_wait(uni(a0 + mext) + 1u);
+        }
       }
       uint32_t back = valid ? umin32(nb_r, umin32(room, cand_r)) : 0u;
       if (BAMD_ENC_BACK2) {
@@ -275,7 +303,7 @@
       const uint32_t total = (uint32_t)__builtin_amdgcn_readlane((int)incl, (int)last) + extra_last;
       uint32_t ll0 = 0, prebytes = 0;
       if (pre) { ll0 = (uint32_t)__builtin_amdgcn_readlane((int)ll, 0); prebytes = 1u + (ll0 >= 15u ? 1u + (ll0 - 15u) / 255u : 0u) + pre; }
-      if (op + prebytes + total + 8u > cap) return 0u;
+      if (op + prebytes + total + 8u > cap) PAR_RETURN(0u);
       if (pre) {
         const uint32_t mc0 = (uint32_t)__builtin_amdgcn_readlane((int)mcode, 0);
         if (lane == 0) ENC_ST1(dst + op, (uint8_t)(((ll0 < 15u ? ll0 : 15u) << 4) | (mc0 < 15u ? mc0 : 15u)));
@@ -373,17 +401,32 @@
   }
 #undef PAR_PUT
 #undef PAR_PUT1
+  if (FEED && __builtin_expect(avail < n, 0)) feed_wait(n);
   op = lz4_emit_tail(dst, op, cap, src + anchor, n - anchor, lane);
-  if (op == 0xffffffffu) return 0u;
+  if (op == 0xffffffffu) PAR_RETURN(0u);
   PROF_LAP(12);
-  return op < n ? op : 0u;
+  PAR_RETURN(op < n ? op : 0u);
+#undef PAR_RETURN
+}
+template <int SS>
+__device__ __forceinline__ uint32_t lz4_encode_wave_par(const gu8* __restrict__ src, uint32_t n, gu8* __restrict__ dst, uint32_t cap,
+                                                        int clevel, enc_entry_t* tab_generic, int lane EPROF_ARG) {
+  return (uint32_t)lz4_encode_wave_fed<SS, false>(src, n, dst, cap, clevel, tab_generic, lane EPROF_PASS, nullptr);
 }
 
 #ifndef BAMD_ENC_STRIDE2_MAXCLEVEL
 #define BAMD_ENC_STRIDE2_MAXCLEVEL 5
 #endif
+__device__ __forceinline__ uint64_t lz4_encode_wave_auto_fed(const gu8* __restrict__ src, uint32_t n, gu8* __restrict__ dst, uint32_t cap,
+                                                             int clevel, enc_entry_t* tab_generic, int lane EPROF_ARG, uint32_t* fword) {
+  if (fword) {
+    if (clevel <= BAMD_ENC_STRIDE2_MAXCLEVEL) return lz4_encode_wave_fed<1, true>(src, n, dst, cap, clevel, tab_generic, lane EPROF_PASS, fword);
+    return lz4_encode_wave_fed<0, true>(src, n, dst, cap, clevel, tab_generic, lane EPROF_PASS, fword);
+  }
+  if (clevel <= BAMD_ENC_STRIDE2_MAXCLEVEL) return lz4_encode_wave_fed<1, false>(src, n, dst, cap, clevel, tab_generic, lane EPROF_PASS, nullptr);
+  return lz4_encode_wave_fed<0, false>(src, n, dst, cap, clevel, tab_generic, lane EPROF_PASS, nullptr);
+}
 __device__ __forceinline__ uint32_t lz4_encode_wave_auto(const gu8* __restrict__ src, uint32_t n, gu8* __restrict__ dst, uint32_t cap,
                                                          int clevel, enc_entry_t* tab_generic, int lane EPROF_ARG) {
-  if (clevel <= BAMD_ENC_STRIDE2_MAXCLEVEL) return lz4_encode_wave_par<1>(src, n, dst, cap, clevel, tab_generic, lane EPROF_PASS);
-  return lz4_encode_wave_par<0>(src, n, dst, cap, clevel, tab_generic, lane EPROF_PASS);
-}
+  return (uint32_t)lz4_encode_wave_auto_fed(src, n, dst, cap, clevel, tab_generic, lane EPROF_PASS, nullptr);
+}
diff --git a/c-blosc_amd/csrc/enc_shuffle.h b/c-blosc_amd/csrc/enc_shuffle.h
--- a/c-blosc_amd/csrc/enc_shuffle.h
+++ b/c-blosc_amd/csrc/enc_shuffle.h
@@ -1,3 +1,22 @@
+struct FeedPub {
+  uint32_t* word;
+  uint32_t seg, next, s;
+  __device__ __forceinline__ void init(uint32_t* w, uint32_t N) { word = w; seg = w ? feed_seg_bytes(N) : 0u; next = seg; s = 0u; }
+  __device__ __forceinline__ void at(uint32_t e, uint32_t N, uint32_t nonper, int lane) {
+    if (word == nullptr || e < next || e >= N) return;
+    s += 1u; next += seg;
+    if (nonper == 0u) return;
+    BAMD_MEM_SYNC();
+    __builtin_amdgcn_s_waitcnt(0);
+    const uint32_t w = FeedWord::make(s, nonper);
+    if (lane == 0) {
+      __hip_atomic_store(word, w, __ATOMIC_RELAXED, __HIP_MEMORY_SCOPE_AGENT);
+#ifdef BAMD_WAVE_EMU
+      if (g_emu_feed_published) g_emu_feed_published(w);
+#endif
+    }
+  }
+};
 template <int T>
 struct ElemRows { uint4 a, b; };
 
@@ -55,7 +74,7 @@
 #pragma unroll
   for (int k = 0; k < T; k++) g_st4(o + (size_t)k * N, r[k]);
 }
-__device__ __forceinline__ uint32_t shuffle_block_rows2(const gu8* src, gu8* dst, uint32_t N, int lane) {
+__device__ __forceinline__ uint32_t shuffle_block_rows2(const gu8* src, gu8* dst, uint32_t N, int lane, FeedPub& pub) {
   uint32_t e = 0, r[16];
   for (; e + 1024u <= N; e += 1024u) {
     const ElemRows2 a = shuffle_load2(src, e, lane), b = shuffle_load2(src, e + 256u, lane);
@@ -64,32 +83,36 @@
     shuffle_rows2(b, r); shuffle_store_rows<2>(dst, N, e + 256u, lane, r);
     shuffle_rows2(c, r); shuffle_store_rows<2>(dst, N, e + 512u, lane, r);
     shuffle_rows2(d, r); shuffle_store_rows<2>(dst, N, e + 768u, lane, r);
+    pub.at(e + 1024u, N, 3u, lane);
   }
   for (; e + 256u <= N; e += 256u) { shuffle_rows2(shuffle_load2(src, e, lane), r); shuffle_store_rows<2>(dst, N, e, lane, r); }
   return e;
 }
-__device__ __forceinline__ uint32_t shuffle_block_rows16(const gu8* src, gu8* dst, uint32_t N, int lane) {
+__device__ __forceinline__ uint32_t shuffle_block_rows16(const gu8* src, gu8* dst, uint32_t N, int lane, FeedPub& pub) {
   uint32_t e = 0, r[16];
   for (; e + 512u <= N; e += 512u) {
     const ElemRows16 a = shuffle_load16(src, e, lane), b = shuffle_load16(src, e + 256u, lane);
     shuffle_rows16(a, r, lane); shuffle_store_rows<16>(dst, N, e, lane, r);
     shuffle_rows16(b, r, lane); shuffle_store_rows<16>(dst, N, e + 256u, lane, r);
+    pub.at(e + 512u, N, 0xffffu, lane);
   }
   for (; e + 256u <= N; e += 256u) { shuffle_rows16(shuffle_load16(src, e, lane), r, lane); shuffle_store_rows<16>(dst, N, e, lane, r); }
   return e;
 }
 template <int T>
-__device__ void shuffle_block_wave_T(const gu8* src, gu8* dst, uint32_t bsize, int lane) {
+__device__ void shuffle_block_wave_T(const gu8* src, gu8* dst, uint32_t bsize, int lane, uint32_t* feed_word = nullptr) {
   const uint32_t N = bsize / T;
   uint32_t e = 0;
-  if constexpr (T == 2) e = shuffle_block_rows2(src, dst, N, lane);
-  else if constexpr (T == 16) e = shuffle_block_rows16(src, dst, N, lane);
+  FeedPub pub; pub.init(feed_word, N);
+  if constexpr (T == 2) e = shuffle_block_rows2(src, dst, N, lane, pub);
+  else if constexpr (T == 16) e = shuffle_block_rows16(src, dst, N, lane, pub);
   else {
   for (; e + 1024u <= N; e += 1024u) {
     const ElemRows<T> a = shuffle_load<T>(src, e, lane), b = shuffle_load<T>(src, e + 256u, lane);
     const ElemRows<T> c = shuffle_load<T>(src, e + 512u, lane), d = shuffle_load<T>(src, e + 768u, lane);
     shuffle_store<T>(dst, N, e, lane, a); shuffle_store<T>(dst, N, e + 256u, lane, b);
     shuffle_store<T>(dst, N, e + 512u, lane, c); shuffle_store<T>(dst, N, e + 768u, lane, d);
+    pub.at(e + 1024u, N, (1u << T) - 1u, lane);
   }
   for (; e + 256u <= N; e += 256u) shuffle_store<T>(dst, N, e, lane, shuffle_load<T>(src, e, lane));
   }
@@ -119,8 +142,9 @@
   return ((w0 >> 8) & 0xffu) == (w0 & 0xffu) ? 1u : 2u;
 }
 template <int T>
-__device__ uint32_t shuffle_block_wave_detect(const gu8* src, gu8* dst, uint32_t bsize, int lane, uint32_t (&period)[8]) {
+__device__ uint32_t shuffle_block_wave_detect(const gu8* src, gu8* dst, uint32_t bsize, int lane, uint32_t (&period)[8], uint32_t* feed_word = nullptr) {
   const uint32_t N = bsize / T;
+  FeedPub pub; pub.init(feed_word, N);
   uint32_t row0[8], r[8];
   uint32_t per = (1u << T) - 1u;
   shuffle_rows<T>(shuffle_load<T>(src, 0u, lane), row0);
@@ -143,6 +167,7 @@
     const ElemRows<T> a = shuffle_load<T>(src, e, lane), b = shuffle_load<T>(src, e + 256u, lane);
     const ElemRows<T> c = shuffle_load<T>(src, e + 512u, lane), d = shuffle_load<T>(src, e + 768u, lane);
     step(a, e); step(b, e + 256u); step(c, e + 512u); step(d, e + 768u);
+    pub.at(e + 1024u, N, ~per & ((1u << T) - 1u), lane);
   }
   for (; e + 256u <= N; e += 256u) step(shuffle_load<T>(src, e, lane), e);
 #pragma unroll
@@ -157,9 +182,10 @@
 }
 
 template <int T>
-__device__ uint32_t shuffle_block_wave_detect_x(const gu8* src, gu8* dst, uint32_t bsize, int lane, uint32_t (&period)[16]) {
+__device__ uint32_t shuffle_block_wave_detect_x(const gu8* src, gu8* dst, uint32_t bsize, int lane, uint32_t (&period)[16], uint32_t* feed_word = nullptr) {
   static_assert(T == 2 || T == 16, "typesize 4 / 8 use shuffle_block_wave_detect");
   const uint32_t N = bsize / T;
+  FeedPub pub; pub.init(feed_word, N);
   uint32_t row0[16], r[16];
   uint32_t per = (1u << T) - 1u;
   if constexpr (T == 2) shuffle_rows2(shuffle_load2(src, 0u, lane), row0); else shuffle_rows16(shuffle_load16(src, 0u, lane), row0, lane);
@@ -182,10 +208,11 @@
       const ElemRows2 a = shuffle_load2(src, e, lane), b = shuffle_load2(src, e + 256u, lane);
       const ElemRows2 c = shuffle_load2(src, e + 512u, lane), d = shuffle_load2(src, e + 768u, lane);
       shuffle_rows2(a, r); step(e); shuffle_rows2(b, r); step(e + 256u); shuffle_rows2(c, r); step(e + 512u); shuffle_rows2(d, r); step(e + 768u);
+      pub.at(e + 1024u, N, ~per & 3u, lane);
     }
     for (; e + 256u <= N; e += 256u) { shuffle_rows2(shuffle_load2(src, e, lane), r); step(e); }
   } else {
-    for (; e + 256u <= N; e += 256u) { shuffle_rows16(shuffle_load16(src, e, lane), r, lane); step(e); }
+    for (; e + 256u <= N; e += 256u) { shuffle_rows16(shuffle_load16(src, e, lane), r, lane); step(e); pub.at(e + 256u, N, ~per & 0xffffu, lane); }
   }
 #pragma unroll
   for (int k = 0; k < T; k++) {
@@ -199,22 +226,26 @@
 }
 
 template <int T>
-__device__ __forceinline__ void shuffle_block_detect_T(const gu8* src, gu8* dst, uint32_t bsize, StreamDesc* planes, int lane) {
+__device__ __forceinline__ uint32_t shuffle_block_detect_T(const gu8* src, gu8* dst, uint32_t bsize, StreamDesc* planes, int lane, uint32_t* feed_word) {
   uint32_t period[(T == 4 || T == 8) ? 8 : 16];
   uint32_t per;
-  if constexpr (T == 4 || T == 8) per = shuffle_block_wave_detect<T>(src, dst, bsize, lane, period);
-  else per = shuffle_block_wave_detect_x<T>(src, dst, bsize, lane, period);
+  if constexpr (T == 4 || T == 8) per = shuffle_block_wave_detect<T>(src, dst, bsize, lane, period, feed_word);
+  else per = shuffle_block_wave_detect_x<T>(src, dst, bsize, lane, period, feed_word);
 #pragma unroll
   for (int k = 0; k < T; k++)
     if ((per & (1u << k)) && lane == 0) planes[k].result = -(int32_t)period[k];
-}
-__device__ __attribute__((noinline)) void shuffle_block_task_x(const gu8* src_, gu8* dst_, uint32_t bsize_, uint32_t T_, bool det_, StreamDesc* planes_, int lane) {
+  return ~per & ((1u << T) - 1u);
+}
+__device__ __attribute__((noinline)) uint32_t shuffle_block_task_x(const gu8* src_, gu8* dst_, uint32_t bsize_, uint32_t T_, bool det_, StreamDesc* planes_, int lane, uint32_t* feed_word_) {
   const gu8* src = uni_ptr(src_); gu8* dst = uni_ptr(dst_);
   const uint32_t bsize = uni(bsize_), T = uni(T_); const bool det = uni((uint32_t)det_) != 0u;
   const uint64_t pv = (uint64_t)planes_;
   StreamDesc* planes = (StreamDesc*)(((uint64_t)uni((uint32_t)(pv >> 32)) << 32) | uni((uint32_t)pv));
-  if (T == 16u) { if (det) shuffle_block_detect_T<16>(src, dst, bsize, planes, lane); else shuffle_block_wave_T<16>(src, dst, bsize, lane); }
-  else { if (det) shuffle_block_detect_T<2>(src, dst, bsize, planes, lane); else shuffle_block_wave_T<2>(src, dst, bsize, lane); }
+  uint32_t* fw = uni_gp(feed_word_);
+  if (T == 16u) { if (det) return shuffle_block_detect_T<16>(src, dst, bsize, planes, lane, fw); shuffle_block_wave_T<16>(src, dst, bsize, lane, fw); return 0xffffu; }
+  if (det) return shuffle_block_detect_T<2>(src, dst, bsize, planes, lane, fw);
+  shuffle_block_wave_T<2>(src, dst, bsize, lane, fw);
+  return 3u;
 }
 template <int T, int EPL>
 __device__ __forceinline__ void bitshuffle_pass(const gu8* src, gu8* dst, uint32_t rowlen, uint32_t e0, uint32_t nchunks, int lane) {
@@ -324,23 +355,34 @@
 }
 
 __device__ __attribute__((noinline)) void shuffle_block_task(const ChunkDesc* chunks, const BlockDesc* blocks, uint32_t gb,
-                                                             uint32_t* blk_ready, StreamDesc* streams, int detect, int lane, volatile uint32_t* lds) {
+                                                             uint32_t* blk_ready, StreamDesc* streams, int flags , int lane, volatile uint32_t* lds) {
+  const bool detect = (flags & ENC_FLAG_DETECT) != 0, feed = (flags & ENC_FLAG_FEED) != 0;
   const BlockDesc* b = blocks + gb;
   const ChunkDesc* c = chunks + uni((uint32_t)b->chunk);
   const uint32_t blk = uni((uint32_t)b->blk), bsize = uni((uint32_t)b->bsize), bs = uni((uint32_t)c->blocksize);
   const gu8* src = uni_ptr(as_global(c->src)) + (size_t)blk * bs;
   gu8* dst = uni_ptr(as_global(c->filt)) + (size_t)blk * bs;
   const uint32_t T = uni((uint32_t)c->typesize), N = bsize / T;
-  const bool det = detect && uni((uint32_t)b->nstreams) == T && N * T == bsize && (N & 255u) == 0u && N >= 1024u &&
-                   (uni((uint32_t)c->fmt) == (uint32_t)FMT_LZ4 || uni((uint32_t)c->fmt) == (uint32_t)FMT_BLOSCLZ);
+  const bool geo = feed_geometry(uni((uint32_t)b->nstreams), T, N, bsize);
+  const bool det = detect && geo && (uni((uint32_t)c->fmt) == (uint32_t)FMT_LZ4 || uni((uint32_t)c->fmt) == (uint32_t)FMT_BLOSCLZ);
   StreamDesc* planes = streams + uni((uint32_t)b->first_stream);
+  const bool regs = !(uni(c->mode) & CH_BITSHUFFLE) && !shuffle_generic_T(T);
+  uint32_t* fw = feed && geo && regs ? blk_ready + gb : nullptr;
+  uint32_t nonper = 0u;
   if (uni(c->mode) & CH_BITSHUFFLE) bitshuffle_block_task_x(src, dst, bsize, T, lane);
   else if (shuffle_generic_T(T)) shuffle_block_generic(lds, src, dst, bsize, T, lane);
-  else if (T == 8u) { if (det) shuffle_block_detect_T<8>(src, dst, bsize, planes, lane); else shuffle_block_wave_T<8>(src, dst, bsize, lane); }
-  else if (T == 4u) { if (det) shuffle_block_detect_T<4>(src, dst, bsize, planes, lane); else shuffle_block_wave_T<4>(src, dst, bsize, lane); }
-  else shuffle_block_task_x(src, dst, bsize, T, det, planes, lane);
+  else if (T == 8u) { if (det) nonper = shuffle_block_detect_T<8>(src, dst, bsize, planes, lane, fw); else { shuffle_block_wave_T<8>(src, dst, bsize, lane, fw); nonper = 0xffu; } }
+  else if (T == 4u) { if (det) nonper = shuffle_block_detect_T<4>(src, dst, bsize, planes, lane, fw); else { shuffle_block_wave_T<4>(src, dst, bsize, lane, fw); nonper = 0xfu; } }
+  else nonper = shuffle_block_task_x(src, dst, bsize, T, det, planes, lane, fw);
+  BAMD_MEM_SYNC();
   __builtin_amdgcn_s_waitcnt(0);
-  if (lane == 0) __hip_atomic_store(&blk_ready[gb], 1u, __ATOMIC_RELAXED, __HIP_MEMORY_SCOPE_AGENT);
+  const uint32_t w = FeedWord::DONE | (fw ? FeedWord::make((N + feed_seg_bytes(N) - 1u) / feed_seg_bytes(N), uni(nonper)) : 0u);
+  if (lane == 0) {
+    __hip_atomic_store(&blk_ready[gb], w, __ATOMIC_RELAXED, __HIP_MEMORY_SCOPE_AGENT);
+#ifdef BAMD_WAVE_EMU
+    if (g_emu_feed_published) g_emu_feed_published(w);
+#endif
+  }
 }
 
 __device__ __forceinline__ uint32_t emit_periodic_stream(const gu8* in, uint32_t n, gu8* out, uint32_t cap, uint32_t p, bool lz4, int lane) {
diff --git a/c-blosc_amd/csrc/engine.h b/c-blosc_amd/csrc/engine.h
--- a/c-blosc_amd/csrc/engine.h
+++ b/c-blosc_amd/csrc/engine.h
@@ -58,6 +58,7 @@
 int engine_persistent_grids(int cap, const char** names, int* launched, int* occupancy);
 int engine_enc_lz_occupancy(int dynamic_lds);
 void engine_last_compress_tasks(uint32_t out[3]);
+int engine_enc_feed(int mode);
 
 int engine_set_device(int dev);
 int engine_thread_device(int dev);
diff --git a/c-blosc_amd/csrc/engine.hip b/c-blosc_amd/csrc/engine.hip
--- a/c-blosc_amd/csrc/engine.hip
+++ b/c-blosc_amd/csrc/engine.hip
@@ -595,6 +595,8 @@
 #endif
 }
 static std::atomic<uint32_t> g_last_enc_tasks[3];
+static std::atomic<int> g_enc_feed_mode{0};
+int engine_enc_feed(int mode) { return g_enc_feed_mode.exchange(mode ? 1 : 0); }
 void engine_last_compress_tasks(uint32_t out[3]) { for (int i = 0; i < 3; i++) out[i] = g_last_enc_tasks[i].load(); }
 
 struct SelectRun { int nchunks; const int* first; int* choice; int* answers; };
@@ -729,7 +731,9 @@
     uint32_t* d_ready = (uint32_t*)(D + o_ready);
     uint64_t* d_seqbufs = r.o_seqbufs ? (uint64_t*)(D + r.o_seqbufs) : nullptr;
     const zenc::CTabs* d_ctabs = r.o_ctabs ? (const zenc::CTabs*)(D + r.o_ctabs) : nullptr;
-    const int detect = (kEncMode[r.v.mode].family == FAM_LZ && periodic_enabled()) ? 1 : 0;
+    const bool feed_on = g_enc_feed_mode.load() != 0;
+    const int detect = ((kEncMode[r.v.mode].family == FAM_LZ && periodic_enabled()) ? ENC_FLAG_DETECT : 0)
+                     | (feed_on ? ENC_FLAG_FEED : 0);
     const dim3 grid(persistent_grid(st, (size_t)g.ntasks, r.v.waves_per_cu)), block(64 * ENC_WAVES);
     BAMD_STREAM_PROFILE(prof, "BLOSC_AMD_ENC_PROFILE", nstr);
     BAMD_WAVE_PROFILE(wprof, "BLOSC_AMD_ENC_PROFILE", grid.x);
diff --git a/c-blosc_amd/csrc/k_encode.hip b/c-blosc_amd/csrc/k_encode.hip
--- a/c-blosc_amd/csrc/k_encode.hip
+++ b/c-blosc_amd/csrc/k_encode.hip
@@ -46,12 +46,14 @@
 #define BAMD_ENC_HELP 256
 #endif
 template <int MODE>
+__device__ __forceinline__ bool feed_stream(int feed, uint32_t fmt) { return MODE == ENC_LZ && BAMD_ENC_PAR && feed && fmt == (uint32_t)FMT_LZ4; }
+template <int MODE>
 __device__ __attribute__((noinline)) void encode_one_stream(StreamDesc* sd_, enc_entry_t* tab_, const ChunkDesc* chunks_, uint32_t* blk_ready_, int lane,
                                                             const BlockDesc* blocks_, uint32_t sid_, uint32_t* plane_cost_, uint64_t* seqbuf_
 #ifdef BAMD_PROFILE_DECODE
                                                             , uint32_t* profslot_
 #endif
-                                                            ) {
+                                                            , int feed_ = 0) {
   StreamDesc* sd; enc_entry_t* tab; const ChunkDesc* chunks; uint32_t* blk_ready; const BlockDesc* blocks; uint32_t sid; uint32_t* plane_cost; uint64_t* seqbuf;
 #ifdef BAMD_PROFILE_DECODE
   uint32_t* profslot;
@@ -68,30 +70,44 @@
   const uint32_t n = uni((uint32_t)sd->in_size), cap = uni((uint32_t)sd->out_size);
   const uint32_t aux = uni((uint32_t)sd->aux);
   const int clevel = (int)(aux & 15u);
+  uint32_t* fword = nullptr;
+  uint32_t fwaited = 0u;
   if (uni(chunks[uni((uint32_t)sd->chunk)].mode) & CH_FUSED_SHUF) {
     const uint32_t gb = aux >> 4;
-    while (__hip_atomic_load(&blk_ready[gb], __ATOMIC_RELAXED, __HIP_MEMORY_SCOPE_AGENT) == 0u) __builtin_amdgcn_s_sleep(16);
+    const bool can = feed_stream<MODE>((int)uni((uint32_t)feed_), uni((uint32_t)sd->fmt));
+    const uint32_t j = can ? sid - uni((uint32_t)blocks[gb].first_stream) : 16u;
+    for (;;) {
+      const uint32_t w = uni(__hip_atomic_load(&blk_ready[gb], __ATOMIC_RELAXED, __HIP_MEMORY_SCOPE_AGENT));
+      if (FeedWord::done(w)) break;
+      if (can && feed_may_start(w, j)) { fword = blk_ready + gb; break; }
+      __builtin_amdgcn_s_sleep(16);
+    }
     __builtin_amdgcn_fence(__ATOMIC_ACQUIRE, "agent");
   }
   PROF_LAP(13);
   const uint64_t cost_t0 = __builtin_amdgcn_s_memtime();
   uint32_t r;
-  const int32_t hint = (int32_t)uni((uint32_t)sd->result);
+  const int32_t hint = fword ? 0 : (int32_t)uni((uint32_t)sd->result);
   constexpr EncMode M = kEncMode[MODE];
   if (M.family == FAM_ZSTD) r = seqbuf ? zstd_encode_wave<M.tables, M.search, M.huffman>(uni_ptr(as_global(sd->in)), n, uni_ptr(as_global(sd->out)), cap, clevel, tab, (BAMD_GAS uint64_t*)seqbuf, lane EPROF_PASS) : 0u;
   else if (M.dynamic) r = seqbuf ? zlib_dyn_encode_wave<M.search>(uni_ptr(as_global(sd->in)), n, uni_ptr(as_global(sd->out)), cap, clevel, tab, (BAMD_GAS uint64_t*)seqbuf, lane EPROF_PASS) : 0u;
   else if (M.family == FAM_ZLIB) r = zlib_encode_wave<M.search>(uni_ptr(as_global(sd->in)), n, uni_ptr(as_global(sd->out)), cap, clevel, tab, lane EPROF_PASS);
   else if (hint < 0) r = emit_periodic_stream(uni_ptr(as_global(sd->in)), n, uni_ptr(as_global(sd->out)), cap, (uint32_t)-hint, uni((uint32_t)sd->fmt) == (uint32_t)FMT_LZ4, lane);
   else if (M.search) r = lz4hc_encode_wave(uni_ptr(as_global(sd->in)), n, uni_ptr(as_global(sd->out)), cap, tab, lane);
-  else if (sd->fmt == FMT_LZ4) r = BAMD_ENC_PAR ? lz4_encode_wave_auto(uni_ptr(as_global(sd->in)), n, uni_ptr(as_global(sd->out)), cap, clevel, tab, lane EPROF_PASS)
-                                                : lz_encode_wave<EF_LZ4>(uni_ptr(as_global(sd->in)), n, uni_ptr(as_global(sd->out)), cap, clevel, tab, lane EPROF_PASS);
+  else if (sd->fmt == FMT_LZ4) {
+    if (BAMD_ENC_PAR) {
+      const uint64_t rw = lz4_encode_wave_auto_fed(uni_ptr(as_global(sd->in)), n, uni_ptr(as_global(sd->out)), cap, clevel, tab, lane EPROF_PASS, fword);
+      r = (uint32_t)rw; fwaited = (uint32_t)(rw >> 32);
+    } else r = lz_encode_wave<EF_LZ4>(uni_ptr(as_global(sd->in)), n, uni_ptr(as_global(sd->out)), cap, clevel, tab, lane EPROF_PASS);
+  }
   else r = lz_encode_wave<EF_BLOSCLZ>(uni_ptr(as_global(sd->in)), n, uni_ptr(as_global(sd->out)), cap, clevel, tab, lane EPROF_PASS);
   if (lane == 0) sd->result = (int32_t)r;
   if (plane_cost && lane == 0) {
     const uint32_t j = sid - (uint32_t)blocks[aux >> 4].first_stream;
-    atomicAdd(plane_cost + (j & 255u), (uint32_t)((__builtin_amdgcn_s_memtime() - cost_t0) >> 10));
-  }
-#ifdef BAMD_PROFILE_DECODE
+    atomicAdd(plane_cost + (j & 255u), (uint32_t)((__builtin_amdgcn_s_memtime() - cost_t0 - (uint64_t)fwaited) >> 10));
+  }
+#ifdef BAMD_PROFILE_DECODE
+  prof_.c[13] += fwaited;
   prof_.c[15] = (uint32_t)__builtin_amdgcn_s_memrealtime();
   if (lane == 0 && profslot) for (int i_ = 0; i_ < 16; i_++) profslot[i_] = prof_.c[i_];
 #endif
@@ -107,7 +123,7 @@
     StreamDesc* __restrict__ streams, uint32_t* __restrict__ tickets , const int32_t* __restrict__ qlist,
     const int32_t* __restrict__ qoff , const int32_t* __restrict__ shoff , const ChunkDesc* __restrict__ chunks, const BlockDesc* __restrict__ blocks,
     uint32_t* __restrict__ blk_ready, uint32_t* __restrict__ plane_cost, int single_queue,
-    uint64_t* __restrict__ seqbufs, const zenc::CTabs* __restrict__ ctabs, int detect_periodic
+    uint64_t* __restrict__ seqbufs, const zenc::CTabs* __restrict__ ctabs, int enc_flags
 #ifdef BAMD_PROFILE_DECODE
     , uint32_t* __restrict__ profbuf, uint32_t* __restrict__ profwave
 #endif
@@ -123,6 +139,7 @@
 #define WPROF_END(acc, t)
 #endif
   constexpr bool ZSTD = kEncMode[MODE].family == FAM_ZSTD;
+  const int feed = enc_flags & ENC_FLAG_FEED;
   constexpr uint32_t SEQWORDS = enc_seq_words(MODE);
   constexpr int TABBYTES = enc_tab_bytes(MODE);
   __shared__ __attribute__((aligned(16))) enc_entry_t tabs[ENC_WAVES][lds_occupied(enc_lds_bytes(MODE)) / 4];
@@ -141,7 +158,7 @@
     const uint32_t s = take_ticket(tickets + 8 + xcc, lane);
     if (s >= shlen) return false;
     WPROF_BEGIN(ts_);
-    shuffle_block_task(chunks, blocks, uni((uint32_t)shlist[shbase + s]), blk_ready, streams, detect_periodic, lane, (volatile uint32_t*)tabs[0]);
+    shuffle_block_task(chunks, blocks, uni((uint32_t)shlist[shbase + s]), blk_ready, streams, enc_flags, lane, (volatile uint32_t*)tabs[0]);
     WPROF_END(wt_shuffle, ts_);
 #ifdef BAMD_PROFILE_DECODE
     wn_shuffle++;
@@ -160,10 +177,14 @@
         const uint32_t gb = uni((uint32_t)sd->aux) >> 4;
         const ChunkDesc* cd = chunks + uni((uint32_t)sd->chunk);
         bool more = !(uni(cd->mode) & CH_BITSHUFFLE) && shuffle_generic_T(uni((uint32_t)cd->typesize));
+        const bool can = feed_stream<MODE>(feed, uni((uint32_t)sd->fmt));
+        const uint32_t pj = can ? (uint32_t)task - uni((uint32_t)blocks[gb].first_stream) : 16u;
 #ifdef BAMD_PROFILE_DECODE
         const uint64_t tw_ = __builtin_amdgcn_s_memtime(), sh0_ = wt_shuffle;
 #endif
-        while (__hip_atomic_load(&blk_ready[gb], __ATOMIC_RELAXED, __HIP_MEMORY_SCOPE_AGENT) == 0u) {
+        for (;;) {
+          const uint32_t w = uni(__hip_atomic_load(&blk_ready[gb], __ATOMIC_RELAXED, __HIP_MEMORY_SCOPE_AGENT));
+          if (FeedWord::done(w) || (can && feed_may_start(w, pj))) break;
           if (BAMD_ENC_HELP && more && __hip_atomic_load(tickets + 8 + xcc, __ATOMIC_RELAXED, __HIP_MEMORY_SCOPE_AGENT) < (single_queue ? gb : gb / 8u) + (uint32_t)BAMD_ENC_HELP) more = shuffle_one();
           else __builtin_amdgcn_s_sleep(16);
         }
@@ -174,10 +195,10 @@
       }
 #ifdef BAMD_PROFILE_DECODE
       const uint64_t te_ = __builtin_amdgcn_s_memtime();
-      encode_one_stream<MODE>(streams + task, tabs[0], chunks, blk_ready, lane, blocks, (uint32_t)task, plane_cost, seqbuf, profbuf ? profbuf + (size_t)task * 16 : nullptr);
+      encode_one_stream<MODE>(streams + task, tabs[0], chunks, blk_ready, lane, blocks, (uint32_t)task, plane_cost, seqbuf, profbuf ? profbuf + (size_t)task * 16 : nullptr, feed);
       wt_stream += __builtin_amdgcn_s_memtime() - te_; wn_stream++;
 #else
-      encode_one_stream<MODE>(streams + task, tabs[0], chunks, blk_ready, lane, blocks, (uint32_t)task, plane_cost, seqbuf);
+      encode_one_stream<MODE>(streams + task, tabs[0], chunks, blk_ready, lane, blocks, (uint32_t)task, plane_cost, seqbuf, feed);
 #endif
     }
     ndone++;
```

Measured after the change: 776.3 GB/s. 4.6% lower.
